# zser092/Focused-Attention-ViT

Hardware: AMD Instinct MI355X
Metric: images/sec (train fwd+bwd) ViT-MHLA 224/p16 (higher is better)
Workload: dtype bf16; 1 GPU; ViT-MHLA-Small (D384/12L/6H, window 7) 224x224 patch16, 197 tokens, 256 images/GPU; step = fwd + cross-entropy + bwd + grad all-reduce + AdamW; global_batch=256, parallelism=dp1, weights=random-init (seed 1234), hip_graph=False

## Files before the change

### focused-attention-vit_amd/_abi.py

```python
from __future__ import annotations

import ctypes as C
import os
import re

_HERE = os.path.dirname(os.path.abspath(__file__))
LIB_PATH = os.path.join(_HERE, "lib", "libfavit.so")
HEADER_PATH = os.path.join(os.path.dirname(_HERE), "include", "favit.h")

F32, BF16, FP8 = 0, 1, 2
F32X3 = 3
E4M3, E5M2 = 0, 1
ACT_NONE, ACT_GELU, ACT_DGELU, ACT_GELU_SAVEGRAD, ACT_MULAUX = 0, 1, 2, 3, 4
ERR_INVALID, ERR_UNSUPPORTED, ERR_ALIGN, ERR_LAUNCH = -1, -2, -3, -4
POOL = {"mean": 0, "max": 1, "attention": 2}

vp, i32, i64, u64, f32 = C.c_void_p, C.c_int32, C.c_int64, C.c_uint64, C.c_float


class GemmDesc(C.Structure):
    _fields_ = [
        ("A", vp), ("B", vp), ("C", vp), ("bias", vp), ("aux_in", vp), ("aux_out", vp), ("residual", vp),
        ("a_rowsum", vp),
        ("M", i64), ("N", i64), ("K", i64),
        ("lda", i64), ("ldb", i64), ("ldc", i64), ("ld_aux_in", i64), ("ld_aux_out", i64), ("ld_res", i64),
        ("sAo", i64), ("sAi", i64), ("sBo", i64), ("sBi", i64), ("sCo", i64), ("sCi", i64),
        ("batch", i32), ("batch_inner", i32), ("a_kmajor", i32), ("b_kmajor", i32),
        ("in_dtype", i32), ("out_dtype", i32), ("act", i32), ("accumulate", i32), ("split_k", i32),
        ("alpha", f32), ("dropout_p", f32), ("fp8_fmt", i32), ("dropout_seed", u64),
        ("scale_a", vp), ("scale_b", vp),
    ]


class SdpaDesc(C.Structure):
    _fields_ = [
        ("q", vp), ("k", vp), ("v", vp), ("o", vp), ("lse", vp), ("dout", vp), ("dq", vp), ("dk", vp), ("dv", vp),
        ("delta", vp), ("mask", vp), ("m_sb", i64), ("m_sq", i64),
        ("q_str", i64 * 3), ("k_str", i64 * 3), ("v_str", i64 * 3), ("o_str", i64 * 3), ("do_str", i64 * 3),
        ("dq_str", i64 * 3), ("dk_str", i64 * 3), ("dv_str", i64 * 3),
        ("B", i32), ("H", i32), ("Lq", i32), ("Lk", i32), ("hd", i32), ("dtype", i32),
        ("scale", f32), ("dropout_p", f32), ("seed", u64),
    ]


class BlockDesc(C.Structure):
    _fields_ = [
        ("x", vp), ("tape", vp), ("g1", vp), ("b1", vp), ("g2", vp), ("b2", vp), ("weff", vp), ("beff", vp),
        ("wproj", vp), ("bproj", vp), ("wfc1", vp), ("bfc1", vp), ("wfc2", vp), ("bfc2", vp),
        ("tape_bytes", i64),
        ("B", i32), ("n", i32), ("D", i32), ("H", i32), ("W", i32), ("hidden", i32), ("training", i32), ("eps", f32),
    ]


BLOCK_TAPE_SLOTS = ("xn1", "mu1", "rs1", "qkv", "o", "lse", "x1", "xn2", "mu2", "rs2", "h", "pre", "x2")
BLOCK_BWD_SLOTS = ("dpre", "dxn2", "g1_f32", "g1_lp", "do", "dqkv", "dxn1", "g_out_f32", "g_out_lp", "part1", "part2")

_SIGS = {
    "favit_abi_version": ([], C.c_int),
    "favit_strerror": ([C.c_int], C.c_char_p),
    "favit_set_dropout_epoch": ([vp], C.c_int),
    "favit_set_health_word": ([vp], C.c_int),
    "favit_gemm": ([C.POINTER(GemmDesc), vp], C.c_int),
    "favit_gemm_last_kernel": ([], C.c_char_p),
    "favit_ln_gemm": ([C.POINTER(GemmDesc), vp, i64, vp, vp, f32, vp, vp, vp, vp], C.c_int),
    "favit_gemm_grouped_tn": ([C.POINTER(GemmDesc), i32, vp], C.c_int),
    "favit_gemm_grouped_tn_workspace": ([C.POINTER(GemmDesc), i32], C.c_int64),
    "favit_gemm_grouped_tn_ws": ([C.POINTER(GemmDesc), i32, vp, i64, vp], C.c_int),
    "favit_gemm_grouped_tn_ragged": ([C.POINTER(GemmDesc), i32, vp], C.c_int),
    "favit_gemm_grouped_tn_ragged_workspace": ([C.POINTER(GemmDesc), i32], C.c_int64),
    "favit_gemm_grouped_tn_ragged_ws": ([C.POINTER(GemmDesc), i32, vp, i64, vp], C.c_int),
    "favit_gemm_grouped_last_splits": ([], C.c_int),
    "favit_gemm_grouped_plan": ([C.POINTER(GemmDesc), i32, i32, vp, i32], C.c_int),
    "favit_cast": ([vp, C.c_int, vp, C.c_int, i64, vp], C.c_int),
    "favit_fp8_amax": ([vp, C.c_int, i64, i64, i64, vp, vp], C.c_int),
    "favit_fp8_quantize": ([vp, C.c_int, i64, i64, i64, vp, i64, vp, i64, C.c_int, vp, vp, vp, vp, vp, vp], C.c_int),
    "favit_layernorm_fwd": ([vp, i64, vp, vp, vp, C.c_int, vp, vp, i64, i32, f32, vp], C.c_int),
    "favit_layernorm_bwd": ([vp, C.c_int, vp, i64, vp, vp, vp, vp, vp, i64, vp, C.c_int, vp, vp, i32, vp, vp, i32,
                             i64, i32, f32, u64, vp], C.c_int),
    "favit_layernorm_fwd_q8": ([vp, i64, vp, vp, vp, vp, vp, i64, i32, f32, vp, C.c_int, vp, vp, vp, vp, vp], C.c_int),
    "favit_layernorm_bwd_q8": ([vp, vp, i64, vp, vp, vp, vp, vp, i64, vp, vp, vp, i32, vp, vp, i32, i64, i32, f32, u64,
                                vp, C.c_int, vp, vp, vp, vp, vp], C.c_int),
    "favit_small_linear_fwd": ([vp, i64, vp, vp, vp, i32, i32, i32, vp], C.c_int),
    "favit_small_linear_bwd": ([vp, vp, i64, vp, vp, vp, vp, i32, i32, i32, i32, vp], C.c_int),
    "favit_reduce_rows": ([vp, i64, vp, i64, i32, i32, vp], C.c_int),
    "favit_reduce_rows_multi": ([i32, vp, vp, vp, i64, i32, vp], C.c_int),
    "favit_reduce_rows_multi_ragged": ([i32, vp, vp, vp, vp, i32, vp], C.c_int),
    "favit_mhla_fold_fwd": ([vp, vp, vp, vp, vp, C.c_int, vp, vp, i32, i32, vp], C.c_int),
    "favit_mhla_fold_fwd_multi": ([i32, vp, vp, vp, vp, vp, C.c_int, vp, i32, i32, vp], C.c_int),
    "favit_mhla_fold_bwd": ([vp, vp, vp, vp, vp, vp, vp, vp, vp, i32, i32, i32, vp], C.c_int),
    "favit_mhla_fold_bwd_multi": ([i32, vp, vp, vp, vp, vp, vp, vp, vp, vp, i32, i32, vp], C.c_int),
    "favit_mhla_attn_fwd": ([vp, vp, vp, i32, i32, i32, i32, i32, C.c_int, f32, u64, vp], C.c_int),
    "favit_mhla_attn_bwd": ([vp, vp, vp, vp, i32, i32, i32, i32, i32, C.c_int, f32, u64, vp], C.c_int),
    "favit_mhla_attn_lse_supported": ([i32, i32, i32, C.c_int], C.c_int),
    "favit_mhla_attn_fwd_lse": ([vp, vp, vp, vp, i32, i32, i32, i32, i32, C.c_int, f32, u64, vp], C.c_int),
    "favit_mhla_attn_bwd_lse": ([vp, vp, vp, vp, vp, vp, i32, i32, i32, i32, i32, C.c_int, f32, u64, vp], C.c_int),
    "favit_sdpa_fwd": ([C.POINTER(SdpaDesc), vp], C.c_int),
    "favit_sdpa_bwd": ([C.POINTER(SdpaDesc), vp], C.c_int),
    "favit_softmax_fwd": ([vp, vp, vp, C.c_int, vp, i64, i64, i32, i64, i32, i32, f32, u64, vp], C.c_int),
    "favit_softmax_bwd": ([vp, C.c_int, vp, vp, C.c_int, i64, i32, i32, f32, u64, vp], C.c_int),
    "favit_patchify_fwd": ([vp, vp, C.c_int, i32, i32, i32, i32, vp], C.c_int),
    "favit_patchify_bwd": ([vp, vp, i32, i32, i32, i32, vp], C.c_int),
    "favit_embed_prologue_fwd": ([vp, vp, vp, vp, i32, i32, i32, vp], C.c_int),
    "favit_embed_prologue_bwd": ([vp, vp, C.c_int, vp, vp, i32, i32, i32, vp], C.c_int),
    "favit_rows_cut_fwd": ([vp, vp, i32, i32, i32, i32, i32, vp], C.c_int),
    "favit_rows_cut_bwd": ([vp, vp, vp, C.c_int, i32, i32, i32, i32, i32, vp], C.c_int),
    "favit_mhla_block_tape_layout": ([C.POINTER(BlockDesc), C.POINTER(i64)], C.c_int64),
    "favit_mhla_block_bwd_layout": ([C.POINTER(BlockDesc), i32, C.POINTER(i64)], C.c_int64),
    "favit_mhla_block_fwd": ([C.POINTER(BlockDesc), vp], C.c_int),
    "favit_mhla_block_bwd": ([C.POINTER(BlockDesc), vp, vp, vp, i64, i32, vp], C.c_int),
    "favit_dropout": ([vp, vp, C.c_int, i64, f32, u64, vp], C.c_int),
    "favit_sppp_map_patches": ([vp, vp, vp, vp, vp, vp, i32, i32, i32, vp], C.c_int),
    "favit_sppp_pool_fwd": ([vp, vp, vp, vp, vp, i32, i32, i32, i32, i32, vp], C.c_int),
    "favit_sppp_pool_bwd": ([vp, vp, vp, vp, vp, vp, vp, i32, i32, i32, i32, i32, vp], C.c_int),
    "favit_sppp_centroids": ([vp, vp, i32, i32, i32, vp], C.c_int),
    "favit_sppp_posenc_fwd": ([vp, vp, vp, i32, i32, i32, i32, vp], C.c_int),
    "favit_image_transform": ([vp, vp, vp, vp, vp, i32, i32, i32, i32, i32, i32, C.POINTER(f32), C.POINTER(f32), vp], C.c_int),
    "favit_image_transform_ragged": ([vp, vp, vp, vp, vp, vp, i32, i32, i32, i32, C.POINTER(f32), C.POINTER(f32), vp], C.c_int),
    "favit_slic_features_workspace": ([i32, i32, i32], C.c_int64),
    "favit_slic_features": ([vp, vp, i32, i32, i32, f32, i32, vp, vp], C.c_int),
    "favit_slic_cluster_workspace": ([i32, i32], C.c_int64),
    "favit_slic_cluster": ([vp, vp, vp, i32, i32, i32, i32, i32, i64, i32, vp, vp], C.c_int),
    "favit_slic_connect": ([vp, vp, vp, vp, vp, i32, i32, i32, i32, vp], C.c_int),
    "favit_cross_entropy": ([vp, vp, vp, vp, i32, i32, f32, vp], C.c_int),
    "favit_adamw": ([vp, vp, vp, vp, vp, i64, f32, f32, f32, f32, f32, f32, f32, f32, vp], C.c_int),
    "favit_cross_entropy_ls": ([vp, vp, vp, vp, i32, i32, f32, f32, vp], C.c_int),
    "favit_grad_norm_workspace": ([], C.c_int64),
    "favit_grad_norm": ([i32, vp, vp, f32, f32, vp, vp, vp, i64, vp], C.c_int),
    "favit_adamw_clip": ([vp, vp, vp, vp, vp, i64, f32, f32, f32, f32, f32, f32, f32, f32, vp, i32, vp], C.c_int),
    "favit_adamw_ema": ([vp, vp, vp, vp, vp, vp, i64, f32, f32, f32, f32, f32, f32, f32, f32, f32, vp], C.c_int),
    "favit_adamw_clip_ema": ([vp, vp, vp, vp, vp, vp, i64, f32, f32, f32, f32, f32, f32, f32, f32, vp, i32, f32, vp],
                             C.c_int),
    "favit_swap_params": ([vp, vp, vp, i64, vp], C.c_int),
    "favit_batch_mix": ([vp, vp, vp, i32, i32, i32, i32, vp], C.c_int),
    "favit_cross_entropy_mix": ([vp, vp, vp, vp, vp, i32, i32, f32, f32, vp], C.c_int),
    "favit_randaugment_max_ops": ([], C.c_int),
    "favit_randaugment": ([vp, vp, vp, vp, vp, i32, vp, C.POINTER(f32), i32, u64, i32, i32, i32, C.POINTER(f32),
                           C.POINTER(f32), vp], C.c_int),
    "favit_random_erase": ([vp, vp, C.POINTER(f32), i32, u64, i32, i32, i32, i32, vp], C.c_int),
}

_lib = None


class FavitLibraryError(RuntimeError):
    pass


def declared_symbols():
    with open(HEADER_PATH) as f:
        txt = f.read()
    return sorted(set(re.findall(r"\b(favit_[a-z0-9_]+)\s*\(", txt)))


def lib():
    global _lib
    if _lib is None:
        if not os.path.exists(LIB_PATH):
            raise FavitLibraryError(
                f"{LIB_PATH} not found: build it with `python -c 'import __graft_entry__ as g; g.build()'` "
                "or `make -C focused-attention-vit_amd/csrc`.  There is no CPU / PyTorch fallback.")
        try:
            l = C.CDLL(LIB_PATH)
        except OSError as e:
            raise FavitLibraryError(f"cannot load {LIB_PATH}: {e}") from e
        for name, (args, res) in _SIGS.items():
            fn = getattr(l, name)
            fn.argtypes = args
            fn.restype = res
        _lib = l
    return _lib


def check(code: int, what: str):
    if code != 0:
        msg = lib().favit_strerror(code).decode()
        raise RuntimeError(f"{what} failed: {msg} (code {code})")
```

### focused-attention-vit_amd/csrc/block.hip

```cpp
#include <string.h>

#include "favit.h"

namespace {
constexpr int64_t ALIGN = 256;
constexpr int TAPE_N = FAVIT_BLOCK_TAPE_SLOTS, BWD_N = FAVIT_BLOCK_BWD_SLOTS;
enum { T_XN1, T_MU1, T_RS1, T_QKV, T_O, T_LSE, T_X1, T_XN2, T_MU2, T_RS2, T_H, T_PRE, T_X2 };
enum { G_DPRE, G_DXN2, G_G1_F32, G_G1_LP, G_DO, G_DQKV, G_DXN1, G_OUT_F32, G_OUT_LP, G_PART1, G_PART2 };

inline int64_t up(int64_t v) { return (v + ALIGN - 1) / ALIGN * ALIGN; }

int check_geometry(const favit_mhla_block_t* d) {
  if (!d) return FAVIT_ERR_INVALID;
  if (d->B <= 0 || d->n <= 0 || d->D <= 0 || d->H <= 0 || d->W <= 0 || d->hidden <= 0 || !(d->eps > 0.f))
    return FAVIT_ERR_INVALID;
  if (d->D % 64 != 0 || d->D % d->H != 0 || d->D / d->H != 64) return FAVIT_ERR_UNSUPPORTED;
  if (d->hidden % 8 != 0) return FAVIT_ERR_UNSUPPORTED;
  if (!favit_mhla_attn_lse_supported(d->n, 64, d->W, FAVIT_BF16)) return FAVIT_ERR_UNSUPPORTED;
  if ((int64_t)d->B * d->n >= (int64_t)1 << 31) return FAVIT_ERR_UNSUPPORTED;
  return FAVIT_OK;
}

int64_t layout(const int64_t* sizes, int n, int64_t* offsets) {
  int64_t off = 0;
  for (int i = 0; i < n; ++i) {
    if (offsets) offsets[i] = off;
    off += up(sizes[i]);
  }
  return off;
}

void tape_sizes(const favit_mhla_block_t* d, int64_t* s) {
  const int64_t M = (int64_t)d->B * d->n, D = d->D, Hd = d->hidden;
  s[T_XN1] = M * D * 2; s[T_MU1] = M * 4; s[T_RS1] = M * 4;
  s[T_QKV] = M * 3 * D * 2; s[T_O] = M * D * 2;
  s[T_LSE] = d->training ? (int64_t)d->B * d->H * d->n * 4 : 0;
  s[T_X1] = M * D * 4;
  s[T_XN2] = M * D * 2; s[T_MU2] = M * 4; s[T_RS2] = M * 4;
  s[T_H] = M * Hd * 2; s[T_PRE] = M * Hd * 2;
  s[T_X2] = M * D * 4;
}

int32_t ln_parts(int64_t rows) { return (int32_t)((rows + 3) / 4 < 2048 ? (rows + 3) / 4 : 2048); }

void bwd_sizes(const favit_mhla_block_t* d, int want_lp_out, int64_t* s) {
  const int64_t M = (int64_t)d->B * d->n, D = d->D, Hd = d->hidden;
  const int64_t part = 2 * (int64_t)ln_parts(M) * D * 4;
  s[G_DPRE] = M * Hd * 2; s[G_DXN2] = M * D * 2;
  s[G_G1_F32] = M * D * 4; s[G_G1_LP] = M * D * 2;
  s[G_DO] = M * D * 2; s[G_DQKV] = M * 3 * D * 2; s[G_DXN1] = M * D * 2;
  s[G_OUT_F32] = M * D * 4; s[G_OUT_LP] = want_lp_out ? M * D * 2 : 0;
  s[G_PART1] = part; s[G_PART2] = part;
}

favit_gemm_t gemm_base(const void* A, const void* B, void* C, int64_t M, int64_t N, int64_t K, int64_t ldb, int b_kmajor,
                       int out_dtype) {
  favit_gemm_t g;
  memset(&g, 0, sizeof(g));
  g.A = A; g.B = B; g.C = C;
  g.M = M; g.N = N; g.K = K;
  g.lda = K; g.ldb = ldb; g.ldc = N;
  g.batch = 1; g.batch_inner = 1;
  g.a_kmajor = 1; g.b_kmajor = b_kmajor;
  g.in_dtype = FAVIT_BF16; g.out_dtype = out_dtype;
  g.act = FAVIT_ACT_NONE;
  g.alpha = 1.0f;
  return g;
}

int check_params(const favit_mhla_block_t* d) {
  if (!d->x || !d->tape || !d->g1 || !d->b1 || !d->g2 || !d->b2 || !d->weff || !d->beff || !d->wproj || !d->bproj ||
      !d->wfc1 || !d->bfc1 || !d->wfc2 || !d->bfc2)
    return FAVIT_ERR_INVALID;
  if (((uintptr_t)d->tape % ALIGN) != 0 || ((uintptr_t)d->x % 16) != 0) return FAVIT_ERR_ALIGN;
  return FAVIT_OK;
}
}

extern "C" int64_t favit_mhla_block_tape_layout(const favit_mhla_block_t* desc, int64_t* offsets_out) {
  const int rc = check_geometry(desc);
  if (rc != FAVIT_OK) return rc;
  int64_t s[TAPE_N];
  tape_sizes(desc, s);
  return layout(s, TAPE_N, offsets_out);
}

extern "C" int64_t favit_mhla_block_bwd_layout(const favit_mhla_block_t* desc, int32_t want_lp_out, int64_t* offsets_out) {
  const int rc = check_geometry(desc);
  if (rc != FAVIT_OK) return rc;
  int64_t s[BWD_N];
  bwd_sizes(desc, want_lp_out, s);
  return layout(s, BWD_N, offsets_out);
}

extern "C" int favit_mhla_block_fwd(const favit_mhla_block_t* d, void* stream) {
  int rc = check_geometry(d);
  if (rc != FAVIT_OK) return rc;
  if ((rc = check_params(d)) != FAVIT_OK) return rc;
  int64_t s[TAPE_N], o[TAPE_N];
  tape_sizes(d, s);
  if (d->tape_bytes < layout(s, TAPE_N, o)) return FAVIT_ERR_INVALID;
  char* t = reinterpret_cast<char*>(d->tape);
  const int64_t M = (int64_t)d->B * d->n;
  const int32_t D = d->D, Hd = d->hidden;
  float* x1 = reinterpret_cast<float*>(t + o[T_X1]);
  if ((rc = favit_layernorm_fwd(d->x, D, d->g1, d->b1, t + o[T_XN1], FAVIT_BF16, reinterpret_cast<float*>(t + o[T_MU1]),
                                reinterpret_cast<float*>(t + o[T_RS1]), M, D, d->eps, stream)) != FAVIT_OK)
    return rc;
  favit_gemm_t g = gemm_base(t + o[T_XN1], d->weff, t + o[T_QKV], M, 3 * D, D, D, 1, FAVIT_BF16);
  g.bias = d->beff;
  g.ld_aux_out = 3 * D; g.ld_res = 3 * D;
  if ((rc = favit_gemm(&g, stream)) != FAVIT_OK) return rc;
  rc = d->training ? favit_mhla_attn_fwd_lse(t + o[T_QKV], t + o[T_O], reinterpret_cast<float*>(t + o[T_LSE]), nullptr,
                                             d->B, d->n, d->H, 64, d->W, FAVIT_BF16, 0.f, 0, stream)
                   : favit_mhla_attn_fwd(t + o[T_QKV], t + o[T_O], nullptr, d->B, d->n, d->H, 64, d->W, FAVIT_BF16, 0.f, 0,
                                         stream);
  if (rc != FAVIT_OK) return rc;
  g = gemm_base(t + o[T_O], d->wproj, x1, M, D, D, D, 1, FAVIT_F32);
  g.bias = d->bproj; g.residual = d->x;
  g.ld_aux_out = D; g.ld_res = D;
  if ((rc = favit_gemm(&g, stream)) != FAVIT_OK) return rc;
  if ((rc = favit_layernorm_fwd(x1, D, d->g2, d->b2, t + o[T_XN2], FAVIT_BF16, reinterpret_cast<float*>(t + o[T_MU2]),
                                reinterpret_cast<float*>(t + o[T_RS2]), M, D, d->eps, stream)) != FAVIT_OK)
    return rc;
  g = gemm_base(t + o[T_XN2], d->wfc1, t + o[T_H], M, Hd, D, D, 1, FAVIT_BF16);
  g.bias = d->bfc1; g.act = FAVIT_ACT_GELU_SAVEGRAD; g.aux_out = t + o[T_PRE];
  g.ld_aux_out = Hd; g.ld_res = Hd;
  if ((rc = favit_gemm(&g, stream)) != FAVIT_OK) return rc;
  g = gemm_base(t + o[T_H], d->wfc2, t + o[T_X2], M, D, Hd, Hd, 1, FAVIT_F32);
  g.bias = d->bfc2; g.residual = x1;
  g.ld_aux_out = D; g.ld_res = D;
  return favit_gemm(&g, stream);
}

extern "C" int favit_mhla_block_bwd(const favit_mhla_block_t* d, const float* g_f32, const void* g_lp, void* bwd_buffers,
                                    int64_t bwd_bytes, int32_t want_lp_out, void* stream) {
  int rc = check_geometry(d);
  if (rc != FAVIT_OK) return rc;
  if ((rc = check_params(d)) != FAVIT_OK) return rc;
  if (!d->training || !g_f32 || !g_lp || !bwd_buffers) return FAVIT_ERR_INVALID;
  if (((uintptr_t)bwd_buffers % ALIGN) != 0 || ((uintptr_t)g_f32 % 16) != 0 || ((uintptr_t)g_lp % 16) != 0)
    return FAVIT_ERR_ALIGN;
  int64_t s[TAPE_N], o[TAPE_N], bs[BWD_N], b[BWD_N];
  tape_sizes(d, s);
  if (d->tape_bytes < layout(s, TAPE_N, o)) return FAVIT_ERR_INVALID;
  bwd_sizes(d, want_lp_out, bs);
  if (bwd_bytes < layout(bs, BWD_N, b)) return FAVIT_ERR_INVALID;
  char* t = reinterpret_cast<char*>(d->tape);
  char* w = reinterpret_cast<char*>(bwd_buffers);
  const int64_t M = (int64_t)d->B * d->n;
  const int32_t D = d->D, Hd = d->hidden, np = ln_parts(M);
  float* g1 = reinterpret_cast<float*>(w + b[G_G1_F32]);
  float* part1 = reinterpret_cast<float*>(w + b[G_PART1]);
  float* part2 = reinterpret_cast<float*>(w + b[G_PART2]);
  favit_gemm_t g = gemm_base(g_lp, d->wfc2, w + b[G_DPRE], M, Hd, D, Hd, 0, FAVIT_BF16);
  g.act = FAVIT_ACT_MULAUX; g.aux_in = t + o[T_PRE]; g.ld_aux_in = Hd;
  if ((rc = favit_gemm(&g, stream)) != FAVIT_OK) return rc;
  g = gemm_base(w + b[G_DPRE], d->wfc1, w + b[G_DXN2], M, D, Hd, D, 0, FAVIT_BF16);
  g.ld_aux_in = D;
  if ((rc = favit_gemm(&g, stream)) != FAVIT_OK) return rc;
  if ((rc = favit_layernorm_bwd(w + b[G_DXN2], FAVIT_BF16, reinterpret_cast<const float*>(t + o[T_X1]), D, d->g2,
                                reinterpret_cast<const float*>(t + o[T_MU2]), reinterpret_cast<const float*>(t + o[T_RS2]),
                                g_f32, g1, D, w + b[G_G1_LP], FAVIT_BF16, part2, part2 + (int64_t)np * D, np, nullptr,
                                nullptr, 1, M, D, 0.f, 0, stream)) != FAVIT_OK)
    return rc;
  g = gemm_base(w + b[G_G1_LP], d->wproj, w + b[G_DO], M, D, D, D, 0, FAVIT_BF16);
  g.ld_aux_in = D;
  if ((rc = favit_gemm(&g, stream)) != FAVIT_OK) return rc;
  if ((rc = favit_mhla_attn_bwd_lse(t + o[T_QKV], w + b[G_DO], t + o[T_O], reinterpret_cast<const float*>(t + o[T_LSE]),
                                    w + b[G_DQKV], nullptr, d->B, d->n, d->H, 64, d->W, FAVIT_BF16, 0.f, 0, stream)) !=
      FAVIT_OK)
    return rc;
  g = gemm_base(w + b[G_DQKV], d->weff, w + b[G_DXN1], M, D, 3 * D, D, 0, FAVIT_BF16);
  g.ld_aux_in = D;
  if ((rc = favit_gemm(&g, stream)) != FAVIT_OK) return rc;
  return favit_layernorm_bwd(w + b[G_DXN1], FAVIT_BF16, d->x, D, d->g1, reinterpret_cast<const float*>(t + o[T_MU1]),
                             reinterpret_cast<const float*>(t + o[T_RS1]), g1, reinterpret_cast<float*>(w + b[G_OUT_F32]), D,
                             want_lp_out ? w + b[G_OUT_LP] : nullptr, FAVIT_BF16, part1, part1 + (int64_t)np * D, np, nullptr,
                             nullptr, 1, M, D, 0.f, 0, stream);
}
```

### focused-attention-vit_amd/functional.py

```python
from __future__ import annotations

import os
import weakref
from typing import List, Optional, Sequence, Tuple

import torch

from . import kernels as K
from ._abi import ACT_DGELU, ACT_GELU, ACT_GELU_SAVEGRAD, ACT_MULAUX, ACT_NONE

_STATE = {"cdt": torch.float32, "epoch": 0, "direct_grads": True, "grad_ready": None}


def set_direct_grads(on: bool) -> None:
    _STATE["direct_grads"] = bool(on)


def set_grad_ready_hook(fn) -> None:
    _STATE["grad_ready"] = fn


def _gt(p):
    if p is None or not _STATE["direct_grads"] or not getattr(p, "requires_grad", False):
        return None
    g = p.grad
    if g is None or g.dtype != torch.float32 or not g.is_contiguous() or g.shape != p.shape or not g.is_cuda:
        return None
    return g


def _ready(*params):
    fn = _STATE["grad_ready"]
    if fn is not None:
        for p in params:
            if p is not None:
                if _SIDE["active"]:
                    _SIDE["pending"].append(p)
                else:
                    fn(p)


_SIDE = {"enabled": False, "stream": None, "active": False, "pending": [], "used": False}


def set_side_stream(on: bool) -> None:
    _SIDE["enabled"] = bool(on)


class _side_stream:

    def __init__(self, *tensors):
        self.tensors = [t for t in tensors if t is not None]

    def __enter__(self):
        if not _SIDE["enabled"]:
            self.ctx = None
            return self
        if _SIDE["stream"] is None:
            _SIDE["stream"] = torch.cuda.Stream()
        s = _SIDE["stream"]
        s.wait_stream(torch.cuda.current_stream())
        for t in self.tensors:
            t.record_stream(s)
        self.ctx = torch.cuda.stream(s)
        self.ctx.__enter__()
        _SIDE["active"] = True
        _SIDE["used"] = True
        return self

    def __exit__(self, *exc):
        if self.ctx is not None:
            _SIDE["active"] = False
            self.ctx.__exit__(*exc)
        return False


def join_side_stream() -> None:
    if _SIDE["used"]:
        torch.cuda.current_stream().wait_stream(_SIDE["stream"])
        _SIDE["used"] = False
    if _SIDE["pending"]:
        fn = _STATE["grad_ready"]
        pend, _SIDE["pending"] = _SIDE["pending"], []
        if fn is not None:
            for p in pend:
                fn(p)


def set_compute_dtype(d) -> None:
    fp8 = x3 = False
    if isinstance(d, str):
        fp8 = d == "fp8"
        x3 = d == "fp32x3"
        d = {"fp32": torch.float32, "float32": torch.float32, "fp32x3": torch.float32, "bf16": torch.bfloat16,
             "bfloat16": torch.bfloat16, "fp8": torch.bfloat16}[d]
    if d not in (torch.float32, torch.bfloat16):
        raise ValueError("compute dtype must be fp32, fp32x3, bf16 or fp8")
    if d == torch.float32 and os.environ.get("FAVIT_FP32_GEMM") == "x3":
        x3 = True
    _STATE["cdt"] = d
    _STATE["fp8"] = fp8
    _STATE["x3"] = x3
    K.set_f32_gemm_split(x3)


def get_compute_mode() -> str:
    if _STATE.get("fp8"):
        return "fp8"
    if _STATE["cdt"] == torch.bfloat16:
        return "bf16"
    return "fp32x3" if _STATE.get("x3") else "fp32"


def get_compute_dtype() -> torch.dtype:
    return _STATE["cdt"]


def bump_weight_epoch(synced_mirrors=()) -> None:
    _STATE["epoch"] += 1
    for m in synced_mirrors:
        m.epoch = _STATE["epoch"]


class _LPMirror:
    __slots__ = ("flat_ref", "lp", "epoch", "versions", "params")

    def __init__(self, flat_p, lp, params=()):
        self.flat_ref, self.lp, self.params = weakref.ref(flat_p), lp, [weakref.ref(p) for p in params]
        self.mark_synced()

    def mark_synced(self):
        self.epoch = _STATE["epoch"]
        self.versions = {id(p): p._version for p in (r() for r in self.params) if p is not None}

    def refresh_if_stale(self) -> bool:
        fp = self.flat_ref()
        if fp is None:
            return False
        stale = self.epoch != _STATE["epoch"]
        if not stale:
            for r in self.params:
                p = r()
                if p is not None and self.versions.get(id(p), p._version) != p._version:
                    stale = True
                    break
        if stale:
            K.cast(fp, torch.bfloat16, out=self.lp)
            self.mark_synced()
        return stale

    def lookup(self, src, w):
        fp = self.flat_ref()
        if fp is None:
            return None
        base, ptr = fp.data_ptr(), w.data_ptr()
        if not (base <= ptr < base + 4 * fp.numel()):
            return False
        if self.epoch != _STATE["epoch"]:
            K.cast(fp, torch.bfloat16, out=self.lp)
            self.epoch = _STATE["epoch"]
        off = (ptr - base) // 4
        view = self.lp[off:off + w.numel()].view(w.shape)
        key = id(src)
        ver = src._version
        if self.versions.get(key, ver) != ver:
            K.cast(w, torch.bfloat16, out=view)
        self.versions[key] = ver
        return view


_LP_MIRRORS: List[_LPMirror] = []


def register_lp_mirror(flat_p: torch.Tensor, flat_lp: torch.Tensor, params=()) -> _LPMirror:
    m = _LPMirror(flat_p, flat_lp, params)
    _LP_MIRRORS.append(m)
    return m


def clear_lp_mirrors() -> None:
    _LP_MIRRORS.clear()


def invalidate_weight_cache() -> None:
    _STATE["epoch"] += 1


def wcast(w: torch.Tensor) -> torch.Tensor:
    cdt = _STATE["cdt"]
    src = w
    w = w.detach()
    if w.dtype == cdt and w.is_contiguous():
        return w
    if cdt == torch.bfloat16 and w.dtype == torch.float32 and w.is_contiguous():
        for m in list(_LP_MIRRORS):
            hit = m.lookup(src, w)
            if hit is None:
                _LP_MIRRORS.remove(m)
            elif hit is not False:
                return hit
    tag = (w.data_ptr(), tuple(w.shape), w._version, _STATE["epoch"], cdt)
    hit = getattr(src, "_favit_cast", None)
    if hit is not None and hit[0] == tag:
        return hit[1]
    c = K.cast(w, cdt)
    try:
        src._favit_cast = (tag, c)
    except AttributeError:
        pass
    return c


def set_dropout_epoch(word: Optional[torch.Tensor]) -> None:
    if word is not None:
        K.require_gpu(word)
        if word.dtype != torch.int64 or word.numel() != 1:
            raise TypeError("the dropout epoch is a one-element int64 device tensor")
    _STATE["drop_epoch"] = word
    from . import _abi
    _abi.check(_abi.lib().favit_set_dropout_epoch(None if word is None else word.data_ptr()), "favit_set_dropout_epoch")


def get_dropout_epoch() -> Optional[torch.Tensor]:
    return _STATE.get("drop_epoch")


def _seed() -> int:
    if torch.cuda.is_available() and torch.cuda.is_current_stream_capturing() and _STATE.get("drop_epoch") is None:
        raise RuntimeError("dropout inside a captured HIP graph: the seed is a kernel argument and would be frozen "
                           "into the graph; register a dropout epoch word first (functional.set_dropout_epoch; "
                           "train.GraphedStep does it for models with dropout)")
    return int(torch.empty((), dtype=torch.int64).random_().item())


_SEG = {"n": 1, "boundaries": []}


class encoder_segments:

    def __init__(self, n: int):
        self.n = max(1, int(n))

    def __enter__(self):
        self.prev = (_SEG["n"], _SEG["boundaries"])
        _SEG["n"], _SEG["boundaries"] = self.n, []
        self.boundaries = _SEG["boundaries"]
        return self

    def __exit__(self, *exc):
        _SEG["n"], _SEG["boundaries"] = self.prev
        return False


def get_encoder_segments() -> int:
    return _SEG["n"]


def note_segment_boundary(x: torch.Tensor) -> torch.Tensor:
    leaf = x.detach().requires_grad_(True)
    _SEG["boundaries"].append((x, leaf))
    return leaf


def _as_cdt(x: torch.Tensor) -> torch.Tensor:
    cdt = _STATE["cdt"]
    x = x.contiguous()
    return x if x.dtype == cdt else K.cast(x, cdt)


def _as_f32(x: torch.Tensor) -> torch.Tensor:
    x = x.contiguous()
    return x if x.dtype == torch.float32 else K.cast(x, torch.float32)


def _mask_u8(mask: Optional[torch.Tensor]) -> Optional[torch.Tensor]:
    if mask is None:
        return None
    return (mask != 0).to(torch.uint8).contiguous()


E4M3, E5M2 = torch.float8_e4m3fn, torch.float8_e5m2


_FP8_HIST = {}


def _fp8_hist(site, role: str):
    if site is None or torch.cuda.is_current_stream_capturing():
        return None
    key = (id(site), role)
    ent = _FP8_HIST.get(key)
    if ent is None or ent[0]() is not site:
        ent = (weakref.ref(site), K.Fp8History(site.device))
        _FP8_HIST[key] = ent
        if len(_FP8_HIST) > 4096:
            for k in [k for k, v in _FP8_HIST.items() if v[0]() is None]:
                del _FP8_HIST[k]
    return ent[1]


def _q8(t: torch.Tensor, fmt: torch.dtype, want_t: bool = False, hist=None):
    hit = getattr(t, "_favit_q8", None)
    if hit is not None and hit[0] == (fmt, t._version) and (hit[1][1] is not None or not want_t):
        return hit[1]
    q, qt, sinv = K.fp8_quantize(t, fmt, want=True, want_t=want_t, hist=hist)
    out = (q, qt, sinv)
    try:
        t._favit_q8 = ((fmt, t._version), out)
    except AttributeError:
        pass
    return out


def _q8_request(chain, prm, which: str, D: int):
    if not _STATE.get("fp8") or get_compute_dtype() != torch.bfloat16 or D % 64 != 0 or os.environ.get("FAVIT_FP8_NO_LNQ8"):
        return None
    idx = getattr(chain, "q8_" + which, None)
    if idx is None or prm is None or idx >= len(prm) or prm[idx] is None:
        return None
    hist = _fp8_hist(prm[idx], "a" if which == "fwd" else "dy")
    return None if hist is None else ((E4M3 if which == "fwd" else E5M2), hist)


def _use_fp8(allow, *mats, k_dims=()):
    if not (allow and _STATE.get("fp8")):
        return False
    return all(m.dtype == torch.bfloat16 and m.dim() == 2 and m.is_contiguous() for m in mats) and \
        all(k % 64 == 0 for k in k_dims)


def lin_fwd(a, w_c, bias, M, N, Kd, out_dtype, *, act=ACT_NONE, residual=None, want_pre=False, drop=(0.0, 0),
            allow_fp8=True, site=None):
    out = torch.empty((M, N), dtype=out_dtype, device=a.device)
    pre = torch.empty((M, N), dtype=out_dtype, device=a.device) if want_pre else None
    if _use_fp8(allow_fp8, a, w_c, k_dims=(Kd,)):
        aq, _, sa = _q8(a, E4M3, hist=_fp8_hist(site, "a"))
        wq, _, sw = _q8(w_c, E4M3, want_t=True, hist=_fp8_hist(site, "w"))
        K.gemm(aq, wq, out, M, N, Kd, Kd, Kd, N, bias=bias, act=act, aux_out=pre, ld_aux_out=N, residual=residual,
               ld_res=N, dropout_p=drop[0], dropout_seed=drop[1], scale_a=sa, scale_b=sw)
        return (out, pre) if want_pre else out
    K.gemm(a, w_c, out, M, N, Kd, Kd, Kd, N, bias=bias, act=act, aux_out=pre, ld_aux_out=N, residual=residual,
           ld_res=N, dropout_p=drop[0], dropout_seed=drop[1])
    return (out, pre) if want_pre else out


_LN_FUSE = bool(os.environ.get("FAVIT_LN_FUSE"))


def lin_fwd_ln(ln, w_c, bias, M, N, Kd, out_dtype, *, act=ACT_NONE, want_pre=False, drop=(0.0, 0)):
    x, gamma, beta = ln
    if _LN_FUSE and w_c.dtype == torch.bfloat16 and get_compute_mode() != "fp8":
        out = torch.empty((M, N), dtype=out_dtype, device=x.device)
        pre = torch.empty((M, N), dtype=out_dtype, device=x.device) if want_pre else None
        r = K.ln_gemm(x, Kd, gamma, beta, w_c, out, M, N, Kd, bias=bias, act=act, aux_out=pre, dropout_p=drop[0],
                      dropout_seed=drop[1])
        if r is not None:
            return (out, pre) + r
    xn, mu, rs = K.layernorm_fwd(x, Kd, gamma, beta, M, Kd, get_compute_dtype())
    o = lin_fwd(xn, w_c, bias, M, N, Kd, out_dtype, act=act, want_pre=want_pre, drop=drop)
    return (o + (xn, mu, rs)) if want_pre else (o, None, xn, mu, rs)


def lin_bwd_x(dy, w_c, M, N, Kd, out_dtype, *, dgelu_pre=None, pre_is_grad=False, drop=(0.0, 0), allow_fp8=True,
              site=None):
    dx = torch.empty((M, Kd), dtype=out_dtype, device=dy.device)
    act = (ACT_MULAUX if pre_is_grad else ACT_DGELU) if dgelu_pre is not None else ACT_NONE
    if _use_fp8(allow_fp8, dy, w_c, k_dims=(N,)) and (dgelu_pre is None or dgelu_pre.dtype == torch.bfloat16):
        dyq, _, sdy = _q8(dy, E5M2, hist=_fp8_hist(site, "dy"))
        _, wqt, sw = _q8(w_c, E4M3, want_t=True, hist=_fp8_hist(site, "w"))
        K.gemm(dyq, wqt, dx, M, Kd, N, N, wqt.stride(0), Kd, act=act, aux_in=dgelu_pre, ld_aux_in=Kd,
               dropout_p=drop[0], dropout_seed=drop[1], scale_a=sdy, scale_b=sw)
        return dx
    K.gemm(dy, w_c, dx, M, Kd, N, N, Kd, Kd, b_kmajor=False, act=act,
           aux_in=dgelu_pre, ld_aux_in=Kd, dropout_p=drop[0], dropout_seed=drop[1])
    return dx


_WG = {"list": None, "blocks": 0, "every": 1, "bytes": 0, "ragged": False, "ends": [], "blk_bytes": 0}
_WG_HOLD_BYTES = int(float(os.environ.get("FAVIT_WGRAD_HOLD_MB", "384")) * (1 << 20))
_WG_HOLD_RAGGED_BYTES = int(float(os.environ.get("FAVIT_WGRAD_HOLD_MB", "2048")) * (1 << 20))


def begin_wgrads(per_block: bool = False) -> None:
    every = 4 if _STATE["grad_ready"] is not None else K.GROUP_MAX // 4
    ragged = per_block
    if _SIDE["enabled"] or os.environ.get("FAVIT_WGRAD_PER_BLOCK"):
        every = 1
        ragged = False
    _WG.update(list=[], blocks=0, every=every, bytes=0, ragged=ragged, ends=[], blk_bytes=0)


def _launch_wgrads(probs) -> None:
    if not K.gemm_grouped_tn(probs):
        for dy, a, dw, db, acc in probs:
            K.gemm(dy, a, dw, dy.shape[1], a.shape[1], dy.shape[0], dy.stride(0), a.stride(0), dw.stride(0),
                   a_kmajor=False, b_kmajor=False, a_rowsum=db, accumulate=acc)


def flush_wgrads(force: bool = True, next_rows=None) -> bool:
    lst = _WG["list"]
    if lst is None:
        return True
    if not force:
        _WG["blocks"] += 1
        nb = _WG["blocks"]
        if _WG["ragged"]:
            ends = _WG["ends"]
            n_blk = len(lst) - (ends[-1] if ends else 0)
            b_blk = _WG["bytes"] - _WG["blk_bytes"]
            ends.append(len(lst))
            _WG["blk_bytes"] = _WG["bytes"]
            scale = next_rows[1] / max(next_rows[0], 1) if next_rows else 1.0
            if nb < _WG["every"] and _WG["bytes"] + b_blk * scale <= _WG_HOLD_RAGGED_BYTES and len(lst) + n_blk <= K.GROUP_MAX:
                return not lst
        elif nb < _WG["every"] and _WG["bytes"] * (nb + 1) <= _WG_HOLD_BYTES * nb and len(lst) * (nb + 1) <= K.GROUP_MAX * nb:
            return not lst
    ends = _WG["ends"]
    _WG.update(blocks=0, bytes=0, ends=[], blk_bytes=0)
    if lst:
        _WG["list"] = []
        probs = [(dy, a, dw, db, acc) for dy, a, dw, db, acc, _ in lst]
        with _side_stream(*[t for pr in probs for t in pr[:4]]):
            if not _WG["ragged"]:
                _launch_wgrads(probs)
            elif not K.gemm_grouped_tn_ragged(probs):
                bounds = [0] + [e for e in ends if 0 < e < len(probs)] + [len(probs)]
                for lo, hi in zip(bounds[:-1], bounds[1:]):
                    if hi > lo:
                        _launch_wgrads(probs[lo:hi])
            for *_, ready in lst:
                _ready(*ready)
    return True


def end_wgrads() -> None:
    flush_wgrads()
    _WG["list"] = None


_DEFER = {"on": False, "fold": [], "ln": []}


def begin_deferred() -> None:
    _DEFER.update(on=not _SIDE["enabled"], fold=[], ln=[])


def flush_deferred() -> None:
    if not _DEFER["on"]:
        return
    assert not _WG["list"], "the latent_proj fold reads weight gradients that have not been launched"
    fold, ln = _DEFER["fold"], _DEFER["ln"]
    _DEFER["fold"], _DEFER["ln"] = [], []
    if ln:
        by_cols = {}
        for e in ln:
            by_cols.setdefault(e[0].shape[-1], []).append(e)
        for es in by_cols.values():
            K.reduce_rows_multi([e[:3] for e in es])
        for e in ln:
            _ready(*e[3])
    by_h = {}
    for e in fold:
        by_h.setdefault((e[6], tuple(e[2].shape), e[5][0] is None), []).append(e)
    for (H, _, _), es in by_h.items():
        K.mhla_fold_bwd_multi([e[:6] for e in es], H)
        for e in es:
            _ready(*e[7])


def end_deferred() -> None:
    flush_deferred()
    _DEFER["on"] = False


_ZPOOL = {"buf": None, "off": 0}


def begin_zero_pool(n_floats: int, device) -> None:
    _ZPOOL["buf"] = torch.zeros(n_floats, dtype=torch.float32, device=device) if n_floats > 0 else None
    _ZPOOL["off"] = 0


def end_zero_pool() -> None:
    _ZPOOL["buf"] = None


def _zero_vec(n: int, device) -> torch.Tensor:
    buf = _ZPOOL["buf"]
    n4 = (n + 3) // 4 * 4
    if buf is not None and buf.device == device and _ZPOOL["off"] + n4 <= buf.numel():
        o = _ZPOOL["off"]
        _ZPOOL["off"] = o + n4
        return buf[o:o + n]
    return torch.zeros(n, dtype=torch.float32, device=device)


def lin_bwd_w(dy, a, M, N, Kd, want_bias=True, wp=None, bp=None, allow_fp8=True):
    frozen_w = wp is not None and not wp.requires_grad
    frozen_b = (not want_bias) or (bp is not None and not bp.requires_grad)
    if frozen_w and frozen_b:
        return None, None
    tw = _gt(wp)
    tb = _gt(bp) if want_bias else None
    dw = tw if tw is not None else torch.empty((N, Kd), dtype=torch.float32, device=dy.device)
    db = None
    if want_bias:
        db = tb if tb is not None else _zero_vec(N, dy.device)
    if _WG["list"] is not None and dy.dtype == torch.bfloat16:
        _WG["list"].append((dy, a, dw, db, tw is not None,
                            [p for p, t in ((wp, tw), (bp, tb)) if t is not None]))
        _WG["bytes"] += dy.numel() * dy.element_size() + a.numel() * a.element_size()
        return (None if tw is not None else dw), (None if tb is not None else db)
    with _side_stream(dy, a, dw, db):
        if not (dy.dtype == torch.bfloat16 and M >= 8192 and (db is not None or not want_bias) and
                K.gemm_grouped_tn([(dy, a, dw, db, tw is not None)])):
            K.gemm(dy, a, dw, N, Kd, M, N, Kd, Kd, a_kmajor=False, b_kmajor=False, a_rowsum=db,
                   accumulate=tw is not None)
    if tw is not None:
        _ready(wp)
    if tb is not None:
        _ready(bp)
    return (None if tw is not None else dw), (None if tb is not None else db)


class _View:
    __slots__ = ("t", "off", "ld", "sb", "sh")

    def __init__(self, t, off, ld, sb, sh):
        self.t, self.off, self.ld, self.sb, self.sh = t, off, ld, sb, sh


def sdpa_fwd(q: _View, k: _View, v: _View, o: _View, B, H, Lq, Lk, hd, scale, mask, m_sb, m_sq, p, seed):
    if hd % 16 == 0:
        return (K.sdpa_fwd(q, k, v, o, B, H, Lq, Lk, hd, scale, mask, m_sb, m_sq, p, seed),)
    cdt = q.t.dtype
    Z = B * H
    S = torch.empty((Z, Lq, Lk), dtype=torch.float32, device=q.t.device)
    K.gemm(q.t, k.t, S, Lq, Lk, hd, q.ld, k.ld, Lk, alpha=scale, batch=Z, batch_inner=H, sA=(q.sb, q.sh),
           sB=(k.sb, k.sh), sC=(H * Lq * Lk, Lq * Lk), a_off=q.off, b_off=k.off)
    P, Pd = K.softmax_fwd(S, cdt, H, Z, Lq, Lk, mask, m_sb, m_sq, p, seed)
    K.gemm(Pd, v.t, o.t, Lq, hd, Lk, Lk, v.ld, o.ld, b_kmajor=False, batch=Z, batch_inner=H,
           sA=(H * Lq * Lk, Lq * Lk), sB=(v.sb, v.sh), sC=(o.sb, o.sh), b_off=v.off, c_off=o.off)
    return P, Pd


def sdpa_bwd(q: _View, k: _View, v: _View, o: _View, do: _View, dq: _View, dk: _View, dv: _View, saved, B, H, Lq, Lk,
             hd, scale, mask, m_sb, m_sq, p, seed):
    if len(saved) == 1:
        K.sdpa_bwd(q, k, v, o, do, dq, dk, dv, saved[0], B, H, Lq, Lk, hd, scale, mask, m_sb, m_sq, p, seed)
        return
    P, Pd = saved
    Z = B * H
    sP = (H * Lq * Lk, Lq * Lk)
    dPd = torch.empty((Z, Lq, Lk), dtype=torch.float32, device=q.t.device)
    K.gemm(do.t, v.t, dPd, Lq, Lk, hd, do.ld, v.ld, Lk, batch=Z, batch_inner=H, sA=(do.sb, do.sh), sB=(v.sb, v.sh),
           sC=sP, a_off=do.off, b_off=v.off)
    dS = K.softmax_bwd(P, dPd, Z, Lq, Lk, p, seed)
    K.gemm(dS, k.t, dq.t, Lq, hd, Lk, Lk, k.ld, dq.ld, b_kmajor=False, alpha=scale, batch=Z, batch_inner=H, sA=sP,
           sB=(k.sb, k.sh), sC=(dq.sb, dq.sh), b_off=k.off, c_off=dq.off)
    K.gemm(dS, q.t, dk.t, Lk, hd, Lq, Lk, q.ld, dk.ld, a_kmajor=False, b_kmajor=False, alpha=scale, batch=Z,
           batch_inner=H, sA=sP, sB=(q.sb, q.sh), sC=(dk.sb, dk.sh), b_off=q.off, c_off=dk.off)
    K.gemm(Pd, do.t, dv.t, Lk, hd, Lq, Lk, do.ld, dv.ld, a_kmajor=False, b_kmajor=False, batch=Z, batch_inner=H,
           sA=sP, sB=(do.sb, do.sh), sC=(dv.sb, dv.sh), b_off=do.off, c_off=dv.off)


class MHLAChain:
    q8_fwd, q8_bwd = 0, 4
    """MultiHeadLatentAttention.forward (models/mhla.py:85-161)."""
    names = ("qkv.weight", "qkv.bias", "latent_proj.weight", "latent_proj.bias", "proj.weight", "proj.bias")

    def __init__(self, H, W, p_attn=0.0, p_proj=0.0):
        if W % 2 == 0:
            raise ValueError("window_size must be odd: the reference crashes on even sizes (models/mhla.py:83)")
        self.H, self.W, self.p_attn, self.p_proj = H, W, p_attn, p_proj

    def fwd(self, xn, prm, B, L, residual, mask, training, pre=None, ln=None):
        wqkv, bqkv, wl, bl, wp, bp = prm
        M, D = xn.shape if ln is None else ln[0].shape
        cdt = xn.dtype if ln is None else get_compute_dtype()
        H, hd = self.H, D // self.H
        pa = self.p_attn if training else 0.0
        pp = self.p_proj if training else 0.0
        sa = _seed() if pa > 0 else 0
        sp = _seed() if pp > 0 else 0
        weff, beff = pre if pre is not None else K.mhla_fold_fwd(wqkv, bqkv, wl, bl, H, cdt)
        if ln is not None:
            qkv, _, xn, mu, rs = lin_fwd_ln(ln[:3], weff, beff, M, 3 * D, D, cdt)
            ln[3][:] = [xn, mu, rs]
        else:
            qkv = lin_fwd(xn, weff, beff, M, 3 * D, D, xn.dtype, site=wqkv)
        o, lse = K.mhla_attn_fwd(qkv, B, L, H, hd, self.W, mask, pa, sa, want_lse=True) if training else \
            (K.mhla_attn_fwd(qkv, B, L, H, hd, self.W, mask, pa, sa), None)
        wp_c = wcast(wp)
        y = lin_fwd(o, wp_c, bp.detach(), M, D, D, torch.float32, residual=residual, drop=(pp, sp), site=wp)
        return y, (xn, weff, qkv, o, wp_c, mask, B, L, pa, sa, pp, sp, prm, lse)

    @staticmethod
    def out_dropout(saved):
        return saved[10], saved[11]

    def bwd(self, saved, dy_lp, premasked=False):
        xn, weff, qkv, o, wp_c, mask, B, L, pa, sa, pp, sp, prm, lse = saved
        wqkv, bqkv, wl, bl, wp, bp = prm
        M, D = xn.shape
        H, hd = self.H, D // self.H
        dym = K.dropout(dy_lp, pp, sp) if (pp > 0 and not premasked) else dy_lp
        do = lin_bwd_x(dym, wp_c, M, D, D, xn.dtype, site=wp)
        dwp, dbp = self.proj_grads(dym, o, prm)
        dqkv = K.mhla_attn_bwd(qkv, do, B, L, H, hd, self.W, mask, pa, sa, o=o if lse is not None else None, lse=lse)
        dxn = lin_bwd_x(dqkv, weff, M, 3 * D, D, xn.dtype, site=wqkv)
        return dxn, self.qkv_grads(dqkv, xn, prm) + [dwp, dbp]

    @staticmethod
    def proj_grads(dym, o, prm):
        M, D = o.shape
        return lin_bwd_w(dym, o, M, D, D, wp=prm[4], bp=prm[5])

    def qkv_grads(self, dqkv, xn, prm):
        wqkv, bqkv, wl, bl = prm[:4]
        M, D = xn.shape
        H = self.H
        dweff, dbeff = lin_bwd_w(dqkv, xn, M, 3 * D, D)
        tg = [_gt(p) for p in (wqkv, bqkv, wl, bl)]
        if all(t is not None for t in tg) and _DEFER["on"]:
            _DEFER["fold"].append((dweff, dbeff, wqkv.detach(), bqkv.detach(), wl.detach(), tg, H, (wqkv, bqkv, wl, bl)))
            return [None, None, None, None]
        if (_DEFER["on"] and not wqkv.requires_grad and not bqkv.requires_grad and tg[2] is not None and tg[3] is not None):
            _DEFER["fold"].append((dweff, dbeff, wqkv.detach(), bqkv.detach(), wl.detach(), [None, None, tg[2], tg[3]], H,
                                   (wl, bl)))
            return [None, None, None, None]
        flush_wgrads()
        if all(t is not None for t in tg):
            with _side_stream(dweff, dbeff):
                K.mhla_fold_bwd(dweff, dbeff, wqkv, bqkv, wl, H, out=tg)
                _ready(wqkv, bqkv, wl, bl)
            return [None, None, None, None]
        join_side_stream()
        return list(K.mhla_fold_bwd(dweff, dbeff, wqkv, bqkv, wl, H))


class DenseChain:
    q8_fwd, q8_bwd = 0, 2
    """vit.MultiHeadAttention.forward (models/vit.py:77-104) and, with the
    nn.MultiheadAttention parameter names, the use_mhla=False branch
    (models/vit_mhla.py:57-62,96-101).  mask: key-keep [B,L] (torch MHA) or None."""

    def __init__(self, H, p_attn=0.0, p_proj=0.0, torch_mha=False):
        self.H, self.p_attn, self.p_proj, self.torch_mha = H, p_attn, p_proj, torch_mha
        self.names = (("in_proj_weight", "in_proj_bias", "out_proj.weight", "out_proj.bias") if torch_mha
                      else ("qkv.weight", "qkv.bias", "proj.weight", "proj.bias"))

    def _views(self, t, B, L, D, hd):
        ld = 3 * D
        return (_View(t, 0, ld, L * ld, hd), _View(t, D, ld, L * ld, hd), _View(t, 2 * D, ld, L * ld, hd))

    def fwd(self, xn, prm, B, L, residual, mask, training, ln=None):
        wqkv, bqkv, wp, bp = prm
        M, D = xn.shape if ln is None else ln[0].shape
        H, hd = self.H, D // self.H
        pa = self.p_attn if training else 0.0
        pp = self.p_proj if (training and not self.torch_mha) else 0.0
        sa = _seed() if pa > 0 else 0
        sp = _seed() if pp > 0 else 0
        wqkv_c, wp_c = wcast(wqkv), wcast(wp)
        if ln is not None:
            qkv, _, xn, mu, rs = lin_fwd_ln(ln[:3], wqkv_c, bqkv.detach(), M, 3 * D, D, get_compute_dtype())
            ln[3][:] = [xn, mu, rs]
        else:
            qkv = lin_fwd(xn, wqkv_c, bqkv.detach(), M, 3 * D, D, xn.dtype, site=wqkv)
        o = torch.empty((M, D), dtype=xn.dtype, device=xn.device)
        q, k, v = self._views(qkv, B, L, D, hd)
        ov = _View(o, 0, D, L * D, hd)
        att = sdpa_fwd(q, k, v, ov, B, H, L, L, hd, hd ** -0.5, mask, L if mask is not None else 0, 0, pa, sa)
        y = lin_fwd(o, wp_c, bp.detach(), M, D, D, torch.float32, residual=residual, drop=(pp, sp), site=wp)
        return y, (xn, wqkv_c, qkv, o, wp_c, att, mask, B, L, pa, sa, pp, sp, prm)

    @staticmethod
    def out_dropout(saved):
        return saved[11], saved[12]

    def bwd(self, saved, dy_lp, premasked=False):
        xn, wqkv_c, qkv, o, wp_c, att, mask, B, L, pa, sa, pp, sp, prm = saved
        wqkv, bqkv, wp, bp = prm
        M, D = xn.shape
        H, hd = self.H, D // self.H
        dym = K.dropout(dy_lp, pp, sp) if (pp > 0 and not premasked) else dy_lp
        do = lin_bwd_x(dym, wp_c, M, D, D, xn.dtype, site=wp)
        dwp, dbp = lin_bwd_w(dym, o, M, D, D, wp=wp, bp=bp)
        dqkv = torch.empty_like(qkv)
        q, k, v = self._views(qkv, B, L, D, hd)
        dq, dk, dv = self._views(dqkv, B, L, D, hd)
        sdpa_bwd(q, k, v, _View(o, 0, D, L * D, hd), _View(do, 0, D, L * D, hd), dq, dk, dv, att, B, H, L, L, hd,
                 hd ** -0.5, mask, L if mask is not None else 0, 0, pa, sa)
        dxn = lin_bwd_x(dqkv, wqkv_c, M, 3 * D, D, xn.dtype, site=wqkv)
        dwqkv, dbqkv = lin_bwd_w(dqkv, xn, M, 3 * D, D, wp=wqkv, bp=bqkv)
        return dxn, [dwqkv, dbqkv, dwp, dbp]


class CrossChain:
    names = ("q_proj.weight", "q_proj.bias", "k_proj.weight", "k_proj.bias", "v_proj.weight", "v_proj.bias",
             "out_proj.weight", "out_proj.bias")

    def __init__(self, H, p_attn=0.0):
        self.H, self.p_attn = H, p_attn

    def fwd(self, qn, kn, prm, B, Lq, Lk, residual, mask, training):
        wq, bq, wk, bk, wv, bv, wo, bo = prm
        D = qn.shape[1]
        H, hd = self.H, D // self.H
        pa = self.p_attn if training else 0.0
        sa = _seed() if pa > 0 else 0
        cdt = qn.dtype
        wq_c, wk_c, wv_c, wo_c = wcast(wq), wcast(wk), wcast(wv), wcast(wo)
        q = lin_fwd(qn, wq_c, bq.detach(), B * Lq, D, D, cdt)
        k = lin_fwd(kn, wk_c, bk.detach(), B * Lk, D, D, cdt)
        v = lin_fwd(kn, wv_c, bv.detach(), B * Lk, D, D, cdt)
        o = torch.empty((B * Lq, D), dtype=cdt, device=qn.device)
        scale = 1.0 / (hd ** 0.5)
        att = sdpa_fwd(_View(q, 0, D, Lq * D, hd), _View(k, 0, D, Lk * D, hd), _View(v, 0, D, Lk * D, hd),
                       _View(o, 0, D, Lq * D, hd), B, H, Lq, Lk, hd, scale, mask,
                       Lq * Lk if mask is not None else 0, Lk if mask is not None else 0, pa, sa)
        y = lin_fwd(o, wo_c, bo.detach(), B * Lq, D, D, torch.float32, residual=residual)
        return y, (qn, kn, q, k, v, o, (wq_c, wk_c, wv_c, wo_c), att, mask, B, Lq, Lk, pa, sa, scale, prm)

    def bwd(self, saved, dy_lp):
        qn, kn, q, k, v, o, (wq_c, wk_c, wv_c, wo_c), att, mask, B, Lq, Lk, pa, sa, scale, prm = saved
        wq, bq, wk, bk, wv, bv, wo, bo = prm
        D = qn.shape[1]
        H, hd = self.H, D // self.H
        cdt = qn.dtype
        Mq, Mk = B * Lq, B * Lk
        do = lin_bwd_x(dy_lp, wo_c, Mq, D, D, cdt)
        dwo, dbo = lin_bwd_w(dy_lp, o, Mq, D, D, wp=wo, bp=bo)
        dq, dk, dv = torch.empty_like(q), torch.empty_like(k), torch.empty_like(v)
        sdpa_bwd(_View(q, 0, D, Lq * D, hd), _View(k, 0, D, Lk * D, hd), _View(v, 0, D, Lk * D, hd),
                 _View(o, 0, D, Lq * D, hd), _View(do, 0, D, Lq * D, hd), _View(dq, 0, D, Lq * D, hd),
                 _View(dk, 0, D, Lk * D, hd), _View(dv, 0, D, Lk * D, hd), att, B, H, Lq, Lk, hd, scale, mask,
                 Lq * Lk if mask is not None else 0, Lk if mask is not None else 0, pa, sa)
        dqn = lin_bwd_x(dq, wq_c, Mq, D, D, cdt)
        dwq, dbq = lin_bwd_w(dq, qn, Mq, D, D, wp=wq, bp=bq)
        dkn = torch.empty((Mk, D), dtype=torch.float32, device=qn.device)
        K.gemm(dk, wk_c, dkn, Mk, D, D, D, D, D, b_kmajor=False)
        K.gemm(dv, wv_c, dkn, Mk, D, D, D, D, D, b_kmajor=False, accumulate=True)
        dwk, dbk = lin_bwd_w(dk, kn, Mk, D, D, wp=wk, bp=bk)
        dwv, dbv = lin_bwd_w(dv, kn, Mk, D, D, wp=wv, bp=bv)
        return dqn, dkn, [dwq, dbq, dwk, dbk, dwv, dbv, dwo, dbo]


class MLPChain:
    q8_fwd, q8_bwd = 0, 2
    """MLP.forward fc1 -> GELU -> drop -> fc2 -> drop (models/vit.py:124-139)."""

    def __init__(self, p=0.0, fc1="fc1", fc2="fc2"):
        self.p = p
        self.names = (f"{fc1}.weight", f"{fc1}.bias", f"{fc2}.weight", f"{fc2}.bias")

    def fwd(self, xn, prm, residual, training, ln=None):
        w1, b1, w2, b2 = prm
        M, D = xn.shape if ln is None else ln[0].shape
        Hd = w1.shape[0]
        Do = w2.shape[0]
        p = self.p if training else 0.0
        s1 = _seed() if p > 0 else 0
        s2 = _seed() if p > 0 else 0
        w1_c, w2_c = wcast(w1), wcast(w2)
        if ln is not None:
            sg = True
            h, pre, xn, mu, rs = lin_fwd_ln(ln[:3], w1_c, b1.detach(), M, Hd, D, get_compute_dtype(), act=ACT_GELU_SAVEGRAD,
                                            want_pre=True, drop=(p, s1))
            ln[3][:] = [xn, mu, rs]
        else:
            sg = self.saves_gelu_grad(xn.dtype)
            h, pre = lin_fwd(xn, w1_c, b1.detach(), M, Hd, D, xn.dtype, act=ACT_GELU_SAVEGRAD if sg else ACT_GELU,
                             want_pre=True, drop=(p, s1), site=w1)
        y = lin_fwd(h, w2_c, b2.detach(), M, Do, Hd, torch.float32, residual=residual, drop=(p, s2), site=w2)
        return y, (xn, (pre, sg), h, w1_c, w2_c, p, s1, s2, prm)

    @staticmethod
    def saves_gelu_grad(cdt) -> bool:
        return cdt != torch.float32

    @staticmethod
    def out_dropout(saved):
        return saved[5], saved[7]

    def bwd(self, saved, dy_lp, premasked=False):
        xn, (pre, sg), h, w1_c, w2_c, p, s1, s2, prm = saved
        w1, b1, w2, b2 = prm
        M, D = xn.shape
        Hd, Do = w1_c.shape[0], w2_c.shape[0]
        dym = K.dropout(dy_lp, p, s2) if (p > 0 and not premasked) else dy_lp
        dpre = lin_bwd_x(dym, w2_c, M, Do, Hd, xn.dtype, dgelu_pre=pre, pre_is_grad=sg, drop=(p, s1), site=w2)
        dw2, db2 = self.fc2_grads(dym, h, prm)
        dxn = lin_bwd_x(dpre, w1_c, M, Hd, D, xn.dtype, site=w1)
        dw1, db1 = self.fc1_grads(dpre, xn, prm)
        return dxn, [dw1, db1, dw2, db2]

    @staticmethod
    def fc2_grads(dym, h, prm):
        return lin_bwd_w(dym, h, dym.shape[0], dym.shape[1], h.shape[1], wp=prm[2], bp=prm[3])

    @staticmethod
    def fc1_grads(dpre, xn, prm):
        return lin_bwd_w(dpre, xn, dpre.shape[0], dpre.shape[1], xn.shape[1], wp=prm[0], bp=prm[1])


class OpFn(torch.autograd.Function):

    @staticmethod
    def forward(ctx, op, n_in, *tensors):
        K.require_gpu(*[t for t in tensors if t is not None])
        ins, prm = tensors[:n_in], tensors[n_in:]
        out, saved = op.fwd(ins, prm)
        ctx.op, ctx.saved, ctx.n_in, ctx.n_prm = op, saved, n_in, len(prm)
        return out

    @staticmethod
    def backward(ctx, dout):
        din, dprm = ctx.op.bwd(ctx.saved, _as_f32(dout), ctx.needs_input_grad[2:2 + ctx.n_in])
        join_side_stream()
        ctx.saved = None
        return (None, None, *din, *dprm)


def run(op, inputs: Sequence[torch.Tensor], params: Sequence[torch.Tensor]) -> torch.Tensor:
    return OpFn.apply(op, len(inputs), *inputs, *params)


class LinearOp:

    def __init__(self, act=ACT_NONE):
        self.act = act

    def fwd(self, ins, prm):
        (x,), (w, b) = ins, prm
        shp = x.shape
        N = w.shape[0]
        if (self.act == ACT_NONE and N <= K.SMALL_LINEAR_MAX_N and x.dtype == torch.float32 and w.dtype == torch.float32
                and (b is None or b.dtype == torch.float32)):
            x2 = x.reshape(-1, shp[-1])
            if x2.stride(-1) != 1:
                x2 = x2.contiguous()
            y = K.small_linear_fwd(x2, w.detach(), None if b is None else b.detach())
            return y.reshape(*shp[:-1], N), ("small", x2, shp, b is not None, (w, b))
        a = _as_cdt(x.reshape(-1, shp[-1]))
        w_c = wcast(w)
        M, Kd, N = a.shape[0], a.shape[1], w.shape[0]
        y = lin_fwd(a, w_c, None if b is None else b.detach(), M, N, Kd, torch.float32, allow_fp8=False)
        return y.reshape(*shp[:-1], N), (a, w_c, shp, b is not None, (w, b))

    def bwd(self, saved, dy, needs):
        if isinstance(saved[0], str):
            _, x2, shp, has_b, (w, b) = saved
            M, N = x2.shape[0], w.shape[0]
            dy2 = _as_f32(dy.reshape(M, N))
            if not dy2.is_contiguous():
                dy2 = dy2.contiguous()
            tw, tb = _gt(w), (_gt(b) if has_b else None)
            direct = tw is not None and (tb is not None or not has_b)
            dx, dw, db = K.small_linear_bwd(dy2, x2, w.detach(), want_dx=bool(needs[0]), want_db=has_b,
                                            dw_out=tw if direct else None, db_out=tb if direct else None)
            if direct:
                _ready(w, *( [b] if has_b else [] ))
            dx = dx.reshape(shp) if dx is not None else None
            return [dx], [dw, db] if has_b else [dw]
        a, w_c, shp, has_b, (w, b) = saved
        M, Kd, N = a.shape[0], a.shape[1], w_c.shape[0]
        dy_c = _as_cdt(dy.reshape(M, N))
        dx = lin_bwd_x(dy_c, w_c, M, N, Kd, torch.float32, allow_fp8=False).reshape(shp) if needs[0] else None
        dw, db = lin_bwd_w(dy_c, a, M, N, Kd, want_bias=has_b, wp=w, bp=b, allow_fp8=False)
        return [dx], [dw, db] if has_b else [dw]


class PatchEmbedOp:

    def __init__(self, P):
        self.P = P

    def fwd(self, ins, prm):
        (img,), (w, b) = ins, prm
        B, Cc, HW, _ = img.shape
        patches = K.patchify_fwd(_as_f32(img), self.P, get_compute_dtype())
        M, Kd = patches.shape
        D = w.shape[0]
        w_c = wcast(w)
        tok = lin_fwd(patches, w_c, b.detach(), M, D, Kd, torch.float32, allow_fp8=False)
        return tok.reshape(B, M // B, D), (patches, w_c, (B, Cc, HW), (w, b))

    def bwd(self, saved, dy, needs):
        patches, w_c, (B, Cc, HW), (w, b) = saved
        M, Kd = patches.shape
        D = w_c.shape[0]
        dy_c = _as_cdt(dy.reshape(M, D))
        dw, db = lin_bwd_w(dy_c, patches, M, D, Kd, wp=w if w.is_leaf else None, bp=b, allow_fp8=False)
        dimg = None
        if needs[0]:
            dpatch = lin_bwd_x(dy_c, w_c, M, D, Kd, torch.float32, allow_fp8=False)
            dimg = K.patchify_bwd(dpatch, B, Cc, HW, self.P)
        return [dimg], [dw, db]


class PrologueOp:

    def __init__(self, has_pos):
        self.has_pos = has_pos

    def fwd(self, ins, prm):
        (tok,) = ins
        cls = prm[0]
        pos = prm[1] if self.has_pos else None
        B, N, D = tok.shape
        x = K.embed_prologue_fwd(_as_f32(tok), cls.detach().contiguous(), None if pos is None else pos.detach().contiguous(),
                                 B, N, D)
        return x, (B, N, D)

    def bwd(self, saved, dy, needs):
        B, N, D = saved
        dtok, dcls, dpos = K.embed_prologue_bwd(dy, B, N, D, torch.float32, want_pos=self.has_pos)
        out = [dcls.reshape(1, 1, D)]
        if self.has_pos:
            out.append(dpos.reshape(1, N + 1, D))
        return [dtok.reshape(B, N, D)], out


class BlockSpec:

    def __init__(self, attn, mlp):
        self.attn, self.mlp = attn, mlp
        self.names = (("norm1.weight", "norm1.bias") + tuple("attn." + n for n in attn.names) +
                      ("norm2.weight", "norm2.bias") + tuple("mlp." + n for n in mlp.names))
        self.n = len(self.names)


def cls_plan(L: int, W: int, depth: int) -> List[Optional[Tuple[int, int]]]:
    h = W // 2
    plan: List[Optional[Tuple[int, int]]] = []
    for k in range(1, depth + 1):
        j = depth - k
        a, b = 1 + h * (j + 1), 1 + h * j
        plan.append(None if a + b >= L else (a, b))
    return plan


def cls_only_cuts(specs: Sequence["BlockSpec"], L: int, mask, training: bool):
    if os.environ.get("FAVIT_NO_PRUNE") or mask is not None or not specs or _STATE.get("fp8"):
        return None
    if not all(isinstance(s.attn, MHLAChain) and isinstance(s.mlp, MLPChain) for s in specs):
        return None
    if len({s.attn.W for s in specs}) != 1:
        return None
    if training and any(s.attn.p_attn > 0 or s.attn.p_proj > 0 or s.mlp.p > 0 for s in specs):
        return None
    plan = cls_plan(L, specs[0].attn.W, len(specs))
    return plan if any(c is not None for c in plan) else None


_NATIVE = {"on": True}


def set_native_blocks(on: bool) -> None:
    _NATIVE["on"] = bool(on)


def _native_blocks_on() -> bool:
    return (_NATIVE["on"] and K.GEMM_TRACE is None and not _SIDE["enabled"] and not _LN_FUSE
            and get_compute_mode() == "bf16" and not os.environ.get("FAVIT_NO_NATIVE_BLOCKS"))


def _carve(flat, off, shape):
    st, n = [], 1
    for d in reversed(shape):
        st.append(n)
        n *= d
    return torch.as_strided(flat, shape, tuple(reversed(st)), off)


class _NativeTape:
    __slots__ = ("plan", "buf", "x", "ln", "pa", "pm", "weff", "wc", "cut", "_bf", "_f32")

    def __init__(self, plan, buf, x, ln, pa, pm, weff, wc, cut):
        self.plan, self.buf, self.x, self.ln, self.pa, self.pm, self.weff, self.wc, self.cut = \
            plan, buf, x, ln, pa, pm, weff, wc, cut
        self._bf = self._f32 = None

    def bf(self, name, *shape):
        if self._bf is None:
            self._bf = self.buf.view(torch.bfloat16)
        return _carve(self._bf, self.plan.off[name][0] // 2, shape)

    def f32(self, name, *shape):
        if self._f32 is None:
            self._f32 = self.buf.view(torch.float32)
        return _carve(self._f32, self.plan.off[name][0] // 4, shape)

    def unpack(self):
        pl = self.plan
        M, D, Hd = pl.M, pl.D, pl.hidden
        (g1, b1, g2, b2), (wp_c, w1_c, w2_c) = self.ln, self.wc
        lse = self.f32("lse", pl.B, pl.H, pl.n) if pl.off["lse"][1] else None
        sa = (self.bf("xn1", M, D), self.weff, self.bf("qkv", M, 3 * D), self.bf("o", M, D), wp_c, None, pl.B, pl.n,
              0.0, 0, 0.0, 0, self.pa, lse)
        sm = (self.bf("xn2", M, D), (self.bf("pre", M, Hd), MLPChain.saves_gelu_grad(torch.bfloat16)), self.bf("h", M, Hd),
              w1_c, w2_c, 0.0, 0, 0, self.pm)
        return (self.x, self.f32("mu1", M), self.f32("rs1", M), (g1, b1), sa, self.f32("x1", M, D), self.f32("mu2", M),
                self.f32("rs2", M), (g2, b2), sm, (self.pa, self.pm), self.cut)


def _tape_cut(tp):
    return tp.cut if isinstance(tp, _NativeTape) else tp[11]


def _tape_rows(tp):
    return tp.plan.M if isinstance(tp, _NativeTape) else tp[0].shape[0]


class EncoderOp:

    def __init__(self, blocks: List[BlockSpec], mask=None, training=False, cuts=None):
        self.blocks, self.mask, self.training = blocks, mask, training
        self.cuts = list(cuts) if cuts is not None else None
        if self.cuts is not None and (len(self.cuts) != len(blocks) or mask is not None):
            raise ValueError("cuts: one entry per block, and no attention mask")

    def fwd(self, ins, prm):
        (x,) = ins
        B, L, D = x.shape
        M = B * L
        L_in = L
        cdt = get_compute_dtype()
        x = _as_f32(x).reshape(M, D)
        tapes = []
        fuse_ok = _LN_FUSE and cdt == torch.bfloat16 and get_compute_mode() == "bf16" and D % 64 == 0 and D <= 512
        pre = [None] * len(self.blocks)
        idx, fp, off = [], [], 0
        for bi, bs in enumerate(self.blocks):
            if isinstance(bs.attn, MHLAChain):
                idx.append(bi)
                fp.append(tuple(prm[off + 2:off + 6]))
            off += bs.n
        if 2 <= len(idx) <= 32 and len({(self.blocks[i].attn.H, tuple(q[0].shape)) for i, q in zip(idx, fp)}) == 1:
            for bi, we in zip(idx, K.mhla_fold_fwd_multi(fp, self.blocks[idx[0]].attn.H, cdt)):
                pre[bi] = we
        native = self.mask is None and x.is_cuda and _native_blocks_on()
        off = 0
        for bi, bs in enumerate(self.blocks):
            p = list(prm[off:off + bs.n])
            off += bs.n
            na = len(bs.attn.names)
            g1, b1 = p[0], p[1]
            pa = p[2:2 + na]
            g2, b2 = p[2 + na], p[3 + na]
            pm = p[4 + na:]
            cut = None
            if self.cuts is not None and self.cuts[bi] is not None and sum(self.cuts[bi]) < L:
                ca, cb = self.cuts[bi]
                x = K.rows_cut_fwd(x, B, L, ca, cb, D).reshape(B * (ca + cb), D)
                cut = (L, ca, cb)
                L = ca + cb
                M = B * L
            if native and pre[bi] is not None:
                nt = self._fwd_native(bs, p, x, B, L, D, pre[bi], cut)
                if nt is not None:
                    tapes.append(nt)
                    x = nt.f32("x2", M, D)
                    continue
            fuse = fuse_ok and M <= 16384
            if fuse and isinstance(bs.attn, (MHLAChain, DenseChain)):
                o1 = [None, None, None]
                kw = {"pre": pre[bi]} if pre[bi] is not None else {}
                x1, sa = bs.attn.fwd(None, pa, B, L, x, self.mask, self.training, ln=(x, g1.detach(), b1.detach(), o1), **kw)
                xn1, mu1, rs1 = o1
            else:
                xn1, mu1, rs1 = K.layernorm_fwd(x, D, g1, b1, M, D, cdt, q8=_q8_request(bs.attn, pa, "fwd", D))
                if pre[bi] is not None:
                    x1, sa = bs.attn.fwd(xn1, pa, B, L, x, self.mask, self.training, pre=pre[bi])
                else:
                    x1, sa = bs.attn.fwd(xn1, pa, B, L, x, self.mask, self.training)
            if fuse and isinstance(bs.mlp, MLPChain):
                o2 = [None, None, None]
                x2, sm = bs.mlp.fwd(None, pm, x1, self.training, ln=(x1, g2.detach(), b2.detach(), o2))
                xn2, mu2, rs2 = o2
            else:
                xn2, mu2, rs2 = K.layernorm_fwd(x1, D, g2, b2, M, D, cdt, q8=_q8_request(bs.mlp, pm, "fwd", D))
                x2, sm = bs.mlp.fwd(xn2, pm, x1, self.training)
            tapes.append((x, mu1, rs1, (g1, b1), sa, x1, mu2, rs2, (g2, b2), sm, (pa, pm), cut))
            x = x2
        return x.reshape(B, L, D), (tapes, B, L_in, D)

    def _fwd_native(self, bs, p, x, B, L, D, pre, cut):
        at, ml = bs.attn, bs.mlp
        if not (isinstance(at, MHLAChain) and isinstance(ml, MLPChain)) or len(p) != 14:
            return None
        if self.training and (at.p_attn > 0 or at.p_proj > 0 or ml.p > 0):
            return None
        g1, b1, wqkv, bqkv, wl, bl, wp, bp, g2, b2, w1, c1, w2, c2 = p
        Hd = w1.shape[0]
        if tuple(w2.shape) != (D, Hd) or tuple(w1.shape) != (Hd, D) or tuple(wp.shape) != (D, D):
            return None
        if any(t.dtype != torch.float32 or not t.is_contiguous() for t in (g1, b1, g2, b2, bp, c1, c2)):
            return None
        weff, beff = pre
        wc = (wcast(wp), wcast(w1), wcast(w2))
        if weff.dtype != torch.bfloat16 or any(w.dtype != torch.bfloat16 or not w.is_contiguous() for w in wc):
            return None
        plans = getattr(g1, "_favit_blocks", None)
        if plans is None:
            plans = g1._favit_blocks = {}
        key = (B, L, D, at.H, at.W, Hd, bool(self.training))
        if key not in plans:
            plans[key] = K.mhla_block_plan(*key)
        plan = plans[key]
        if plan is None:
            return None
        buf = torch.empty(plan.tape_bytes, dtype=torch.uint8, device=x.device)
        if K.mhla_block_fwd(plan, x, buf, g1, b1, g2, b2, weff, beff, wc[0], bp, wc[1], c1, wc[2], c2) != 0:
            return None
        return _NativeTape(plan, buf, x, (g1, b1, g2, b2), p[2:8], p[10:], weff, wc, cut)

    def _bwd_native(self, bs, tp, g, g_lp):
        plan = tp.plan
        g1, b1, g2, b2 = tp.ln
        tg = [_gt(q) for q in tp.ln]
        if any(t is None for t in tg):
            return None
        M, D, Hd = plan.M, plan.D, plan.hidden
        if (g.dtype != torch.float32 or g_lp.dtype != torch.bfloat16 or tuple(g.shape) != (M, D) or not g.is_contiguous()
                or tuple(g_lp.shape) != (M, D) or not g_lp.is_contiguous()):
            return None
        want_lp = tp.cut is None
        arena = torch.empty(plan.bwd_bytes[want_lp], dtype=torch.uint8, device=g.device)
        wp_c, w1_c, w2_c = tp.wc
        if K.mhla_block_bwd(plan, tp.x, tp.buf, g1, g2, tp.weff, wp_c, w1_c, w2_c, g, g_lp, arena, want_lp) != 0:
            return None
        bo = plan.boff[want_lp]
        abf, af = arena.view(torch.bfloat16), arena.view(torch.float32)
        part = lambda k: _carve(af, bo[k][0] // 4, (2, plan.nparts, D))
        g1_lp = _carve(abf, bo["g1_lp"][0] // 2, (M, D))
        dqkv = _carve(abf, bo["dqkv"][0] // 2, (M, 3 * D))
        dw2, db2 = bs.mlp.fc2_grads(g_lp, tp.bf("h", M, Hd), tp.pm)
        dw1, db1 = bs.mlp.fc1_grads(_carve(abf, bo["dpre"][0] // 2, (M, Hd)), tp.bf("xn2", M, D), tp.pm)
        _DEFER["ln"].append((part("part2"), tg[2], tg[3], (g2, b2)))
        dwp, dbp = bs.attn.proj_grads(g1_lp, tp.bf("o", M, D), tp.pa)
        ga = bs.attn.qkv_grads(dqkv, tp.bf("xn1", M, D), tp.pa) + [dwp, dbp]
        _DEFER["ln"].append((part("part1"), tg[0], tg[1], (g1, b1)))
        g_out = _carve(af, bo["g_out_f32"][0] // 4, (M, D))
        return g_out, (_carve(abf, bo["g_out_lp"][0] // 2, (M, D)) if want_lp else None), ga, [dw1, db1, dw2, db2]

    def bwd(self, saved, dy, needs):
        tapes, B, L, D = saved
        g = dy.reshape(-1, D)
        g_lp = _as_cdt(g)
        grads = []
        begin_wgrads(per_block=any(_tape_cut(tp) is not None for tp in tapes))
        begin_deferred()
        begin_zero_pool(sum(3 * D + 4 for bs in self.blocks if isinstance(bs.attn, MHLAChain)), dy.device)

        def ln_bwd(dxn, xin, gam, bet, mu, rs, dres, pd, q8=None, want_lp=True):
            M = xin.shape[0]
            if not gam.requires_grad and not bet.requires_grad:
                return K.layernorm_bwd(dxn, xin, D, gam, mu, rs, M, D, dres=dres, want_lp=want_lp, lp_drop=pd, frozen=True, q8=q8)
            tg_, tb_ = _gt(gam), _gt(bet)
            lst = _DEFER["ln"] if (_DEFER["on"] and tg_ is not None and tb_ is not None) else None
            n0 = len(lst) if lst is not None else 0
            out = K.layernorm_bwd(dxn, xin, D, gam, mu, rs, M, D, dres=dres, want_lp=want_lp, dg_out=tg_, db_out=tb_,
                                  lp_drop=pd, defer=lst, q8=q8)
            if lst is not None:
                lst[n0] = lst[n0] + ((gam, bet),)
            elif out[2] is None:
                _ready(gam, bet)
            return out
        try:
            order = list(zip(reversed(self.blocks), reversed(tapes)))
            premasked = False
            for bi, (bs, tp) in enumerate(order):
                pd_n, q8n = (0.0, 0), None
                if bi + 1 < len(order) and not isinstance(order[bi + 1][1], _NativeTape):
                    nbs, ntp = order[bi + 1]
                    pd_n = nbs.mlp.out_dropout(ntp[9])
                    q8n = _q8_request(nbs.mlp, ntp[10][1], "bwd", D)
                done = None
                if isinstance(tp, _NativeTape):
                    if not premasked and pd_n[0] == 0 and q8n is None and _DEFER["on"] and _native_blocks_on():
                        done = self._bwd_native(bs, tp, g, g_lp)
                    if done is None:
                        tp = tp.unpack()
                if done is not None:
                    g, g_lp, ga, gm = done
                    dg1 = db1 = dg2 = db2 = None
                    cut, lp_dt = tp.cut, torch.bfloat16
                else:
                    x, mu1, rs1, (g1, b1), sa, x1, mu2, rs2, (g2, b2), sm, (pa_, _), cut = tp
                    dxn2, gm = bs.mlp.bwd(sm, g_lp, premasked=premasked)
                    pd = bs.attn.out_dropout(sa) if hasattr(bs.attn, "out_dropout") else (0.0, 0)
                    g, g_lp, dg2, db2 = ln_bwd(dxn2, x1, g2, b2, mu2, rs2, g, pd,
                                               q8=_q8_request(bs.attn, pa_, "bwd", D) if hasattr(bs.attn, "out_dropout") else None)
                    dxn1, ga = (bs.attn.bwd(sa, g_lp, premasked=pd[0] > 0) if hasattr(bs.attn, "out_dropout")
                                else bs.attn.bwd(sa, g_lp))
                    g, g_lp, dg1, db1 = ln_bwd(dxn1, x, g1, b1, mu1, rs1, g, pd_n, q8=q8n, want_lp=cut is None)
                    lp_dt = dxn1.dtype
                premasked = pd_n[0] > 0
                if cut is not None:
                    n_in, ca, cb = cut
                    more = bi + 1 < len(order) and g.dtype != lp_dt
                    g, g_lp = K.rows_cut_bwd(g, B, n_in, ca, cb, D, lp_dtype=lp_dt if more else None)
                    g = g.reshape(B * n_in, D)
                    g_lp = g_lp.reshape(B * n_in, D) if g_lp is not None else g
                nxt = (_tape_rows(tp), _tape_rows(order[bi + 1][1])) if bi + 1 < len(order) else None
                if flush_wgrads(force=False, next_rows=nxt) and _STATE["grad_ready"] is not None:
                    flush_deferred()
                if not _SIDE["enabled"]:
                    join_side_stream()
                grads = [dg1, db1] + ga + [dg2, db2] + gm + grads
        except BaseException:
            _WG["list"] = None
            _SIDE["pending"].clear()
            _DEFER.update(on=False, fold=[], ln=[])
            end_zero_pool()
            raise
        end_wgrads()
        end_deferred()
        end_zero_pool()
        join_side_stream()
        return [g.reshape(B, L, D)], grads


class FinalNormOp:

    def fwd(self, ins, prm):
        (x,), (g, b) = ins, prm
        B, L, D = x.shape
        x = _as_f32(x)
        y, mu, rs = K.layernorm_fwd(x, L * D, g, b, B, D, torch.float32)
        return y, (x, mu, rs, (g, b), (B, L, D))

    def bwd(self, saved, dy, needs):
        x, mu, rs, (g, b), (B, L, D) = saved
        dx = torch.zeros((B, L, D), dtype=torch.float32, device=x.device)
        _, _, dg, db = K.layernorm_bwd(dy, x, L * D, g, mu, rs, B, D, dx=dx, lddx=L * D, dg_out=_gt(g), db_out=_gt(b))
        if dg is None:
            _ready(g, b)
        return [dx], [dg, db]


class AttnOp:

    def __init__(self, chain, mask=None, training=False):
        self.chain, self.mask, self.training = chain, mask, training

    def fwd(self, ins, prm):
        (x,) = ins
        B, L, D = x.shape
        xn = _as_cdt(x.reshape(B * L, D))
        y, saved = self.chain.fwd(xn, list(prm), B, L, None, self.mask, self.training)
        return y.reshape(B, L, D), (saved, (B, L, D))

    def bwd(self, saved, dy, needs):
        s, (B, L, D) = saved
        dxn, grads = self.chain.bwd(s, _as_cdt(dy.reshape(B * L, D)))
        return [_as_f32(dxn).reshape(B, L, D)], grads


class MLPOp:
    def __init__(self, chain, training=False):
        self.chain, self.training = chain, training

    def fwd(self, ins, prm):
        (x,) = ins
        shp = x.shape
        xn = _as_cdt(x.reshape(-1, shp[-1]))
        y, saved = self.chain.fwd(xn, list(prm), None, self.training)
        return y.reshape(*shp[:-1], y.shape[-1]), (saved, shp)

    def bwd(self, saved, dy, needs):
        s, shp = saved
        dxn, grads = self.chain.bwd(s, _as_cdt(dy.reshape(-1, dy.shape[-1])))
        return [_as_f32(dxn).reshape(shp)], grads


class CrossAttnOp:

    def __init__(self, chain, mask=None, training=False):
        self.chain, self.mask, self.training = chain, mask, training

    def fwd(self, ins, prm):
        q, kv = ins
        B, Lq, D = q.shape
        Lk = kv.shape[1]
        qn, kn = _as_cdt(q.reshape(B * Lq, D)), _as_cdt(kv.reshape(B * Lk, D))
        y, saved = self.chain.fwd(qn, kn, list(prm), B, Lq, Lk, None, self.mask, self.training)
        return y.reshape(B, Lq, D), (saved, (B, Lq, Lk, D))

    def bwd(self, saved, dy, needs):
        s, (B, Lq, Lk, D) = saved
        dqn, dkn, grads = self.chain.bwd(s, _as_cdt(dy.reshape(B * Lq, D)))
        return [_as_f32(dqn).reshape(B, Lq, D), dkn.reshape(B, Lk, D)], grads


class CrossBlockOp:

    def __init__(self, chain, mlp, mask=None, training=False):
        self.chain, self.mlp, self.mask, self.training = chain, mlp, mask, training
        self.names = (("norm1_query.weight", "norm1_query.bias", "norm1_kv.weight", "norm1_kv.bias") +
                      tuple("attn." + n for n in chain.names) + ("norm2.weight", "norm2.bias") +
                      tuple("mlp." + n for n in mlp.names))

    def fwd(self, ins, prm):
        q, kv = ins
        B, Lq, D = q.shape
        Lk = kv.shape[1]
        Mq, Mk = B * Lq, B * Lk
        cdt = get_compute_dtype()
        p = list(prm)
        q2, kv2 = _as_f32(q).reshape(Mq, D), _as_f32(kv).reshape(Mk, D)
        qn, muq, rsq = K.layernorm_fwd(q2, D, p[0], p[1], Mq, D, cdt)
        kn, muk, rsk = K.layernorm_fwd(kv2, D, p[2], p[3], Mk, D, cdt)
        x1, sa = self.chain.fwd(qn, kn, p[4:12], B, Lq, Lk, q2, self.mask, self.training)
        xn2, mu2, rs2 = K.layernorm_fwd(x1, D, p[12], p[13], Mq, D, cdt)
        x2, sm = self.mlp.fwd(xn2, p[14:], x1, self.training)
        return x2.reshape(B, Lq, D), (q2, kv2, muq, rsq, muk, rsk, sa, x1, mu2, rs2, sm, p, (B, Lq, Lk, D))

    def bwd(self, saved, dy, needs):
        q2, kv2, muq, rsq, muk, rsk, sa, x1, mu2, rs2, sm, p, (B, Lq, Lk, D) = saved
        Mq, Mk = B * Lq, B * Lk
        g = dy.reshape(Mq, D)
        dxn2, gm = self.mlp.bwd(sm, _as_cdt(g))
        g, g_lp, dg2, db2 = K.layernorm_bwd(dxn2, x1, D, p[12], mu2, rs2, Mq, D, dres=g, want_lp=True)
        dqn, dkn, ga = self.chain.bwd(sa, g_lp)
        dq, _, dgq, dbq = K.layernorm_bwd(dqn, q2, D, p[0], muq, rsq, Mq, D, dres=g)
        dkv, _, dgk, dbk = K.layernorm_bwd(dkn, kv2, D, p[2], muk, rsk, Mk, D)
        return [dq.reshape(B, Lq, D), dkv.reshape(B, Lk, D)], [dgq, dbq, dgk, dbk] + ga + [dg2, db2] + gm


class PoolOp:

    def __init__(self, kind, perm, offs, R):
        self.kind, self.perm, self.offs, self.R = kind, perm, offs, R

    def fwd(self, ins, prm):
        (emb,) = ins
        emb = _as_f32(emb)
        out, argmax = K.sppp_pool_fwd(emb, self.perm, self.offs, self.kind, self.R)
        return out, (emb, argmax)

    def bwd(self, saved, dy, needs):
        emb, argmax = saved
        return [K.sppp_pool_bwd(dy, emb, self.perm, self.offs, argmax, self.kind, self.R)], []


class PosEncOp:

    def __init__(self, cent):
        self.cent = cent

    def fwd(self, ins, prm):
        (x,) = ins
        return K.sppp_posenc_fwd(_as_f32(x), self.cent), None

    def bwd(self, saved, dy, needs):
        return [dy], []


class DropoutOp:

    def __init__(self, p):
        self.p = p

    def fwd(self, ins, prm):
        s = _seed()
        return K.dropout(_as_f32(ins[0]), self.p, s), s

    def bwd(self, saved, dy, needs):
        return [K.dropout(dy, self.p, saved)], []
```

### focused-attention-vit_amd/kernels.py

```python
from __future__ import annotations

import ctypes as C
import math
from typing import Optional

import numpy as np
import torch

from . import _abi
from ._abi import ACT_DGELU, ACT_GELU, ACT_NONE, BF16, F32, GemmDesc, SdpaDesc

_DT = {torch.float32: F32, torch.bfloat16: BF16}

_F32_GEMM = {"in_dtype": F32}


def set_f32_gemm_split(on: bool) -> None:
    _F32_GEMM["in_dtype"] = _abi.F32X3 if on else F32

GEMM_TRACE = None


def dt(t_or_dtype) -> int:
    d = t_or_dtype.dtype if torch.is_tensor(t_or_dtype) else t_or_dtype
    try:
        return _DT[d]
    except KeyError:
        raise TypeError(f"favit kernels support float32 / bfloat16 only, got {d}") from None


def require_gpu(*ts):
    cur = None
    for t in ts:
        if t is None:
            continue
        if not t.is_cuda:
            raise RuntimeError(
                "focused-attention-vit_amd runs its hot path in HIP kernels on an MI355X; got a CPU tensor. "
                "There is no CPU fallback (move the module and its inputs to the GPU).")
        if cur is None:
            cur = torch.cuda.current_device()
        if t.device.index != cur:
            raise RuntimeError(
                f"tensor on cuda:{t.device.index} but the current device is cuda:{cur}: one process drives one GPU "
                "(torch.cuda.set_device(local_rank) before building the model), or wrap the call in "
                "`with torch.cuda.device(t.device):`")


def _p(t: Optional[torch.Tensor]):
    return None if t is None else C.c_void_p(t.data_ptr())


def _st():
    return C.c_void_p(torch.cuda.current_stream().cuda_stream)


def gemm(A, B, Cc, M, N, K, lda, ldb, ldc, *, a_kmajor=True, b_kmajor=True, bias=None, act=ACT_NONE,
         aux_in=None, ld_aux_in=0, aux_out=None, ld_aux_out=0, residual=None, ld_res=0, a_rowsum=None,
         accumulate=False, alpha=1.0, batch=1, batch_inner=1, sA=(0, 0), sB=(0, 0), sC=(0, 0), split_k=0,
         a_off=0, b_off=0, c_off=0, dropout_p=0.0, dropout_seed=0, scale_a=None, scale_b=None, in_dtype=None):
    require_gpu(A, B, Cc)
    fp8 = A.dtype in _FP8_DT
    if fp8:
        if B.dtype != torch.float8_e4m3fn:
            raise TypeError("fp8 gemm: B must be float8_e4m3fn")
    elif A.dtype != B.dtype:
        raise TypeError("gemm operands must share a dtype")
    d = GemmDesc()
    ea, ec = A.element_size(), Cc.element_size()
    d.A = A.data_ptr() + a_off * ea
    d.B = B.data_ptr() + b_off * ea
    d.C = Cc.data_ptr() + c_off * ec
    d.bias = bias.data_ptr() if bias is not None else None
    d.aux_in = aux_in.data_ptr() if aux_in is not None else None
    d.aux_out = aux_out.data_ptr() if aux_out is not None else None
    d.residual = residual.data_ptr() if residual is not None else None
    d.a_rowsum = a_rowsum.data_ptr() if a_rowsum is not None else None
    d.M, d.N, d.K = M, N, K
    d.lda, d.ldb, d.ldc = lda, ldb, ldc
    d.ld_aux_in, d.ld_aux_out, d.ld_res = ld_aux_in, ld_aux_out, ld_res
    d.sAo, d.sAi = sA
    d.sBo, d.sBi = sB
    d.sCo, d.sCi = sC
    d.batch, d.batch_inner = batch, batch_inner
    d.a_kmajor, d.b_kmajor = int(a_kmajor), int(b_kmajor)
    d.in_dtype, d.out_dtype = (_abi.FP8 if fp8 else dt(A)), dt(Cc)
    if d.in_dtype == F32:
        d.in_dtype = _F32_GEMM["in_dtype"] if in_dtype is None else in_dtype
    elif in_dtype is not None:
        raise TypeError("in_dtype selects the product of fp32 operands only")
    if fp8:
        d.fp8_fmt = 1 if A.dtype == torch.float8_e5m2 else 0
        d.scale_a = scale_a.data_ptr() if scale_a is not None else None
        d.scale_b = scale_b.data_ptr() if scale_b is not None else None
    d.act = act
    d.accumulate = int(accumulate)
    d.split_k = split_k
    d.alpha = alpha
    d.dropout_p = dropout_p
    d.dropout_seed = dropout_seed
    if bias is not None and bias.dtype != torch.float32:
        raise TypeError("bias must be fp32")
    if residual is not None and residual.dtype != torch.float32:
        raise TypeError("residual must be fp32")
    if GEMM_TRACE is None:
        _abi.check(_abi.lib().favit_gemm(C.byref(d), _st()), "favit_gemm")
        return
    e0, e1 = torch.cuda.Event(enable_timing=True), torch.cuda.Event(enable_timing=True)
    e0.record()
    _abi.check(_abi.lib().favit_gemm(C.byref(d), _st()), "favit_gemm")
    e1.record()
    key = ("fp8" if fp8 else "bf16" if A.dtype == torch.bfloat16 else "f32x3" if d.in_dtype == _abi.F32X3 else "f32") + ("_K" if a_kmajor else "_M") + ("K" if b_kmajor else "M") + \
          ("_obf16" if Cc.dtype == torch.bfloat16 else "_of32")
    GEMM_TRACE.append((e0, e1, 2.0 * M * N * K * batch, key, (M, N, K, batch), _abi.lib().favit_gemm_last_kernel().decode()))


def ln_gemm(x, ldx, gamma, beta, w, out, M, N, D, *, bias=None, act=ACT_NONE, aux_in=None, ld_aux_in=0, aux_out=None,
            residual=None, dropout_p=0.0, dropout_seed=0, eps=1e-5):
    require_gpu(x, gamma, beta, w, out)
    if w.dtype != torch.bfloat16 or x.dtype != torch.float32:
        return None
    d = GemmDesc()
    d.A = None
    d.B, d.C = w.data_ptr(), out.data_ptr()
    d.bias = bias.data_ptr() if bias is not None else None
    d.aux_in = aux_in.data_ptr() if aux_in is not None else None
    d.aux_out = aux_out.data_ptr() if aux_out is not None else None
    d.residual = residual.data_ptr() if residual is not None else None
    d.M, d.N, d.K = M, N, D
    d.lda, d.ldb, d.ldc = D, w.stride(0), out.stride(0)
    d.ld_aux_in, d.ld_aux_out, d.ld_res = ld_aux_in, N, N
    d.batch, d.batch_inner = 1, 1
    d.a_kmajor, d.b_kmajor = 1, 1
    d.in_dtype, d.out_dtype = BF16, dt(out)
    d.act, d.alpha = act, 1.0
    d.dropout_p, d.dropout_seed = dropout_p, dropout_seed
    xn = torch.empty((M, D), dtype=torch.bfloat16, device=x.device)
    mean = torch.empty(M, dtype=torch.float32, device=x.device)
    rstd = torch.empty(M, dtype=torch.float32, device=x.device)
    if GEMM_TRACE is not None:
        e0, e1 = torch.cuda.Event(enable_timing=True), torch.cuda.Event(enable_timing=True)
        e0.record()
    rc = _abi.lib().favit_ln_gemm(C.byref(d), _p(x), ldx, _p(gamma), _p(beta), eps, _p(xn), _p(mean), _p(rstd), _st())
    if rc == -2:
        return None
    _abi.check(rc, "favit_ln_gemm")
    if GEMM_TRACE is not None:
        e1.record()
        GEMM_TRACE.append((e0, e1, 2.0 * M * N * D, "bf16_KK_" + ("obf16" if out.dtype == torch.bfloat16 else "of32"),
                           (M, N, D, 1), "s64ln"))
    return xn, mean, rstd


_GROUPED_WS = {}
_GROUPED_WS_RETIRED = []


GROUP_MAX = 48


def gemm_grouped_tn(problems, use_workspace: bool = True) -> bool:
    if len(problems) > GROUP_MAX:
        T = problems[0][0].shape[0]
        if any(p[0].shape[0] != T or p[0].dtype != torch.bfloat16 or p[1].dtype != torch.bfloat16 for p in problems) or T % 32:
            return False
        for i in range(0, len(problems), GROUP_MAX):
            if not gemm_grouped_tn(problems[i:i + GROUP_MAX], use_workspace):
                raise RuntimeError("grouped weight-gradient launch declined a chunk after launching another")
        return True
    return _grouped_launch(problems, use_workspace, False)


def gemm_grouped_tn_ragged(problems, use_workspace: bool = True) -> bool:
    if len(problems) > GROUP_MAX:
        return False
    return _grouped_launch(problems, use_workspace, True)


def _grouped_launch(problems, use_workspace, ragged):
    n = len(problems)
    if n == 0:
        return True
    L = _abi.lib()
    f_query, f_ws, f_plain = ((L.favit_gemm_grouped_tn_ragged_workspace, L.favit_gemm_grouped_tn_ragged_ws,
                               L.favit_gemm_grouped_tn_ragged) if ragged else
                              (L.favit_gemm_grouped_tn_workspace, L.favit_gemm_grouped_tn_ws, L.favit_gemm_grouped_tn))
    arr = (GemmDesc * n)()
    T = problems[0][0].shape[0]
    for d, (dy, a, dw, db, acc) in zip(arr, problems):
        require_gpu(dy, a, dw)
        if dy.dtype != torch.bfloat16 or a.dtype != torch.bfloat16 or dw.dtype != torch.float32:
            return False
        if a.shape[0] != dy.shape[0] or (dy.shape[0] != T and not ragged):
            return False
        T_i = dy.shape[0]
        N, Kd = dy.shape[1], a.shape[1]
        d.A, d.B, d.C = dy.data_ptr(), a.data_ptr(), dw.data_ptr()
        d.a_rowsum = db.data_ptr() if db is not None else None
        d.M, d.N, d.K = N, Kd, T_i
        d.lda, d.ldb, d.ldc = dy.stride(0), a.stride(0), dw.stride(0)
        d.batch, d.batch_inner = 1, 1
        d.a_kmajor, d.b_kmajor = 0, 0
        d.in_dtype, d.out_dtype = BF16, F32
        d.act, d.accumulate, d.split_k = ACT_NONE, int(acc), 0
        d.alpha, d.dropout_p, d.dropout_seed = 1.0, 0.0, 0
    if GEMM_TRACE is not None:
        e0, e1 = torch.cuda.Event(enable_timing=True), torch.cuda.Event(enable_timing=True)
        e0.record()
    need = int(f_query(arr, n)) if use_workspace else 0
    if need > 0:
        dev = problems[0][0].device
        ws = _GROUPED_WS.get(dev.index)
        if ws is None or ws.numel() < need:
            if ws is not None:
                _GROUPED_WS_RETIRED.append(ws)
            ws = torch.empty(need, dtype=torch.uint8, device=dev)
            _GROUPED_WS[dev.index] = ws
        rc = f_ws(arr, n, _p(ws), ws.numel(), _st())
    else:
        rc = f_plain(arr, n, _st())
    if rc == -2:
        return False
    _abi.check(rc, "favit_gemm_grouped_tn")
    if GEMM_TRACE is not None:
        e1.record()
        fl = sum(2.0 * p[0].shape[0] * p[0].shape[1] * p[1].shape[1] for p in problems)
        GEMM_TRACE.append((e0, e1, fl, "bf16_MM_of32_grouped", (len(problems), int(_abi.lib().favit_gemm_grouped_last_splits())),
                           "grouped_tn"))
    return True


_FP8_DT = (torch.float8_e4m3fn, torch.float8_e5m2)


class Fp8History:
    __slots__ = ("slots", "scale_inv", "calls")

    NSLOT = 256

    def __init__(self, device):
        self.slots = torch.zeros(3 * self.NSLOT, dtype=torch.float32, device=device)
        self.scale_inv = torch.ones(1, dtype=torch.float32, device=device)
        self.calls = 0


def fp8_quantize(src: torch.Tensor, fmt: torch.dtype, *, want=True, want_t=False, colsum: Optional[torch.Tensor] = None,
                 hist: Optional[Fp8History] = None):
    require_gpu(src)
    if src.dim() != 2 or src.stride(1) != 1:
        raise ValueError("fp8_quantize expects a row-major 2-D matrix")
    rows, cols = src.shape
    dev = src.device
    L = _abi.lib()
    q = torch.empty((rows, cols), dtype=fmt, device=dev) if want else None
    ld_t = (rows + 63) // 64 * 64
    q_t = torch.empty((cols, ld_t), dtype=fmt, device=dev) if want_t else None
    f8 = _abi.E5M2 if fmt == torch.float8_e5m2 else _abi.E4M3
    if hist is None:
        st = torch.zeros(2, dtype=torch.float32, device=dev)
        _abi.check(L.favit_fp8_amax(_p(src), dt(src), rows, cols, src.stride(0), _p(st), _st()), "favit_fp8_amax")
        _abi.check(L.favit_fp8_quantize(_p(src), dt(src), rows, cols, src.stride(0), _p(q), cols, _p(q_t), ld_t, f8,
                                        _p(st), C.c_void_p(st.data_ptr() + 4), _p(colsum), None, None, _st()),
                   "favit_fp8_quantize")
        return q, q_t, st[1:2]
    base = hist.slots.data_ptr()
    stride = 4 * hist.NSLOT
    cur, nxt, clr = hist.calls % 3, (hist.calls + 1) % 3, (hist.calls + 2) % 3
    if hist.calls == 0:
        _abi.check(L.favit_fp8_amax(_p(src), dt(src), rows, cols, src.stride(0), C.c_void_p(base + stride * cur), _st()),
                   "favit_fp8_amax")
    hist.calls += 1
    sinv = torch.empty(1, dtype=torch.float32, device=dev)
    _abi.check(L.favit_fp8_quantize(_p(src), dt(src), rows, cols, src.stride(0), _p(q), cols, _p(q_t), ld_t, f8,
                                    C.c_void_p(base + stride * cur), _p(sinv), _p(colsum), C.c_void_p(base + stride * nxt),
                                    C.c_void_p(base + stride * clr), _st()), "favit_fp8_quantize")
    return q, q_t, sinv


def cast(src: torch.Tensor, dtype: torch.dtype, out: Optional[torch.Tensor] = None) -> torch.Tensor:
    require_gpu(src)
    src = src.contiguous()
    if out is None:
        out = torch.empty(src.shape, dtype=dtype, device=src.device)
    _abi.check(_abi.lib().favit_cast(_p(src), dt(src), _p(out), dt(out), src.numel(), _st()), "favit_cast")
    return out


def _q8_slots(hist: "Fp8History"):
    base, stride = hist.slots.data_ptr(), 4 * hist.NSLOT
    cur, nxt, clr = hist.calls % 3, (hist.calls + 1) % 3, (hist.calls + 2) % 3
    hist.calls += 1
    return C.c_void_p(base + stride * cur), C.c_void_p(base + stride * nxt), C.c_void_p(base + stride * clr)


def _q8_fused_ok(q8, out_dtype, D) -> bool:
    return q8 is not None and q8[1] is not None and q8[1].calls > 0 and out_dtype == torch.bfloat16 and D % 4 == 0


def layernorm_fwd(x, ldx, gamma, beta, rows, D, out_dtype, eps=1e-5, q8=None):
    require_gpu(x, gamma, beta)
    y = torch.empty((rows, D), dtype=out_dtype, device=x.device)
    mean = torch.empty(rows, dtype=torch.float32, device=x.device)
    rstd = torch.empty(rows, dtype=torch.float32, device=x.device)
    if _q8_fused_ok(q8, out_dtype, D):
        fmt, hist = q8
        q = torch.empty((rows, D), dtype=fmt, device=x.device)
        sinv = torch.empty(1, dtype=torch.float32, device=x.device)
        cur, nxt, clr = _q8_slots(hist)
        _abi.check(_abi.lib().favit_layernorm_fwd_q8(_p(x), ldx, _p(gamma), _p(beta), _p(y), _p(mean), _p(rstd), rows, D, eps,
                                                     _p(q), _abi.E5M2 if fmt == torch.float8_e5m2 else _abi.E4M3, cur,
                                                     _p(sinv), nxt, clr, _st()), "favit_layernorm_fwd_q8")
        y._favit_q8 = ((fmt, y._version), (q, None, sinv))
        return y, mean, rstd
    _abi.check(_abi.lib().favit_layernorm_fwd(_p(x), ldx, _p(gamma), _p(beta), _p(y), dt(y), _p(mean), _p(rstd),
                                              rows, D, eps, _st()), "favit_layernorm_fwd")
    return y, mean, rstd


SMALL_LINEAR_MAX_N = 64


def small_linear_fwd(x, w, bias):
    require_gpu(x, w)
    M, Kd = x.shape
    N = w.shape[0]
    y = torch.empty((M, N), dtype=torch.float32, device=x.device)
    _abi.check(_abi.lib().favit_small_linear_fwd(_p(x), x.stride(0), _p(w), _p(bias), _p(y), M, N, Kd, _st()),
               "favit_small_linear_fwd")
    return y


def small_linear_bwd(dy, x, w, *, want_dx=True, dw_out=None, db_out=None, want_db=True):
    require_gpu(dy, x, w)
    M, Kd = x.shape
    N = w.shape[0]
    dev = x.device
    dx = torch.empty((M, Kd), dtype=torch.float32, device=dev) if want_dx else None
    acc = dw_out is not None and (db_out is not None or not want_db)
    dw = dw_out if acc else torch.empty((N, Kd), dtype=torch.float32, device=dev)
    db = (db_out if acc else torch.empty(N, dtype=torch.float32, device=dev)) if want_db else None
    _abi.check(_abi.lib().favit_small_linear_bwd(_p(dy), _p(x), x.stride(0), _p(w), _p(dx), _p(dw), _p(db), int(acc), M, N, Kd,
                                                 _st()), "favit_small_linear_bwd")
    return dx, (None if acc else dw), (None if (acc or not want_db) else db)


def layernorm_bwd(dy, x, ldx, gamma, mean, rstd, rows, D, *, dres=None, dx=None, lddx=None, want_lp=False,
                  dg_out=None, db_out=None, lp_drop=(0.0, 0), defer=None, frozen=False, q8=None):
    require_gpu(dy, x)
    dev = x.device
    if dx is None:
        dx = torch.empty((rows, D), dtype=torch.float32, device=dev)
        lddx = D
    dx_lp = torch.empty((rows, D), dtype=dy.dtype, device=dev) if want_lp else None
    nparts = int(min(2048, (rows + 3) // 4))
    part = torch.empty((2, nparts, D), dtype=torch.float32, device=dev)
    acc = dg_out is not None and db_out is not None
    if frozen:
        acc, dg, db = True, None, None
    elif acc and defer is not None:
        defer.append((part, dg_out, db_out))
        dg = db = None
    elif acc:
        dg, db = dg_out, db_out
    else:
        dgb = torch.empty((2, D), dtype=torch.float32, device=dev)
        dg, db = dgb[0], dgb[1]
    if want_lp and _q8_fused_ok(q8, dy.dtype, D):
        fmt, hist = q8
        q = torch.empty((rows, D), dtype=fmt, device=dev)
        sinv = torch.empty(1, dtype=torch.float32, device=dev)
        cur, nxt, clr = _q8_slots(hist)
        _abi.check(_abi.lib().favit_layernorm_bwd_q8(_p(dy), _p(x), ldx, _p(gamma), _p(mean), _p(rstd), _p(dres), _p(dx), lddx,
                                                     _p(dx_lp), _p(part[0]), _p(part[1]), nparts, _p(dg), _p(db), int(acc), rows, D,
                                                     float(lp_drop[0]), int(lp_drop[1]) & ((1 << 64) - 1), _p(q),
                                                     _abi.E5M2 if fmt == torch.float8_e5m2 else _abi.E4M3, cur, _p(sinv), nxt, clr,
                                                     _st()), "favit_layernorm_bwd_q8")
        dx_lp._favit_q8 = ((fmt, dx_lp._version), (q, None, sinv))
        return (dx, dx_lp, None, None) if acc else (dx, dx_lp, dg, db)
    _abi.check(_abi.lib().favit_layernorm_bwd(_p(dy), dt(dy), _p(x), ldx, _p(gamma), _p(mean), _p(rstd), _p(dres),
                                              _p(dx), lddx, _p(dx_lp), dt(dy), _p(part[0]), _p(part[1]), nparts,
                                              _p(dg), _p(db), int(acc), rows, D, float(lp_drop[0]), int(lp_drop[1]) & ((1 << 64) - 1),
                                              _st()), "favit_layernorm_bwd")
    return (dx, dx_lp, None, None) if acc else (dx, dx_lp, dg, db)


def reduce_rows_multi(entries):
    if entries and any(tuple(e[0].shape) != tuple(entries[0][0].shape) for e in entries):
        return reduce_rows_multi_ragged(entries)
    for i in range(0, len(entries), 32):
        chunk = entries[i:i + 32]
        n = len(chunk)
        rows, cols = chunk[0][0].shape[1], chunk[0][0].shape[2]
        arr = C.c_void_p * n
        for part, o0, o1 in chunk:
            require_gpu(part, o0, o1)
            if tuple(part.shape) != (2, rows, cols) or not part.is_contiguous() or part.dtype != torch.float32:
                raise ValueError("reduce_rows_multi: every entry must be a contiguous fp32 [2, rows, cols] stack of one shape")
        _abi.check(_abi.lib().favit_reduce_rows_multi(n, arr(*[e[0].data_ptr() for e in chunk]),
                                                      arr(*[e[1].data_ptr() for e in chunk]),
                                                      arr(*[e[2].data_ptr() for e in chunk]), rows, cols, _st()),
                   "favit_reduce_rows_multi")


def reduce_rows_multi_ragged(entries):
    if not entries:
        return
    cols = entries[0][0].shape[-1]
    for part, o0, o1 in entries:
        require_gpu(part, o0, o1)
        if part.dim() != 3 or part.shape[0] != 2 or part.shape[2] != cols or not part.is_contiguous() or part.dtype != torch.float32:
            raise ValueError("reduce_rows_multi: every entry must be a contiguous fp32 [2, rows, cols] stack of one cols")
    for i in range(0, len(entries), 32):
        chunk = entries[i:i + 32]
        n = len(chunk)
        arr = C.c_void_p * n
        rows = (C.c_int64 * n)(*[e[0].shape[1] for e in chunk])
        _abi.check(_abi.lib().favit_reduce_rows_multi_ragged(n, arr(*[e[0].data_ptr() for e in chunk]),
                                                             arr(*[e[1].data_ptr() for e in chunk]),
                                                             arr(*[e[2].data_ptr() for e in chunk]), rows, cols, _st()),
                   "favit_reduce_rows_multi_ragged")


def reduce_rows(t2d: torch.Tensor) -> torch.Tensor:
    require_gpu(t2d)
    rows, cols = t2d.shape
    out = torch.empty(cols, dtype=torch.float32, device=t2d.device)
    _abi.check(_abi.lib().favit_reduce_rows(_p(t2d), t2d.stride(0), _p(out), rows, cols, 0, _st()), "favit_reduce_rows")
    return out


def mhla_fold_fwd(wqkv, bqkv, wl, bl, H, dtype):
    require_gpu(wqkv, bqkv, wl, bl)
    D = wqkv.shape[1]
    weff = torch.empty((3 * D, D), dtype=dtype, device=wqkv.device)
    beff = torch.empty(3 * D, dtype=torch.float32, device=wqkv.device)
    _abi.check(_abi.lib().favit_mhla_fold_fwd(_p(wqkv), _p(bqkv), _p(wl), _p(bl), _p(weff), dt(weff), None, _p(beff),
                                              D, H, _st()), "favit_mhla_fold_fwd")
    return weff, beff


def mhla_fold_fwd_multi(params, H, dtype):
    n = len(params)
    D = params[0][0].shape[1]
    dev = params[0][0].device
    for q in params:
        require_gpu(*q)
    weff = torch.empty((n, 3 * D, D), dtype=dtype, device=dev)
    beff = torch.empty((n, 3 * D), dtype=torch.float32, device=dev)
    arr = C.c_void_p * n
    cols = [arr(*[q[j].data_ptr() for q in params]) for j in range(4)]
    wp = arr(*[weff[i].data_ptr() for i in range(n)])
    bp = arr(*[beff[i].data_ptr() for i in range(n)])
    _abi.check(_abi.lib().favit_mhla_fold_fwd_multi(n, cols[0], cols[1], cols[2], cols[3], wp, dt(weff), bp, D, H, _st()),
               "favit_mhla_fold_fwd_multi")
    return [(weff[i], beff[i]) for i in range(n)]


def mhla_fold_bwd(dweff, dbeff, wqkv, bqkv, wl, H, out=None):
    D = wqkv.shape[1]
    hd = D // H
    dev = wqkv.device
    acc = out is not None
    if acc:
        dwqkv, dbqkv, dwl, dbl = out
    else:
        dwqkv = torch.empty((3 * D, D), dtype=torch.float32, device=dev)
        dbqkv = torch.empty(3 * D, dtype=torch.float32, device=dev)
        dwl = torch.empty((hd, hd), dtype=torch.float32, device=dev)
        dbl = torch.empty(hd, dtype=torch.float32, device=dev)
    _abi.check(_abi.lib().favit_mhla_fold_bwd(_p(dweff), _p(dbeff), _p(wqkv), _p(bqkv), _p(wl), _p(dwqkv), _p(dbqkv),
                                              _p(dwl), _p(dbl), D, H, int(acc), _st()), "favit_mhla_fold_bwd")
    return dwqkv, dbqkv, dwl, dbl


def mhla_fold_bwd_multi(entries, H):
    for i in range(0, len(entries), 16):
        chunk = entries[i:i + 16]
        n = len(chunk)
        D = chunk[0][2].shape[1]
        arr = C.c_void_p * n
        cols = []
        for j in range(5):
            cols.append(arr(*[e[j].data_ptr() for e in chunk]))
        for j in range(4):
            cols.append(arr(*[(e[5][j].data_ptr() if e[5][j] is not None else None) for e in chunk]))
        for e in chunk:
            require_gpu(*e[:5], *e[5])
        _abi.check(_abi.lib().favit_mhla_fold_bwd_multi(n, *cols, D, H, _st()), "favit_mhla_fold_bwd_multi")


def mhla_attn_lse_supported(L, hd, W, dtype) -> bool:
    code = {torch.float32: _abi.F32, torch.bfloat16: _abi.BF16}.get(dtype)
    return code is not None and bool(_abi.lib().favit_mhla_attn_lse_supported(L, hd, W, code))


def mhla_attn_fwd(qkv, B, L, H, hd, W, mask=None, p=0.0, seed=0, want_lse=False):
    require_gpu(qkv, mask)
    out = torch.empty((B * L, H * hd), dtype=qkv.dtype, device=qkv.device)
    if want_lse and mhla_attn_lse_supported(L, hd, W, qkv.dtype):
        lse = torch.empty((B, H, L), dtype=torch.float32, device=qkv.device)
        _abi.check(_abi.lib().favit_mhla_attn_fwd_lse(_p(qkv), _p(out), _p(lse), _p(mask), B, L, H, hd, W, dt(qkv), p,
                                                      seed, _st()), "favit_mhla_attn_fwd_lse")
        return out, lse
    _abi.check(_abi.lib().favit_mhla_attn_fwd(_p(qkv), _p(out), _p(mask), B, L, H, hd, W, dt(qkv), p, seed, _st()),
               "favit_mhla_attn_fwd")
    return (out, None) if want_lse else out


def mhla_attn_bwd(qkv, dout, B, L, H, hd, W, mask=None, p=0.0, seed=0, o=None, lse=None):
    require_gpu(qkv, dout, mask, o, lse)
    dqkv = torch.empty_like(qkv)
    if o is not None and lse is not None:
        _abi.check(_abi.lib().favit_mhla_attn_bwd_lse(_p(qkv), _p(dout), _p(o), _p(lse), _p(dqkv), _p(mask), B, L, H, hd,
                                                      W, dt(qkv), p, seed, _st()), "favit_mhla_attn_bwd_lse")
        return dqkv
    _abi.check(_abi.lib().favit_mhla_attn_bwd(_p(qkv), _p(dout), _p(dqkv), _p(mask), B, L, H, hd, W, dt(qkv), p, seed,
                                              _st()), "favit_mhla_attn_bwd")
    return dqkv


class BlockPlan:
    __slots__ = ("desc", "ref", "M", "D", "hidden", "B", "n", "H", "nparts", "tape_bytes", "off", "bwd_bytes", "boff")


def mhla_block_plan(B, n, D, H, W, hidden, training, eps=1e-5) -> Optional[BlockPlan]:
    d = _abi.BlockDesc()
    d.B, d.n, d.D, d.H, d.W, d.hidden, d.training, d.eps = B, n, D, H, W, hidden, int(bool(training)), eps
    lib = _abi.lib()
    to = (C.c_int64 * len(_abi.BLOCK_TAPE_SLOTS))()
    tape_bytes = lib.favit_mhla_block_tape_layout(C.byref(d), to)
    if tape_bytes < 0:
        return None
    p = BlockPlan()
    p.desc, p.ref, p.M, p.D, p.hidden, p.B, p.n, p.H = d, C.byref(d), B * n, D, hidden, B, n, H
    p.nparts = int(min(2048, (B * n + 3) // 4))
    p.tape_bytes = d.tape_bytes = tape_bytes
    ends = list(to[1:]) + [tape_bytes]
    p.off = {k: (to[i], ends[i] - to[i]) for i, k in enumerate(_abi.BLOCK_TAPE_SLOTS)}
    p.bwd_bytes, p.boff = [], []
    for want_lp in (0, 1):
        bo = (C.c_int64 * len(_abi.BLOCK_BWD_SLOTS))()
        nb = lib.favit_mhla_block_bwd_layout(C.byref(d), want_lp, bo)
        ends = list(bo[1:]) + [nb]
        p.bwd_bytes.append(nb)
        p.boff.append({k: (bo[i], ends[i] - bo[i]) for i, k in enumerate(_abi.BLOCK_BWD_SLOTS)})
    return p


def _block_code(code: int, what: str) -> int:
    if code == _abi.ERR_LAUNCH:
        _abi.check(code, what)
    return code


def mhla_block_fwd(plan: BlockPlan, x, tape, g1, b1, g2, b2, weff, beff, wproj, bproj, wfc1, bfc1, wfc2, bfc2) -> int:
    d = plan.desc
    d.x, d.tape, d.tape_bytes = x.data_ptr(), tape.data_ptr(), tape.numel()
    d.g1, d.b1, d.g2, d.b2 = g1.data_ptr(), b1.data_ptr(), g2.data_ptr(), b2.data_ptr()
    d.weff, d.beff, d.wproj, d.bproj = weff.data_ptr(), beff.data_ptr(), wproj.data_ptr(), bproj.data_ptr()
    d.wfc1, d.bfc1, d.wfc2, d.bfc2 = wfc1.data_ptr(), bfc1.data_ptr(), wfc2.data_ptr(), bfc2.data_ptr()
    return _block_code(_abi.lib().favit_mhla_block_fwd(plan.ref, _st()), "favit_mhla_block_fwd")


def mhla_block_bwd(plan: BlockPlan, x, tape, g1, g2, weff, wproj, wfc1, wfc2, g, g_lp, arena, want_lp_out: bool) -> int:
    d = plan.desc
    d.x, d.tape, d.tape_bytes = x.data_ptr(), tape.data_ptr(), tape.numel()
    d.g1, d.g2 = g1.data_ptr(), g2.data_ptr()
    d.weff, d.wproj, d.wfc1, d.wfc2 = weff.data_ptr(), wproj.data_ptr(), wfc1.data_ptr(), wfc2.data_ptr()
    return _block_code(_abi.lib().favit_mhla_block_bwd(plan.ref, g.data_ptr(), g_lp.data_ptr(), arena.data_ptr(),
                                                       arena.numel(), int(bool(want_lp_out)), _st()),
                       "favit_mhla_block_bwd")


def _sdpa_desc(q, k, v, o, lse, B, H, Lq, Lk, hd, scale, mask, m_sb, m_sq, p, seed):
    d = SdpaDesc()
    es = q.t.element_size()
    for name, vw in (("q", q), ("k", k), ("v", v), ("o", o)):
        setattr(d, name, vw.t.data_ptr() + vw.off * es)
        getattr(d, name + "_str")[:] = [vw.ld, vw.sb, vw.sh]
    d.lse = lse.data_ptr()
    d.mask = mask.data_ptr() if mask is not None else None
    d.m_sb, d.m_sq = m_sb, m_sq
    d.B, d.H, d.Lq, d.Lk, d.hd, d.dtype = B, H, Lq, Lk, hd, dt(q.t)
    d.scale, d.dropout_p, d.seed = scale, p, seed
    return d


def sdpa_fwd(q, k, v, o, B, H, Lq, Lk, hd, scale, mask=None, m_sb=0, m_sq=0, p=0.0, seed=0):
    require_gpu(q.t, k.t, v.t, o.t, mask)
    lse = torch.empty((B * H, Lq), dtype=torch.float32, device=q.t.device)
    d = _sdpa_desc(q, k, v, o, lse, B, H, Lq, Lk, hd, scale, mask, m_sb, m_sq, p, seed)
    _abi.check(_abi.lib().favit_sdpa_fwd(C.byref(d), _st()), "favit_sdpa_fwd")
    return lse


def sdpa_bwd(q, k, v, o, do, dq, dk, dv, lse, B, H, Lq, Lk, hd, scale, mask=None, m_sb=0, m_sq=0, p=0.0, seed=0):
    require_gpu(q.t, k.t, v.t, o.t, do.t, dq.t, dk.t, dv.t, lse, mask)
    delta = torch.empty((B * H, Lq), dtype=torch.float32, device=q.t.device)
    d = _sdpa_desc(q, k, v, o, lse, B, H, Lq, Lk, hd, scale, mask, m_sb, m_sq, p, seed)
    es = q.t.element_size()
    for name, vw in (("dout", do), ("dq", dq), ("dk", dk), ("dv", dv)):
        setattr(d, name, vw.t.data_ptr() + vw.off * es)
        getattr(d, ("do" if name == "dout" else name) + "_str")[:] = [vw.ld, vw.sb, vw.sh]
    d.delta = delta.data_ptr()
    _abi.check(_abi.lib().favit_sdpa_bwd(C.byref(d), _st()), "favit_sdpa_bwd")


def softmax_fwd(S, p_dtype, H, Z, Lq, Lk, mask=None, m_sb=0, m_sq=0, p=0.0, seed=0):
    require_gpu(S, mask)
    P = torch.empty((Z, Lq, Lk), dtype=p_dtype, device=S.device)
    Pd = torch.empty_like(P) if p > 0 else None
    _abi.check(_abi.lib().favit_softmax_fwd(_p(S), _p(P), _p(Pd), dt(P), _p(mask), m_sb, m_sq, H, Z, Lq, Lk, p, seed,
                                            _st()), "favit_softmax_fwd")
    return P, (Pd if Pd is not None else P)


def softmax_bwd(P, dPd, Z, Lq, Lk, p=0.0, seed=0):
    dS = torch.empty_like(P)
    _abi.check(_abi.lib().favit_softmax_bwd(_p(P), dt(P), _p(dPd), _p(dS), dt(dS), Z, Lq, Lk, p, seed, _st()),
               "favit_softmax_bwd")
    return dS


def patchify_fwd(img, P, dtype):
    require_gpu(img)
    B, Cc, HW, HW2 = img.shape
    if HW != HW2 or HW % P:
        raise ValueError("patchify needs square images with size divisible by patch_size")
    img = img.contiguous()
    g = HW // P
    out = torch.empty((B * g * g, P * P * Cc), dtype=dtype, device=img.device)
    _abi.check(_abi.lib().favit_patchify_fwd(_p(img), _p(out), dt(out), B, Cc, HW, P, _st()), "favit_patchify_fwd")
    return out


def patchify_bwd(dpatch, B, Cc, HW, P):
    dimg = torch.empty((B, Cc, HW, HW), dtype=torch.float32, device=dpatch.device)
    _abi.check(_abi.lib().favit_patchify_bwd(_p(dpatch), _p(dimg), B, Cc, HW, P, _st()), "favit_patchify_bwd")
    return dimg


def embed_prologue_fwd(tok, cls, pos, B, N, D):
    x = torch.empty((B, N + 1, D), dtype=torch.float32, device=tok.device)
    _abi.check(_abi.lib().favit_embed_prologue_fwd(_p(tok), _p(cls), _p(pos), _p(x), B, N, D, _st()),
               "favit_embed_prologue_fwd")
    return x


def embed_prologue_bwd(dx, B, N, D, tok_dtype, want_pos=True):
    dev = dx.device
    dtok = torch.empty((B * N, D), dtype=tok_dtype, device=dev)
    dcls = torch.empty(D, dtype=torch.float32, device=dev)
    dpos = torch.empty((N + 1, D), dtype=torch.float32, device=dev) if want_pos else None
    _abi.check(_abi.lib().favit_embed_prologue_bwd(_p(dx), _p(dtok), dt(dtok), _p(dcls), _p(dpos), B, N, D, _st()),
               "favit_embed_prologue_bwd")
    return dtok, dcls, dpos


def rows_cut_fwd(x, B, n_in, a, b, D):
    require_gpu(x)
    if x.dtype != torch.float32 or not x.is_contiguous() or x.numel() != B * n_in * D:
        raise ValueError("rows_cut_fwd expects a contiguous fp32 [B, n_in, D] tensor")
    y = torch.empty((B, a + b, D), dtype=torch.float32, device=x.device)
    _abi.check(_abi.lib().favit_rows_cut_fwd(_p(x), _p(y), B, n_in, a, b, D, _st()), "favit_rows_cut_fwd")
    return y


def rows_cut_bwd(dy, B, n_in, a, b, D, lp_dtype=None):
    require_gpu(dy)
    if dy.dtype != torch.float32 or not dy.is_contiguous() or dy.numel() != B * (a + b) * D:
        raise ValueError("rows_cut_bwd expects a contiguous fp32 [B, a + b, D] tensor")
    dx = torch.empty((B, n_in, D), dtype=torch.float32, device=dy.device)
    lp = torch.empty((B, n_in, D), dtype=lp_dtype, device=dy.device) if lp_dtype is not None else None
    _abi.check(_abi.lib().favit_rows_cut_bwd(_p(dy), _p(dx), _p(lp), dt(lp) if lp is not None else F32, B, n_in, a, b, D,
                                             _st()), "favit_rows_cut_bwd")
    return dx, lp


def dropout(x, p, seed):
    y = torch.empty_like(x)
    _abi.check(_abi.lib().favit_dropout(_p(x), _p(y), dt(x), x.numel(), p, seed, _st()), "favit_dropout")
    return y


def sppp_map_patches(seg, P):
    require_gpu(seg)
    if seg.dtype != torch.int64:
        seg = seg.to(torch.int64)
    seg = seg.contiguous()
    B, HW, _ = seg.shape
    N = (HW // P) ** 2
    dev = seg.device
    rank = torch.empty((B, N), dtype=torch.int32, device=dev)
    ntok = torch.empty(B, dtype=torch.int32, device=dev)
    perm = torch.empty((B, N), dtype=torch.int32, device=dev)
    offs = torch.empty((B, N + 1), dtype=torch.int32, device=dev)
    dom = torch.empty((B, N), dtype=torch.int64, device=dev)
    _abi.check(_abi.lib().favit_sppp_map_patches(_p(seg), _p(rank), _p(ntok), _p(perm), _p(offs), _p(dom), B, HW, P,
                                                 _st()), "favit_sppp_map_patches")
    return rank, ntok, perm, offs, dom


def sppp_pool_fwd(emb, perm, offs, kind, R):
    B, N, D = emb.shape
    out = torch.empty((B, R, D), dtype=torch.float32, device=emb.device)
    argmax = torch.empty((B, R, D), dtype=torch.int32, device=emb.device) if kind == 1 else None
    _abi.check(_abi.lib().favit_sppp_pool_fwd(_p(emb), _p(perm), _p(offs), _p(out), _p(argmax), kind, B, N, R, D,
                                              _st()), "favit_sppp_pool_fwd")
    return out, argmax


def sppp_pool_bwd(dout, emb, perm, offs, argmax, kind, R):
    B, N, D = emb.shape
    demb = torch.zeros_like(emb)
    _abi.check(_abi.lib().favit_sppp_pool_bwd(_p(dout), _p(emb), None, _p(perm), _p(offs), _p(argmax), _p(demb), kind,
                                              B, N, R, D, _st()), "favit_sppp_pool_bwd")
    return demb


def sppp_centroids(seg, S):
    require_gpu(seg)
    seg = seg.to(torch.int64).contiguous()
    B, HW, _ = seg.shape
    cent = torch.empty((B, S, 2), dtype=torch.float32, device=seg.device)
    _abi.check(_abi.lib().favit_sppp_centroids(_p(seg), _p(cent), B, HW, S, _st()), "favit_sppp_centroids")
    return cent


def sppp_posenc_fwd(x, cent):
    B, L, D = x.shape
    y = torch.empty_like(x)
    _abi.check(_abi.lib().favit_sppp_posenc_fwd(_p(x), _p(cent), _p(y), B, L, D, 0 if cent is None else cent.shape[1], _st()),
               "favit_sppp_posenc_fwd")
    return y


def slic_grid(H, W, n_segments):
    import math
    if H * W <= n_segments:
        return list(range(H)), list(range(W)), 1
    s = math.sqrt(H * W / float(n_segments))
    sy = sx = s
    if min(H, W) < s:
        if H <= W:
            sy, sx = float(H), (W / float(n_segments))
        else:
            sx, sy = float(W), (H / float(n_segments))
    ys = list(range(int(sy // 2), H, max(1, int(round(sy)))))
    xs = list(range(int(sx // 2), W, max(1, int(round(sx)))))
    return ys, xs, max(max(1, int(round(sy))), max(1, int(round(sx))))


def slic(images, n_segments=16, compactness=0.1, sigma=1.0, max_num_iter=10, min_size_factor=0.5, stages=False,
         rescale=True):
    require_gpu(images)
    if images.dim() != 4 or images.shape[1] != 3 or images.dtype != torch.float32:
        raise TypeError("slic expects fp32 images [B, 3, H, W]")
    images = images.contiguous()
    B, _, H, W = images.shape
    ys, xs, step = slic_grid(H, W, n_segments)
    if len(ys) * len(xs) > 64:
        raise ValueError("slic: at most 64 seed centres are supported")
    dev = images.device
    init = torch.tensor([[y, x] for y in ys for x in xs], dtype=torch.int32, device=dev)
    Kc = init.shape[0]
    coef = int(round((step / float(compactness)) ** 2))
    min_size = int(min_size_factor * (H * W / float(Kc)))
    feat = torch.empty((B, H * W, 4), dtype=torch.int16, device=dev)
    lab = torch.empty((B, H * W), dtype=torch.uint8, device=dev)
    ws = torch.empty((2, B, H * W), dtype=torch.int32, device=dev)
    out = torch.empty((B, H, W), dtype=torch.int64, device=dev)
    nreg = torch.empty(B, dtype=torch.int32, device=dev)
    L = _abi.lib()
    fws = torch.empty(int(L.favit_slic_features_workspace(B, H, W)) // 4, dtype=torch.float32, device=dev)
    _abi.check(L.favit_slic_features(_p(images), _p(feat), B, H, W, float(sigma), int(bool(rescale)), _p(fws), _st()),
               "favit_slic_features")
    cws = torch.empty(int(L.favit_slic_cluster_workspace(Kc, B)) // 8 + 1, dtype=torch.int64, device=dev)
    _abi.check(L.favit_slic_cluster(_p(feat), _p(lab), _p(init), Kc, B, H, W, step, coef, max_num_iter, _p(cws), _st()),
               "favit_slic_cluster")
    _abi.check(L.favit_slic_connect(_p(lab), _p(ws[0]), _p(ws[1]), _p(out), _p(nreg), B, H, W, min_size, _st()),
               "favit_slic_connect")
    return (out, feat, lab.view(B, H, W), nreg) if stages else out


def slic_stage_times(images, n_segments=16, compactness=0.1, sigma=1.0, max_num_iter=10, min_size_factor=0.5, reps=5):
    out = []
    import functools
    B, _, H, W = images.shape
    ys, xs, step = slic_grid(H, W, n_segments)
    dev = images.device
    init = torch.tensor([[y, x] for y in ys for x in xs], dtype=torch.int32, device=dev)
    Kc = init.shape[0]
    coef = int(round((step / float(compactness)) ** 2))
    min_size = int(min_size_factor * (H * W / float(Kc)))
    feat = torch.empty((B, H * W, 4), dtype=torch.int16, device=dev)
    lab = torch.empty((B, H * W), dtype=torch.uint8, device=dev)
    ws = torch.empty((2, B, H * W), dtype=torch.int32, device=dev)
    o = torch.empty((B, H, W), dtype=torch.int64, device=dev)
    nreg = torch.empty(B, dtype=torch.int32, device=dev)
    L = _abi.lib()
    cws = torch.empty(int(L.favit_slic_cluster_workspace(Kc, B)) // 8 + 1, dtype=torch.int64, device=dev)
    fws = torch.empty(int(L.favit_slic_features_workspace(B, H, W)) // 4, dtype=torch.float32, device=dev)
    stages = [
        ("features", lambda: L.favit_slic_features(_p(images), _p(feat), B, H, W, float(sigma), 1, _p(fws), _st())),
        ("cluster", lambda: L.favit_slic_cluster(_p(feat), _p(lab), _p(init), Kc, B, H, W, step, coef, max_num_iter, _p(cws), _st())),
        ("connect", lambda: L.favit_slic_connect(_p(lab), _p(ws[0]), _p(ws[1]), _p(o), _p(nreg), B, H, W, min_size, _st())),
    ]
    for name, fn in stages:
        fn()
        torch.cuda.synchronize()
        e0, e1 = torch.cuda.Event(enable_timing=True), torch.cuda.Event(enable_timing=True)
        e0.record()
        for _ in range(reps):
            fn()
        e1.record()
        torch.cuda.synchronize()
        out.append((name, e0.elapsed_time(e1) / reps))
    return out


def batch_mix(x, lam, box):
    require_gpu(x, lam, box)
    if x.dim() != 4 or x.dtype != torch.float32 or not x.is_contiguous():
        raise TypeError("batch_mix: x must be a contiguous fp32 [B, C, H, W] tensor")
    B, Cn, H, W = x.shape
    if lam.dtype != torch.float32 or tuple(lam.shape) != (B,) or not lam.is_contiguous():
        raise TypeError("batch_mix: lam must be a contiguous fp32 [B] tensor")
    if box.dtype != torch.int32 or tuple(box.shape) != (B, 4) or not box.is_contiguous():
        raise TypeError("batch_mix: box must be a contiguous int32 [B, 4] tensor of (y0, y1, x0, x1)")
    _abi.check(_abi.lib().favit_batch_mix(_p(x), _p(lam), _p(box), B, Cn, H, W, _st()), "favit_batch_mix")
    return x


def _erase_fill(value, channels):
    n = max(int(channels), 3)
    if isinstance(value, str):
        if value != "normal":
            raise ValueError(f"erase value {value!r}: a number, a per-channel sequence or 'normal'")
        return (C.c_float * n)(), 1
    v = [float(value)] * n if np.ndim(value) == 0 else [float(t) for t in value]
    if len(v) < channels or not all(math.isfinite(t) for t in v):
        raise ValueError(f"erase value {value!r}: one finite number, or one per channel ({channels})")
    v = (v + [v[-1]] * n)[:n]
    return (C.c_float * n)(*v), 0


def randaugment(src_u8, ops, mean, std, erase_box=None, erase_value=0.0, erase_seed=0, want_bytes=False):
    require_gpu(src_u8, ops)
    if src_u8.dtype != torch.uint8 or src_u8.dim() != 4 or src_u8.shape[1] != src_u8.shape[2] or not src_u8.is_contiguous():
        raise TypeError("randaugment: src_u8 must be a contiguous uint8 [B, S, S, C] tensor")
    B, S, _, Cn = src_u8.shape
    if ops.dtype != torch.int32 or ops.dim() != 3 or ops.shape[0] != B or ops.shape[2] != 8 or not ops.is_contiguous():
        raise TypeError(f"randaugment: ops must be a contiguous int32 [{B}, n_ops, 8] tensor")
    fill, normal = (None, 0)
    if erase_box is not None:
        require_gpu(erase_box)
        if erase_box.dtype != torch.int32 or tuple(erase_box.shape) != (B, 4) or not erase_box.is_contiguous():
            raise TypeError(f"randaugment: erase_box must be a contiguous int32 [{B}, 4] tensor of (y0, y1, x0, x1)")
        fill, normal = _erase_fill(erase_value, Cn)
    dev = src_u8.device
    scratch = torch.empty((2, B, S, S, Cn), dtype=torch.uint8, device=dev)
    out = torch.empty((B, Cn, S, S), dtype=torch.float32, device=dev)
    u8 = torch.empty((B, S, S, Cn), dtype=torch.uint8, device=dev) if want_bytes else None
    _abi.check(_abi.lib().favit_randaugment(_p(src_u8), _p(scratch), _p(out), _p(u8), _p(ops), int(ops.shape[1]),
                                            _p(erase_box), fill, normal, int(erase_seed) & 0xFFFFFFFFFFFFFFFF, B, S, Cn,
                                            mean, std, _st()), "favit_randaugment")
    return (out, u8) if want_bytes else out


def random_erase(x, box, value=0.0, seed=0):
    require_gpu(x, box)
    if x.dim() != 4 or x.dtype != torch.float32 or not x.is_contiguous():
        raise TypeError("random_erase: x must be a contiguous fp32 [B, C, H, W] tensor")
    B, Cn, H, W = x.shape
    if box.dtype != torch.int32 or tuple(box.shape) != (B, 4) or not box.is_contiguous():
        raise TypeError(f"random_erase: box must be a contiguous int32 [{B}, 4] tensor of (y0, y1, x0, x1)")
    fill, normal = _erase_fill(value, Cn)
    _abi.check(_abi.lib().favit_random_erase(_p(x), _p(box), fill, normal, int(seed) & 0xFFFFFFFFFFFFFFFF, B, Cn, H, W,
                                             _st()), "favit_random_erase")
    return x


def cross_entropy(logits, labels, grad_scale=None, label_smoothing=0.0, mix_lam=None):
    if not 0.0 <= label_smoothing < 1.0:
        raise ValueError(f"cross_entropy: label_smoothing must be in [0, 1), got {label_smoothing}")
    require_gpu(logits, labels)
    if logits.dim() != 2 or logits.dtype != torch.float32 or not logits.is_contiguous():
        raise TypeError("cross_entropy: logits must be a contiguous fp32 [B, C] tensor")
    B, Cn = logits.shape
    if labels.dtype != torch.int64 or tuple(labels.shape) != (B,) or not labels.is_contiguous():
        raise TypeError("cross_entropy: labels must be a contiguous int64 [B] tensor of class indices "
                        "(out-of-range labels, e.g. ignore_index = -100, give a NaN loss row)")
    loss_rows = torch.empty(B, dtype=torch.float32, device=logits.device)
    dlog = torch.empty_like(logits) if grad_scale is not None else None
    gs = 0.0 if grad_scale is None else grad_scale
    if mix_lam is not None:
        require_gpu(mix_lam)
        if mix_lam.dtype != torch.float32 or tuple(mix_lam.shape) != (B,) or not mix_lam.is_contiguous():
            raise TypeError("cross_entropy: mix_lam must be a contiguous fp32 [B] tensor")
        _abi.check(_abi.lib().favit_cross_entropy_mix(_p(logits), _p(labels), _p(mix_lam), _p(loss_rows), _p(dlog), B,
                                                      Cn, gs, float(label_smoothing), _st()),
                   "favit_cross_entropy_mix")
    elif label_smoothing:
        _abi.check(_abi.lib().favit_cross_entropy_ls(_p(logits), _p(labels), _p(loss_rows), _p(dlog), B, Cn, gs,
                                                     float(label_smoothing), _st()), "favit_cross_entropy_ls")
    else:
        _abi.check(_abi.lib().favit_cross_entropy(_p(logits), _p(labels), _p(loss_rows), _p(dlog), B, Cn, gs, _st()),
                   "favit_cross_entropy")
    return loss_rows, dlog


GRAD_NORM_MAX_BUFS = 16


def grad_norm_workspace(device) -> torch.Tensor:
    return torch.empty(int(_abi.lib().favit_grad_norm_workspace()) // 8, dtype=torch.float64, device=device)


def grad_norm(bufs, scale=1.0, max_norm=0.0, out=None, skipped=None, ws=None):
    bufs = list(bufs)
    n = len(bufs)
    if n > GRAD_NORM_MAX_BUFS:
        raise ValueError(f"grad_norm: at most {GRAD_NORM_MAX_BUFS} buffers per call, got {n}")
    if not n and out is None:
        raise ValueError("grad_norm: no buffer and no `out` to take the device from")
    require_gpu(*bufs, out, skipped, ws)
    for t in bufs:
        if t.dtype != torch.float32 or (t.numel() and not t.is_contiguous()):
            raise TypeError("grad_norm: every buffer must be a contiguous fp32 tensor")
    dev = bufs[0].device if n else out.device
    if out is None:
        out = torch.empty(2, dtype=torch.float32, device=dev)
    elif out.dtype != torch.float32 or out.numel() != 2 or not out.is_contiguous():
        raise TypeError("grad_norm: out must be two contiguous fp32")
    if skipped is not None and (skipped.dtype != torch.int32 or skipped.numel() != 1):
        raise TypeError("grad_norm: skipped must be one int32")
    if ws is None:
        ws = grad_norm_workspace(dev)
    ptrs = (C.c_void_p * max(1, n))(*[t.data_ptr() if t.numel() else None for t in bufs])
    lens = (C.c_int64 * max(1, n))(*[t.numel() for t in bufs])
    _abi.check(_abi.lib().favit_grad_norm(n, ptrs, lens, float(scale), float(max_norm), _p(out), _p(skipped), _p(ws),
                                          ws.numel() * ws.element_size(), _st()), "favit_grad_norm")
    return out


def adamw(p, g, m, v, lr, beta1, beta2, eps, wd, step, grad_scale=1.0, p_lp=None, coef=None, skip_nonfinite=False,
          ema=None, ema_decay=0.0):
    bc1 = 1.0 - beta1 ** step
    bc2 = 1.0 - beta2 ** step
    if ema is not None:
        require_gpu(ema)
        if ema.dtype != torch.float32 or ema.numel() != p.numel() or (ema.numel() and not ema.is_contiguous()):
            raise TypeError("adamw: ema must be a contiguous fp32 tensor of p's length")
        if not 0.0 <= float(ema_decay) <= 1.0:
            raise ValueError(f"adamw: ema_decay must be in [0, 1], got {ema_decay}")
    if coef is None:
        if skip_nonfinite:
            raise ValueError("adamw: skip_nonfinite needs the device coefficient of grad_norm (coef)")
        if ema is not None:
            _abi.check(_abi.lib().favit_adamw_ema(_p(p), _p(g), _p(m), _p(v), _p(p_lp), _p(ema), p.numel(), lr, beta1,
                                                  beta2, eps, wd, bc1, bc2, grad_scale, float(ema_decay), _st()),
                       "favit_adamw_ema")
            return
        _abi.check(_abi.lib().favit_adamw(_p(p), _p(g), _p(m), _p(v), _p(p_lp), p.numel(), lr, beta1, beta2, eps, wd,
                                          bc1, bc2, grad_scale, _st()), "favit_adamw")
        return
    require_gpu(coef)
    if coef.dtype != torch.float32 or coef.numel() != 1:
        raise TypeError("adamw: coef must be one fp32 on the device")
    if ema is not None:
        _abi.check(_abi.lib().favit_adamw_clip_ema(_p(p), _p(g), _p(m), _p(v), _p(p_lp), _p(ema), p.numel(), lr, beta1,
                                                   beta2, eps, wd, bc1, bc2, grad_scale, _p(coef),
                                                   int(bool(skip_nonfinite)), float(ema_decay), _st()),
                   "favit_adamw_clip_ema")
        return
    _abi.check(_abi.lib().favit_adamw_clip(_p(p), _p(g), _p(m), _p(v), _p(p_lp), p.numel(), lr, beta1, beta2, eps, wd,
                                           bc1, bc2, grad_scale, _p(coef), int(bool(skip_nonfinite)), _st()),
               "favit_adamw_clip")


def swap_params(a, b, a_lp=None):
    require_gpu(a, b, a_lp)
    for t in (a, b):
        if t.dtype != torch.float32 or (t.numel() and not t.is_contiguous()):
            raise TypeError("swap_params: a and b must be contiguous fp32 tensors")
    if a.numel() != b.numel() or (a_lp is not None and (a_lp.dtype != torch.bfloat16 or a_lp.numel() != a.numel()
                                                         or (a_lp.numel() and not a_lp.is_contiguous()))):
        raise TypeError("swap_params: b (fp32) and a_lp (bf16, optional) must have a's length")
    _abi.check(_abi.lib().favit_swap_params(_p(a), _p(b), _p(a_lp), a.numel(), _st()), "favit_swap_params")
```

### focused-attention-vit_amd/models/vit.py

```python
import torch
import torch.nn as nn

from ._backend import F, params


class PatchRearrange(nn.Module):

    def __init__(self, patch_size):
        super().__init__()
        self.patch_size = patch_size

    def extra_repr(self):
        return f"'b c (h p1) (w p2) -> b (h w) (p1 p2 c)', p1=p2={self.patch_size}"

    def forward(self, x):
        raise RuntimeError("PatchRearrange is fused into PatchEmbedding.forward")


class PatchEmbedding(nn.Module):

    def __init__(self, img_size=224, patch_size=16, in_channels=3, embed_dim=768):
        super().__init__()
        self.img_size = img_size
        self.patch_size = patch_size
        self.num_patches = (img_size // patch_size) ** 2
        self.projection = nn.Sequential(
            PatchRearrange(patch_size),
            nn.Linear(patch_size * patch_size * in_channels, embed_dim),
        )

    def forward(self, x):
        lin = self.projection[1]
        return F.run(F.PatchEmbedOp(self.patch_size), [x], [lin.weight, lin.bias])


class MultiHeadAttention(nn.Module):

    def __init__(self, embed_dim, num_heads, dropout=0.0):
        super().__init__()
        self.embed_dim = embed_dim
        self.num_heads = num_heads
        self.head_dim = embed_dim // num_heads
        assert self.head_dim * num_heads == embed_dim, "embed_dim must be divisible by num_heads"
        self.qkv = nn.Linear(embed_dim, embed_dim * 3)
        self.attn_dropout = nn.Dropout(dropout)
        self.proj = nn.Linear(embed_dim, embed_dim)
        self.proj_dropout = nn.Dropout(dropout)

    def _chain(self):
        return F.DenseChain(self.num_heads, self.attn_dropout.p, self.proj_dropout.p)

    def forward(self, x):
        ch = self._chain()
        return F.run(F.AttnOp(ch, None, self.training), [x], params(self, ch.names))


class MLP(nn.Module):

    def __init__(self, in_features, hidden_features, out_features, dropout=0.0):
        super().__init__()
        self.fc1 = nn.Linear(in_features, hidden_features)
        self.act = nn.GELU()
        self.fc2 = nn.Linear(hidden_features, out_features)
        self.dropout = nn.Dropout(dropout)

    def _chain(self):
        return F.MLPChain(self.dropout.p)

    def forward(self, x):
        ch = self._chain()
        return F.run(F.MLPOp(ch, self.training), [x], params(self, ch.names))


class TransformerBlock(nn.Module):

    def __init__(self, embed_dim, num_heads, mlp_ratio=4.0, dropout=0.0, attn_dropout=0.0):
        super().__init__()
        self.norm1 = nn.LayerNorm(embed_dim)
        self.attn = MultiHeadAttention(embed_dim, num_heads, attn_dropout)
        self.norm2 = nn.LayerNorm(embed_dim)
        self.mlp = MLP(in_features=embed_dim, hidden_features=int(embed_dim * mlp_ratio), out_features=embed_dim,
                       dropout=dropout)

    def _spec(self):
        return F.BlockSpec(self.attn._chain(), self.mlp._chain())

    def forward(self, x):
        spec = self._spec()
        return F.run(F.EncoderOp([spec], None, self.training), [x], params(self, spec.names))


def run_encoder(blocks, x, mask, training, cls_only=False):
    blocks = list(blocks)
    nseg = max(1, min(F.get_encoder_segments(), len(blocks)))
    m = F._mask_u8(mask)
    per = (len(blocks) + nseg - 1) // nseg
    all_specs = [b._spec() for b in blocks]
    cuts = F.cls_only_cuts(all_specs, x.shape[1], m, training) if cls_only else None
    for i in range(0, len(blocks), per):
        grp = blocks[i:i + per]
        specs = all_specs[i:i + per]
        prm = []
        for b, s in zip(grp, specs):
            prm += params(b, s.names)
        if i:
            x = F.note_segment_boundary(x)
        x = F.run(F.EncoderOp(specs, m, training, cuts=None if cuts is None else cuts[i:i + per]), [x], prm)
    return x


def embed_dropout(x, p, training):
    if not training or p <= 0.0:
        return x
    return F.run(F.DropoutOp(p), [x], [])


class VisionTransformer(nn.Module):

    def __init__(self, img_size=224, patch_size=4, in_channels=3, num_classes=1000, embed_dim=768, depth=12,
                 num_heads=12, mlp_ratio=4.0, dropout=0.0, attn_dropout=0.0, embed_dropout=0.0):
        super().__init__()
        self.img_size = img_size
        self.patch_size = patch_size
        self.in_channels = in_channels
        self.num_classes = num_classes
        self.embed_dim = embed_dim
        self.depth = depth
        self.num_heads = num_heads
        self.patch_embed = PatchEmbedding(img_size=img_size, patch_size=patch_size, in_channels=in_channels,
                                          embed_dim=embed_dim)
        num_patches = self.patch_embed.num_patches
        self.cls_token = nn.Parameter(torch.zeros(1, 1, embed_dim))
        self.pos_embed = nn.Parameter(torch.zeros(1, num_patches + 1, embed_dim))
        self.pos_drop = nn.Dropout(embed_dropout)
        self.blocks = nn.ModuleList([
            TransformerBlock(embed_dim=embed_dim, num_heads=num_heads, mlp_ratio=mlp_ratio, dropout=dropout,
                             attn_dropout=attn_dropout) for _ in range(depth)])
        self.norm = nn.LayerNorm(embed_dim)
        self.head = nn.Linear(embed_dim, num_classes)
        self._init_weights()

    def _init_weights(self):
        nn.init.normal_(self.cls_token, std=0.02)
        nn.init.normal_(self.pos_embed, std=0.02)
        self.apply(self._init_weights_recursive)

    def _init_weights_recursive(self, m):
        if isinstance(m, nn.Linear):
            nn.init.normal_(m.weight, std=0.02)
            if m.bias is not None:
                nn.init.zeros_(m.bias)
        elif isinstance(m, nn.LayerNorm):
            nn.init.ones_(m.weight)
            nn.init.zeros_(m.bias)

    def forward_features(self, x):
        tok = self.patch_embed(x)
        x = F.run(F.PrologueOp(True), [tok], [self.cls_token, self.pos_embed])
        x = embed_dropout(x, self.pos_drop.p, self.training)
        x = run_encoder(self.blocks, x, None, self.training)
        return F.run(F.FinalNormOp(), [x], [self.norm.weight, self.norm.bias])

    def forward(self, x):
        x = self.forward_features(x)
        return F.run(F.LinearOp(), [x], [self.head.weight, self.head.bias])

    def get_num_parameters(self):
        return sum(p.numel() for p in self.parameters() if p.requires_grad)
```

### include/favit.h

```cpp
#ifndef FAVIT_H_
#define FAVIT_H_

#include <stdint.h>

#ifdef __cplusplus
extern "C" {
#endif

#define FAVIT_ABI_VERSION 8
#define FAVIT_FP8_AMAX_SLOTS 256

enum { FAVIT_F32 = 0, FAVIT_BF16 = 1, FAVIT_FP8 = 2, FAVIT_F32X3 = 3 };
enum { FAVIT_E4M3 = 0, FAVIT_E5M2 = 1 };

enum {
  FAVIT_OK = 0,
  FAVIT_ERR_INVALID = -1,
  FAVIT_ERR_UNSUPPORTED = -2,
  FAVIT_ERR_ALIGN = -3,
  FAVIT_ERR_LAUNCH = -4
};

enum {
  FAVIT_ACT_NONE = 0,
  FAVIT_ACT_GELU = 1,
  FAVIT_ACT_DGELU = 2,
  FAVIT_ACT_GELU_SAVEGRAD = 3,
  FAVIT_ACT_MULAUX = 4
};
enum { FAVIT_POOL_MEAN = 0, FAVIT_POOL_MAX = 1, FAVIT_POOL_ATTENTION = 2 };

int favit_abi_version(void);
const char* favit_strerror(int code);

int favit_set_dropout_epoch(const uint64_t* device_word);

int favit_set_health_word(uint32_t* device_words);

typedef struct favit_gemm_t {
  const void* A;
  const void* B;
  void* C;
  const float* bias;
  const void* aux_in;
  void* aux_out;
  const float* residual;
  float* a_rowsum;
  int64_t M, N, K;
  int64_t lda, ldb, ldc, ld_aux_in, ld_aux_out, ld_res;
  int64_t sAo, sAi, sBo, sBi, sCo, sCi;
  int32_t batch, batch_inner;
  int32_t a_kmajor, b_kmajor;
  int32_t in_dtype, out_dtype;
  int32_t act;
  int32_t accumulate;
  int32_t split_k;
  float alpha;
  float dropout_p;
  int32_t fp8_fmt;
  uint64_t dropout_seed;
  const float* scale_a;
  const float* scale_b;
} favit_gemm_t;

int favit_gemm(const favit_gemm_t* g, void* stream);
const char* favit_gemm_last_kernel(void);

int favit_ln_gemm(const favit_gemm_t* g, const float* x, int64_t ldx, const float* gamma, const float* beta, float eps,
                  void* xn, float* mean, float* rstd, void* stream);

int favit_gemm_grouped_tn(const favit_gemm_t* gs, int32_t count, void* stream);
int64_t favit_gemm_grouped_tn_workspace(const favit_gemm_t* gs, int32_t count);
int favit_gemm_grouped_tn_ws(const favit_gemm_t* gs, int32_t count, void* workspace, int64_t workspace_bytes,
                             void* stream);
int favit_gemm_grouped_tn_ragged(const favit_gemm_t* gs, int32_t count, void* stream);
int64_t favit_gemm_grouped_tn_ragged_workspace(const favit_gemm_t* gs, int32_t count);
int favit_gemm_grouped_tn_ragged_ws(const favit_gemm_t* gs, int32_t count, void* workspace, int64_t workspace_bytes,
                                    void* stream);
int favit_gemm_grouped_last_splits(void);
int favit_gemm_grouped_plan(const favit_gemm_t* gs, int32_t count, int32_t ragged, int64_t* out, int32_t cap);

int favit_fp8_amax(const void* src, int src_dtype, int64_t rows, int64_t cols, int64_t ld_src, float* amax,
                   void* stream);
int favit_fp8_quantize(const void* src, int src_dtype, int64_t rows, int64_t cols, int64_t ld_src, void* dst,
                       int64_t ld_dst, void* dst_t, int64_t ld_t, int fmt, const float* amax, float* scale_inv,
                       float* colsum, float* amax_next, float* amax_clear, void* stream);

int favit_cast(const void* src, int src_dtype, void* dst, int dst_dtype, int64_t n, void* stream);

int favit_layernorm_fwd(const float* x, int64_t ldx, const float* gamma, const float* beta, void* y, int y_dtype,
                        float* mean, float* rstd, int64_t rows, int32_t D, float eps, void* stream);
int favit_layernorm_bwd(const void* dy, int dy_dtype, const float* x, int64_t ldx, const float* gamma,
                        const float* mean, const float* rstd, const float* dres, float* dx, int64_t lddx,
                        void* dx_lp, int lp_dtype, float* dgamma_part, float* dbeta_part, int32_t nparts,
                        float* dgamma, float* dbeta, int32_t accumulate, int64_t rows, int32_t D,
                        float lp_dropout_p, uint64_t lp_dropout_seed, void* stream);
int favit_layernorm_fwd_q8(const float* x, int64_t ldx, const float* gamma, const float* beta, void* y, float* mean,
                           float* rstd, int64_t rows, int32_t D, float eps, void* q, int fmt, const float* amax,
                           float* scale_inv, float* amax_next, float* amax_clear, void* stream);
int favit_layernorm_bwd_q8(const void* dy, const float* x, int64_t ldx, const float* gamma, const float* mean,
                           const float* rstd, const float* dres, float* dx, int64_t lddx, void* dx_lp,
                           float* dgamma_part, float* dbeta_part, int32_t nparts, float* dgamma, float* dbeta,
                           int32_t accumulate, int64_t rows, int32_t D, float lp_dropout_p, uint64_t lp_dropout_seed,
                           void* q, int fmt, const float* amax, float* scale_inv, float* amax_next, float* amax_clear,
                           void* stream);
int favit_small_linear_fwd(const float* x, int64_t ldx, const float* w, const float* bias, float* y, int32_t M, int32_t N,
                           int32_t K, void* stream);
int favit_small_linear_bwd(const float* dy, const float* x, int64_t ldx, const float* w, float* dx, float* dw, float* db,
                           int32_t accumulate, int32_t M, int32_t N, int32_t K, void* stream);
int favit_reduce_rows(const float* in, int64_t ld, float* out, int64_t rows, int32_t cols, int32_t accumulate,
                      void* stream);
int favit_reduce_rows_multi(int32_t n, const float* const* in, float* const* out0, float* const* out1, int64_t rows,
                            int32_t cols, void* stream);
int favit_reduce_rows_multi_ragged(int32_t n, const float* const* in, float* const* out0, float* const* out1,
                                   const int64_t* rows, int32_t cols, void* stream);

int favit_mhla_fold_fwd(const float* wqkv, const float* bqkv, const float* wl, const float* bl, void* weff,
                        int weff_dtype, float* weff_f32 , float* beff, int32_t D,
                        int32_t H, void* stream);
int favit_mhla_fold_fwd_multi(int32_t n, const float* const* wqkv, const float* const* bqkv, const float* const* wl,
                              const float* const* bl, void* const* weff, int weff_dtype, float* const* beff,
                              int32_t D, int32_t H, void* stream);

int favit_mhla_fold_bwd(const float* dweff, const float* dbeff, const float* wqkv, const float* bqkv,
                        const float* wl, float* dwqkv, float* dbqkv, float* dwl, float* dbl, int32_t D, int32_t H,
                        int32_t accumulate, void* stream);
int favit_mhla_fold_bwd_multi(int32_t n, const float* const* dweff, const float* const* dbeff, const float* const* wqkv,
                              const float* const* bqkv, const float* const* wl, float* const* dwqkv,
                              float* const* dbqkv, float* const* dwl, float* const* dbl, int32_t D, int32_t H,
                              void* stream);

int favit_mhla_attn_fwd(const void* qkv, void* out, const uint8_t* mask, int32_t B, int32_t L, int32_t H,
                        int32_t hd, int32_t W, int dtype, float dropout_p, uint64_t seed, void* stream);
int favit_mhla_attn_bwd(const void* qkv, const void* dout, void* dqkv, const uint8_t* mask, int32_t B, int32_t L,
                        int32_t H, int32_t hd, int32_t W, int dtype, float dropout_p, uint64_t seed,
                        void* stream);
int favit_mhla_attn_lse_supported(int32_t L, int32_t hd, int32_t W, int dtype);
int favit_mhla_attn_fwd_lse(const void* qkv, void* out, float* lse, const uint8_t* mask, int32_t B, int32_t L, int32_t H,
                            int32_t hd, int32_t W, int dtype, float dropout_p, uint64_t seed, void* stream);
int favit_mhla_attn_bwd_lse(const void* qkv, const void* dout, const void* o, const float* lse, void* dqkv,
                            const uint8_t* mask, int32_t B, int32_t L, int32_t H, int32_t hd, int32_t W, int dtype,
                            float dropout_p, uint64_t seed, void* stream);

int favit_softmax_fwd(const float* S, void* P, void* Pd, int p_dtype, const uint8_t* mask, int64_t m_sb,
                      int64_t m_sq, int32_t H, int64_t Z, int32_t Lq, int32_t Lk, float dropout_p, uint64_t seed,
                      void* stream);
int favit_softmax_bwd(const void* P, int p_dtype, const float* dPd, void* dS, int ds_dtype, int64_t Z, int32_t Lq,
                      int32_t Lk, float dropout_p, uint64_t seed, void* stream);

int favit_image_transform(const uint8_t* src, uint8_t* tmp, float* out, uint8_t* out_u8, const int32_t* params, int32_t B,
                          int32_t Hs, int32_t Ws, int32_t C, int32_t ch_max, int32_t S, const float* mean,
                          const float* std, void* stream);
int favit_image_transform_ragged(const uint8_t* src, const int64_t* src_desc, uint8_t* tmp, float* out,
                                 uint8_t* out_u8, const int32_t* params, int32_t B, int32_t C, int32_t ch_max,
                                 int32_t S, const float* mean, const float* std, void* stream);

int64_t favit_slic_features_workspace(int32_t B, int32_t H, int32_t W);
int favit_slic_features(const float* img, int16_t* feat, int32_t B, int32_t H, int32_t W, float sigma, int32_t rescale,
                        float* ws, void* stream);
int64_t favit_slic_cluster_workspace(int32_t K, int32_t B);
int favit_slic_cluster(const int16_t* feat, uint8_t* labels, const int32_t* init_yx, int32_t K, int32_t B, int32_t H,
                       int32_t W, int32_t step, int64_t coef, int32_t iters, void* ws, void* stream);
int favit_slic_connect(const uint8_t* labels, int32_t* ws_comp, int32_t* ws_aux, int64_t* out, int32_t* n_regions,
                       int32_t B, int32_t H, int32_t W, int32_t min_size, void* stream);

typedef struct favit_sdpa {
  const void* q;
  const void* k;
  const void* v;
  void* o;
  float* lse;
  const void* dout;
  void* dq;
  void* dk;
  void* dv;
  float* delta;
  const uint8_t* mask;
  int64_t m_sb, m_sq;
  int64_t q_str[3], k_str[3], v_str[3], o_str[3], do_str[3], dq_str[3], dk_str[3], dv_str[3];
  int32_t B, H, Lq, Lk, hd, dtype;
  float scale, dropout_p;
  uint64_t seed;
} favit_sdpa_t;
int favit_sdpa_fwd(const favit_sdpa_t* s, void* stream);
int favit_sdpa_bwd(const favit_sdpa_t* s, void* stream);

int favit_patchify_fwd(const float* img, void* out, int out_dtype, int32_t B, int32_t C, int32_t HW, int32_t P,
                       void* stream);
int favit_patchify_bwd(const float* dpatch, float* dimg, int32_t B, int32_t C, int32_t HW, int32_t P, void* stream);
int favit_embed_prologue_fwd(const float* tok, const float* cls, const float* pos, float* x, int32_t B, int32_t N,
                             int32_t D, void* stream);
int favit_embed_prologue_bwd(const float* dx, void* dtok, int dtok_dtype, float* dcls, float* dpos, int32_t B,
                             int32_t N, int32_t D, void* stream);

int favit_rows_cut_fwd(const float* x, float* y, int32_t B, int32_t n_in, int32_t a, int32_t b, int32_t D, void* stream);
int favit_rows_cut_bwd(const float* dy, float* dx, void* dx_lp, int lp_dtype, int32_t B, int32_t n_in, int32_t a,
                       int32_t b, int32_t D, void* stream);

#define FAVIT_BLOCK_TAPE_SLOTS 13
#define FAVIT_BLOCK_BWD_SLOTS 11
typedef struct favit_mhla_block {
  const float* x;
  void* tape;
  const float* g1;
  const float* b1;
  const float* g2;
  const float* b2;
  const void* weff;
  const float* beff;
  const void* wproj;
  const float* bproj;
  const void* wfc1;
  const float* bfc1;
  const void* wfc2;
  const float* bfc2;
  int64_t tape_bytes;
  int32_t B, n, D, H, W, hidden;
  int32_t training;
  float eps;
} favit_mhla_block_t;
int64_t favit_mhla_block_tape_layout(const favit_mhla_block_t* desc, int64_t* offsets_out );
int64_t favit_mhla_block_bwd_layout(const favit_mhla_block_t* desc, int32_t want_lp_out,
                                    int64_t* offsets_out );
int favit_mhla_block_fwd(const favit_mhla_block_t* desc, void* stream);
int favit_mhla_block_bwd(const favit_mhla_block_t* desc, const float* g_f32, const void* g_lp, void* bwd_buffers,
                         int64_t bwd_bytes, int32_t want_lp_out, void* stream);

int favit_dropout(const void* x, void* y, int dtype, int64_t n, float p, uint64_t seed, void* stream);

int favit_sppp_map_patches(const int64_t* seg, int32_t* patch_rank, int32_t* n_tokens, int32_t* perm,
                           int32_t* offs, int64_t* dom_ws, int32_t B, int32_t HW, int32_t P, void* stream);
int favit_sppp_pool_fwd(const float* emb, const int32_t* perm, const int32_t* offs, float* out, int32_t* argmax,
                        int32_t kind, int32_t B, int32_t N, int32_t R, int32_t D, void* stream);
int favit_sppp_pool_bwd(const float* dout, const float* emb, const int32_t* patch_rank, const int32_t* perm,
                        const int32_t* offs, const int32_t* argmax, float* demb, int32_t kind, int32_t B,
                        int32_t N, int32_t R, int32_t D, void* stream);
int favit_sppp_centroids(const int64_t* seg, float* cent, int32_t B, int32_t HW, int32_t S, void* stream);
int favit_sppp_posenc_fwd(const float* x, const float* cent, float* y, int32_t B, int32_t L, int32_t D,
                          int32_t n_cent, void* stream);

int favit_cross_entropy(const float* logits, const int64_t* labels, float* loss_rows, float* dlogits, int32_t B,
                        int32_t C, float grad_scale, void* stream);
int favit_adamw(float* p, const float* g, float* m, float* v, void* p_bf16, int64_t n, float lr, float beta1,
                float beta2, float eps, float weight_decay, float bias_c1, float bias_c2, float grad_scale,
                void* stream);

int favit_cross_entropy_ls(const float* logits, const int64_t* labels, float* loss_rows, float* dlogits, int32_t B,
                           int32_t C, float grad_scale, float label_smoothing, void* stream);

int64_t favit_grad_norm_workspace(void);
int favit_grad_norm(int32_t n, const float* const* bufs, const int64_t* lens, float scale, float max_norm,
                    float* out, uint32_t* skipped, void* ws, int64_t ws_bytes, void* stream);

int favit_adamw_clip(float* p, const float* g, float* m, float* v, void* p_bf16, int64_t n, float lr, float beta1,
                     float beta2, float eps, float weight_decay, float bias_c1, float bias_c2, float grad_scale,
                     const float* coef, int32_t skip_nonfinite, void* stream);

int favit_adamw_ema(float* p, const float* g, float* m, float* v, void* p_bf16, float* ema, int64_t n, float lr,
                    float beta1, float beta2, float eps, float weight_decay, float bias_c1, float bias_c2,
                    float grad_scale, float ema_decay, void* stream);
int favit_adamw_clip_ema(float* p, const float* g, float* m, float* v, void* p_bf16, float* ema, int64_t n, float lr,
                         float beta1, float beta2, float eps, float weight_decay, float bias_c1, float bias_c2,
                         float grad_scale, const float* coef, int32_t skip_nonfinite, float ema_decay, void* stream);

int favit_swap_params(float* a, float* b, void* a_bf16, int64_t n, void* stream);

int favit_batch_mix(float* x, const float* lam, const int32_t* box, int32_t B, int32_t C, int32_t H, int32_t W,
                    void* stream);
int favit_cross_entropy_mix(const float* logits, const int64_t* labels, const float* lam, float* loss_rows,
                            float* dlogits, int32_t B, int32_t C, float grad_scale, float label_smoothing,
                            void* stream);

int favit_randaugment_max_ops(void);
int favit_randaugment(const uint8_t* src_u8, uint8_t* scratch, float* out, uint8_t* out_u8, const int32_t* ops,
                      int32_t n_ops, const int32_t* erase_box, const float* erase_value, int32_t erase_normal,
                      uint64_t erase_seed, int32_t B, int32_t S, int32_t C, const float* mean, const float* std,
                      void* stream);
int favit_random_erase(float* x, const int32_t* box, const float* value, int32_t normal, uint64_t seed, int32_t B,
                       int32_t C, int32_t H, int32_t W, void* stream);

#ifdef __cplusplus
}
#endif
#endif
```

Before: 55160 images/sec.

## Split encoder block into attention and MLP halves, run MLP on retained rows only

Splits the fused MHLA block into separate attention and MLP forward/backward entry points so the MLP (LN2, fc1, fc2) can run on a compacted subset of token rows (n_mlp) when the following layer cuts tokens. The tape and backward buffers are sized by the reduced row count, which avoids MLP compute and memory on rows that are dropped afterwards. It also adds a cheaper raw-stream lookup for launches. This only takes effect when token cuts are present and narrow-MLP mode is enabled, and it adds extra compaction and bookkeeping.

```diff
diff --git a/focused-attention-vit_amd/_abi.py b/focused-attention-vit_amd/_abi.py
--- a/focused-attention-vit_amd/_abi.py
+++ b/focused-attention-vit_amd/_abi.py
@@ -50,6 +50,10 @@
         ("tape_bytes", i64),
         ("B", i32), ("n", i32), ("D", i32), ("H", i32), ("W", i32), ("hidden", i32), ("training", i32), ("eps", f32),
     ]
+
+
+class BlockMlp(C.Structure):
+    _fields_ = [("x1c", vp), ("n_mlp", i32), ("reserved", i32)]
 
 
 BLOCK_TAPE_SLOTS = ("xn1", "mu1", "rs1", "qkv", "o", "lse", "x1", "xn2", "mu2", "rs2", "h", "pre", "x2")
@@ -108,6 +112,12 @@
     "favit_mhla_block_bwd_layout": ([C.POINTER(BlockDesc), i32, C.POINTER(i64)], C.c_int64),
     "favit_mhla_block_fwd": ([C.POINTER(BlockDesc), vp], C.c_int),
     "favit_mhla_block_bwd": ([C.POINTER(BlockDesc), vp, vp, vp, i64, i32, vp], C.c_int),
+    "favit_mhla_block_tape_layout2": ([C.POINTER(BlockDesc), C.POINTER(BlockMlp), C.POINTER(i64)], C.c_int64),
+    "favit_mhla_block_bwd_layout2": ([C.POINTER(BlockDesc), C.POINTER(BlockMlp), i32, C.POINTER(i64)], C.c_int64),
+    "favit_mhla_block_attn_fwd": ([C.POINTER(BlockDesc), C.POINTER(BlockMlp), vp], C.c_int),
+    "favit_mhla_block_mlp_fwd": ([C.POINTER(BlockDesc), C.POINTER(BlockMlp), vp], C.c_int),
+    "favit_mhla_block_mlp_bwd": ([C.POINTER(BlockDesc), C.POINTER(BlockMlp), vp, vp, vp, i64, i32, vp], C.c_int),
+    "favit_mhla_block_attn_bwd": ([C.POINTER(BlockDesc), C.POINTER(BlockMlp), vp, vp, vp, i64, i32, vp], C.c_int),
     "favit_dropout": ([vp, vp, C.c_int, i64, f32, u64, vp], C.c_int),
     "favit_sppp_map_patches": ([vp, vp, vp, vp, vp, vp, i32, i32, i32, vp], C.c_int),
     "favit_sppp_pool_fwd": ([vp, vp, vp, vp, vp, i32, i32, i32, i32, i32, vp], C.c_int),
diff --git a/focused-attention-vit_amd/csrc/block.hip b/focused-attention-vit_amd/csrc/block.hip
--- a/focused-attention-vit_amd/csrc/block.hip
+++ b/focused-attention-vit_amd/csrc/block.hip
@@ -30,27 +30,32 @@
   return off;
 }
 
-void tape_sizes(const favit_mhla_block_t* d, int64_t* s) {
-  const int64_t M = (int64_t)d->B * d->n, D = d->D, Hd = d->hidden;
+int check_rows(const favit_mhla_block_t* d, const favit_mhla_block_mlp_t* r) {
+  if (!r) return FAVIT_ERR_INVALID;
+  if (r->n_mlp <= 0 || r->n_mlp > d->n) return FAVIT_ERR_INVALID;
+  return FAVIT_OK;
+}
+
+void tape_sizes(const favit_mhla_block_t* d, int32_t n_mlp, int64_t* s) {
+  const int64_t M = (int64_t)d->B * d->n, Mm = (int64_t)d->B * n_mlp, D = d->D, Hd = d->hidden;
   s[T_XN1] = M * D * 2; s[T_MU1] = M * 4; s[T_RS1] = M * 4;
   s[T_QKV] = M * 3 * D * 2; s[T_O] = M * D * 2;
   s[T_LSE] = d->training ? (int64_t)d->B * d->H * d->n * 4 : 0;
   s[T_X1] = M * D * 4;
-  s[T_XN2] = M * D * 2; s[T_MU2] = M * 4; s[T_RS2] = M * 4;
-  s[T_H] = M * Hd * 2; s[T_PRE] = M * Hd * 2;
-  s[T_X2] = M * D * 4;
+  s[T_XN2] = Mm * D * 2; s[T_MU2] = Mm * 4; s[T_RS2] = Mm * 4;
+  s[T_H] = Mm * Hd * 2; s[T_PRE] = Mm * Hd * 2;
+  s[T_X2] = Mm * D * 4;
 }
 
 int32_t ln_parts(int64_t rows) { return (int32_t)((rows + 3) / 4 < 2048 ? (rows + 3) / 4 : 2048); }
 
-void bwd_sizes(const favit_mhla_block_t* d, int want_lp_out, int64_t* s) {
-  const int64_t M = (int64_t)d->B * d->n, D = d->D, Hd = d->hidden;
-  const int64_t part = 2 * (int64_t)ln_parts(M) * D * 4;
-  s[G_DPRE] = M * Hd * 2; s[G_DXN2] = M * D * 2;
-  s[G_G1_F32] = M * D * 4; s[G_G1_LP] = M * D * 2;
+void bwd_sizes(const favit_mhla_block_t* d, int32_t n_mlp, int want_lp_out, int64_t* s) {
+  const int64_t M = (int64_t)d->B * d->n, Mm = (int64_t)d->B * n_mlp, D = d->D, Hd = d->hidden;
+  s[G_DPRE] = Mm * Hd * 2; s[G_DXN2] = Mm * D * 2;
+  s[G_G1_F32] = Mm * D * 4; s[G_G1_LP] = n_mlp == d->n ? M * D * 2 : 0;
   s[G_DO] = M * D * 2; s[G_DQKV] = M * 3 * D * 2; s[G_DXN1] = M * D * 2;
   s[G_OUT_F32] = M * D * 4; s[G_OUT_LP] = want_lp_out ? M * D * 2 : 0;
-  s[G_PART1] = part; s[G_PART2] = part;
+  s[G_PART1] = 2 * (int64_t)ln_parts(M) * D * 4; s[G_PART2] = 2 * (int64_t)ln_parts(Mm) * D * 4;
 }
 
 favit_gemm_t gemm_base(const void* A, const void* B, void* C, int64_t M, int64_t N, int64_t K, int64_t ldb, int b_kmajor,
@@ -75,35 +80,12 @@
   if (((uintptr_t)d->tape % ALIGN) != 0 || ((uintptr_t)d->x % 16) != 0) return FAVIT_ERR_ALIGN;
   return FAVIT_OK;
 }
-}
-
-extern "C" int64_t favit_mhla_block_tape_layout(const favit_mhla_block_t* desc, int64_t* offsets_out) {
-  const int rc = check_geometry(desc);
-  if (rc != FAVIT_OK) return rc;
-  int64_t s[TAPE_N];
-  tape_sizes(desc, s);
-  return layout(s, TAPE_N, offsets_out);
-}
-
-extern "C" int64_t favit_mhla_block_bwd_layout(const favit_mhla_block_t* desc, int32_t want_lp_out, int64_t* offsets_out) {
-  const int rc = check_geometry(desc);
-  if (rc != FAVIT_OK) return rc;
-  int64_t s[BWD_N];
-  bwd_sizes(desc, want_lp_out, s);
-  return layout(s, BWD_N, offsets_out);
-}
-
-extern "C" int favit_mhla_block_fwd(const favit_mhla_block_t* d, void* stream) {
-  int rc = check_geometry(d);
-  if (rc != FAVIT_OK) return rc;
-  if ((rc = check_params(d)) != FAVIT_OK) return rc;
-  int64_t s[TAPE_N], o[TAPE_N];
-  tape_sizes(d, s);
-  if (d->tape_bytes < layout(s, TAPE_N, o)) return FAVIT_ERR_INVALID;
+
+int attn_half_fwd(const favit_mhla_block_t* d, const int64_t* o, void* stream) {
+  int rc;
   char* t = reinterpret_cast<char*>(d->tape);
   const int64_t M = (int64_t)d->B * d->n;
-  const int32_t D = d->D, Hd = d->hidden;
-  float* x1 = reinterpret_cast<float*>(t + o[T_X1]);
+  const int32_t D = d->D;
   if ((rc = favit_layernorm_fwd(d->x, D, d->g1, d->b1, t + o[T_XN1], FAVIT_BF16, reinterpret_cast<float*>(t + o[T_MU1]),
                                 reinterpret_cast<float*>(t + o[T_RS1]), M, D, d->eps, stream)) != FAVIT_OK)
     return rc;
@@ -116,55 +98,55 @@
                    : favit_mhla_attn_fwd(t + o[T_QKV], t + o[T_O], nullptr, d->B, d->n, d->H, 64, d->W, FAVIT_BF16, 0.f, 0,
                                          stream);
   if (rc != FAVIT_OK) return rc;
-  g = gemm_base(t + o[T_O], d->wproj, x1, M, D, D, D, 1, FAVIT_F32);
+  g = gemm_base(t + o[T_O], d->wproj, t + o[T_X1], M, D, D, D, 1, FAVIT_F32);
   g.bias = d->bproj; g.residual = d->x;
   g.ld_aux_out = D; g.ld_res = D;
-  if ((rc = favit_gemm(&g, stream)) != FAVIT_OK) return rc;
+  return favit_gemm(&g, stream);
+}
+
+int mlp_half_fwd(const favit_mhla_block_t* d, const float* x1, int64_t Mm, const int64_t* o, void* stream) {
+  int rc;
+  char* t = reinterpret_cast<char*>(d->tape);
+  const int32_t D = d->D, Hd = d->hidden;
   if ((rc = favit_layernorm_fwd(x1, D, d->g2, d->b2, t + o[T_XN2], FAVIT_BF16, reinterpret_cast<float*>(t + o[T_MU2]),
-                                reinterpret_cast<float*>(t + o[T_RS2]), M, D, d->eps, stream)) != FAVIT_OK)
+                                reinterpret_cast<float*>(t + o[T_RS2]), Mm, D, d->eps, stream)) != FAVIT_OK)
     return rc;
-  g = gemm_base(t + o[T_XN2], d->wfc1, t + o[T_H], M, Hd, D, D, 1, FAVIT_BF16);
+  favit_gemm_t g = gemm_base(t + o[T_XN2], d->wfc1, t + o[T_H], Mm, Hd, D, D, 1, FAVIT_BF16);
   g.bias = d->bfc1; g.act = FAVIT_ACT_GELU_SAVEGRAD; g.aux_out = t + o[T_PRE];
   g.ld_aux_out = Hd; g.ld_res = Hd;
   if ((rc = favit_gemm(&g, stream)) != FAVIT_OK) return rc;
-  g = gemm_base(t + o[T_H], d->wfc2, t + o[T_X2], M, D, Hd, Hd, 1, FAVIT_F32);
+  g = gemm_base(t + o[T_H], d->wfc2, t + o[T_X2], Mm, D, Hd, Hd, 1, FAVIT_F32);
   g.bias = d->bfc2; g.residual = x1;
   g.ld_aux_out = D; g.ld_res = D;
   return favit_gemm(&g, stream);
 }
 
-extern "C" int favit_mhla_block_bwd(const favit_mhla_block_t* d, const float* g_f32, const void* g_lp, void* bwd_buffers,
-                                    int64_t bwd_bytes, int32_t want_lp_out, void* stream) {
-  int rc = check_geometry(d);
-  if (rc != FAVIT_OK) return rc;
-  if ((rc = check_params(d)) != FAVIT_OK) return rc;
-  if (!d->training || !g_f32 || !g_lp || !bwd_buffers) return FAVIT_ERR_INVALID;
-  if (((uintptr_t)bwd_buffers % ALIGN) != 0 || ((uintptr_t)g_f32 % 16) != 0 || ((uintptr_t)g_lp % 16) != 0)
-    return FAVIT_ERR_ALIGN;
-  int64_t s[TAPE_N], o[TAPE_N], bs[BWD_N], b[BWD_N];
-  tape_sizes(d, s);
-  if (d->tape_bytes < layout(s, TAPE_N, o)) return FAVIT_ERR_INVALID;
-  bwd_sizes(d, want_lp_out, bs);
-  if (bwd_bytes < layout(bs, BWD_N, b)) return FAVIT_ERR_INVALID;
-  char* t = reinterpret_cast<char*>(d->tape);
-  char* w = reinterpret_cast<char*>(bwd_buffers);
+int mlp_half_bwd(const favit_mhla_block_t* d, const float* x1, int64_t Mm, const float* g_f32, const void* g_lp,
+                 const int64_t* o, char* w, const int64_t* b, void* g1_lp, void* stream) {
+  int rc;
+  char* t = reinterpret_cast<char*>(d->tape);
+  const int32_t D = d->D, Hd = d->hidden, np = ln_parts(Mm);
+  float* part2 = reinterpret_cast<float*>(w + b[G_PART2]);
+  favit_gemm_t g = gemm_base(g_lp, d->wfc2, w + b[G_DPRE], Mm, Hd, D, Hd, 0, FAVIT_BF16);
+  g.act = FAVIT_ACT_MULAUX; g.aux_in = t + o[T_PRE]; g.ld_aux_in = Hd;
+  if ((rc = favit_gemm(&g, stream)) != FAVIT_OK) return rc;
+  g = gemm_base(w + b[G_DPRE], d->wfc1, w + b[G_DXN2], Mm, D, Hd, D, 0, FAVIT_BF16);
+  g.ld_aux_in = D;
+  if ((rc = favit_gemm(&g, stream)) != FAVIT_OK) return rc;
+  return favit_layernorm_bwd(w + b[G_DXN2], FAVIT_BF16, x1, D, d->g2, reinterpret_cast<const float*>(t + o[T_MU2]),
+                             reinterpret_cast<const float*>(t + o[T_RS2]), g_f32, reinterpret_cast<float*>(w + b[G_G1_F32]),
+                             D, g1_lp, FAVIT_BF16, part2, part2 + (int64_t)np * D, np, nullptr, nullptr, 1, Mm, D, 0.f, 0,
+                             stream);
+}
+
+int attn_half_bwd(const favit_mhla_block_t* d, const float* g1, const void* g1_lp, const int64_t* o, char* w,
+                  const int64_t* b, int want_lp_out, void* stream) {
+  int rc;
+  char* t = reinterpret_cast<char*>(d->tape);
   const int64_t M = (int64_t)d->B * d->n;
-  const int32_t D = d->D, Hd = d->hidden, np = ln_parts(M);
-  float* g1 = reinterpret_cast<float*>(w + b[G_G1_F32]);
+  const int32_t D = d->D, np = ln_parts(M);
   float* part1 = reinterpret_cast<float*>(w + b[G_PART1]);
-  float* part2 = reinterpret_cast<float*>(w + b[G_PART2]);
-  favit_gemm_t g = gemm_base(g_lp, d->wfc2, w + b[G_DPRE], M, Hd, D, Hd, 0, FAVIT_BF16);
-  g.act = FAVIT_ACT_MULAUX; g.aux_in = t + o[T_PRE]; g.ld_aux_in = Hd;
-  if ((rc = favit_gemm(&g, stream)) != FAVIT_OK) return rc;
-  g = gemm_base(w + b[G_DPRE], d->wfc1, w + b[G_DXN2], M, D, Hd, D, 0, FAVIT_BF16);
-  g.ld_aux_in = D;
-  if ((rc = favit_gemm(&g, stream)) != FAVIT_OK) return rc;
-  if ((rc = favit_layernorm_bwd(w + b[G_DXN2], FAVIT_BF16, reinterpret_cast<const float*>(t + o[T_X1]), D, d->g2,
-                                reinterpret_cast<const float*>(t + o[T_MU2]), reinterpret_cast<const float*>(t + o[T_RS2]),
-                                g_f32, g1, D, w + b[G_G1_LP], FAVIT_BF16, part2, part2 + (int64_t)np * D, np, nullptr,
-                                nullptr, 1, M, D, 0.f, 0, stream)) != FAVIT_OK)
-    return rc;
-  g = gemm_base(w + b[G_G1_LP], d->wproj, w + b[G_DO], M, D, D, D, 0, FAVIT_BF16);
+  favit_gemm_t g = gemm_base(g1_lp, d->wproj, w + b[G_DO], M, D, D, D, 0, FAVIT_BF16);
   g.ld_aux_in = D;
   if ((rc = favit_gemm(&g, stream)) != FAVIT_OK) return rc;
   if ((rc = favit_mhla_attn_bwd_lse(t + o[T_QKV], w + b[G_DO], t + o[T_O], reinterpret_cast<const float*>(t + o[T_LSE]),
@@ -179,3 +161,134 @@
                              want_lp_out ? w + b[G_OUT_LP] : nullptr, FAVIT_BF16, part1, part1 + (int64_t)np * D, np, nullptr,
                              nullptr, 1, M, D, 0.f, 0, stream);
 }
+
+int check_call(const favit_mhla_block_t* d, int32_t n_mlp, int64_t* o) {
+  int rc = check_params(d);
+  if (rc != FAVIT_OK) return rc;
+  int64_t s[TAPE_N];
+  tape_sizes(d, n_mlp, s);
+  return d->tape_bytes < layout(s, TAPE_N, o) ? FAVIT_ERR_INVALID : FAVIT_OK;
+}
+
+int check_bwd_call(const favit_mhla_block_t* d, int32_t n_mlp, const float* g_f32, const void* g_lp, void* bwd_buffers,
+                   int64_t bwd_bytes, int32_t want_lp_out, int64_t* o, int64_t* b) {
+  int rc = check_params(d);
+  if (rc != FAVIT_OK) return rc;
+  if (!d->training || !g_f32 || !g_lp || !bwd_buffers) return FAVIT_ERR_INVALID;
+  if (((uintptr_t)bwd_buffers % ALIGN) != 0 || ((uintptr_t)g_f32 % 16) != 0 || ((uintptr_t)g_lp % 16) != 0)
+    return FAVIT_ERR_ALIGN;
+  int64_t s[TAPE_N], bs[BWD_N];
+  tape_sizes(d, n_mlp, s);
+  if (d->tape_bytes < layout(s, TAPE_N, o)) return FAVIT_ERR_INVALID;
+  bwd_sizes(d, n_mlp, want_lp_out, bs);
+  if (bwd_bytes < layout(bs, BWD_N, b)) return FAVIT_ERR_INVALID;
+  return FAVIT_OK;
+}
+
+int check_x1c(const favit_mhla_block_mlp_t* r) {
+  if (!r->x1c) return FAVIT_ERR_INVALID;
+  return ((uintptr_t)r->x1c % 16) != 0 ? FAVIT_ERR_ALIGN : FAVIT_OK;
+}
+}
+
+extern "C" int64_t favit_mhla_block_tape_layout(const favit_mhla_block_t* desc, int64_t* offsets_out) {
+  const int rc = check_geometry(desc);
+  if (rc != FAVIT_OK) return rc;
+  int64_t s[TAPE_N];
+  tape_sizes(desc, desc->n, s);
+  return layout(s, TAPE_N, offsets_out);
+}
+
+extern "C" int64_t favit_mhla_block_bwd_layout(const favit_mhla_block_t* desc, int32_t want_lp_out, int64_t* offsets_out) {
+  const int rc = check_geometry(desc);
+  if (rc != FAVIT_OK) return rc;
+  int64_t s[BWD_N];
+  bwd_sizes(desc, desc->n, want_lp_out, s);
+  return layout(s, BWD_N, offsets_out);
+}
+
+extern "C" int favit_mhla_block_fwd(const favit_mhla_block_t* d, void* stream) {
+  int rc = check_geometry(d);
+  if (rc != FAVIT_OK) return rc;
+  int64_t o[TAPE_N];
+  if ((rc = check_call(d, d->n, o)) != FAVIT_OK) return rc;
+  if ((rc = attn_half_fwd(d, o, stream)) != FAVIT_OK) return rc;
+  return mlp_half_fwd(d, reinterpret_cast<const float*>(reinterpret_cast<char*>(d->tape) + o[T_X1]), (int64_t)d->B * d->n, o,
+                      stream);
+}
+
+extern "C" int favit_mhla_block_bwd(const favit_mhla_block_t* d, const float* g_f32, const void* g_lp, void* bwd_buffers,
+                                    int64_t bwd_bytes, int32_t want_lp_out, void* stream) {
+  int rc = check_geometry(d);
+  if (rc != FAVIT_OK) return rc;
+  int64_t o[TAPE_N], b[BWD_N];
+  if ((rc = check_bwd_call(d, d->n, g_f32, g_lp, bwd_buffers, bwd_bytes, want_lp_out, o, b)) != FAVIT_OK) return rc;
+  char* w = reinterpret_cast<char*>(bwd_buffers);
+  const float* x1 = reinterpret_cast<const float*>(reinterpret_cast<char*>(d->tape) + o[T_X1]);
+  if ((rc = mlp_half_bwd(d, x1, (int64_t)d->B * d->n, g_f32, g_lp, o, w, b, w + b[G_G1_LP], stream)) != FAVIT_OK) return rc;
+  return attn_half_bwd(d, reinterpret_cast<const float*>(w + b[G_G1_F32]), w + b[G_G1_LP], o, w, b, want_lp_out, stream);
+}
+
+extern "C" int64_t favit_mhla_block_tape_layout2(const favit_mhla_block_t* desc, const favit_mhla_block_mlp_t* rows,
+                                                 int64_t* offsets_out) {
+  int rc = check_geometry(desc);
+  if (rc != FAVIT_OK) return rc;
+  if ((rc = check_rows(desc, rows)) != FAVIT_OK) return rc;
+  int64_t s[TAPE_N];
+  tape_sizes(desc, rows->n_mlp, s);
+  return layout(s, TAPE_N, offsets_out);
+}
+
+extern "C" int64_t favit_mhla_block_bwd_layout2(const favit_mhla_block_t* desc, const favit_mhla_block_mlp_t* rows,
+                                                int32_t want_lp_out, int64_t* offsets_out) {
+  int rc = check_geometry(desc);
+  if (rc != FAVIT_OK) return rc;
+  if ((rc = check_rows(desc, rows)) != FAVIT_OK) return rc;
+  int64_t s[BWD_N];
+  bwd_sizes(desc, rows->n_mlp, want_lp_out, s);
+  return layout(s, BWD_N, offsets_out);
+}
+
+extern "C" int favit_mhla_block_attn_fwd(const favit_mhla_block_t* d, const favit_mhla_block_mlp_t* r, void* stream) {
+  int rc = check_geometry(d);
+  if (rc != FAVIT_OK) return rc;
+  if ((rc = check_rows(d, r)) != FAVIT_OK) return rc;
+  int64_t o[TAPE_N];
+  if ((rc = check_call(d, r->n_mlp, o)) != FAVIT_OK) return rc;
+  return attn_half_fwd(d, o, stream);
+}
+
+extern "C" int favit_mhla_block_mlp_fwd(const favit_mhla_block_t* d, const favit_mhla_block_mlp_t* r, void* stream) {
+  int rc = check_geometry(d);
+  if (rc != FAVIT_OK) return rc;
+  if ((rc = check_rows(d, r)) != FAVIT_OK) return rc;
+  if ((rc = check_x1c(r)) != FAVIT_OK) return rc;
+  int64_t o[TAPE_N];
+  if ((rc = check_call(d, r->n_mlp, o)) != FAVIT_OK) return rc;
+  return mlp_half_fwd(d, r->x1c, (int64_t)d->B * r->n_mlp, o, stream);
+}
+
+extern "C" int favit_mhla_block_mlp_bwd(const favit_mhla_block_t* d, const favit_mhla_block_mlp_t* r, const float* g_f32,
+                                        const void* g_lp, void* bwd_buffers, int64_t bwd_bytes, int32_t want_lp_out,
+                                        void* stream) {
+  int rc = check_geometry(d);
+  if (rc != FAVIT_OK) return rc;
+  if ((rc = check_rows(d, r)) != FAVIT_OK) return rc;
+  if ((rc = check_x1c(r)) != FAVIT_OK) return rc;
+  int64_t o[TAPE_N], b[BWD_N];
+  if ((rc = check_bwd_call(d, r->n_mlp, g_f32, g_lp, bwd_buffers, bwd_bytes, want_lp_out, o, b)) != FAVIT_OK) return rc;
+  char* w = reinterpret_cast<char*>(bwd_buffers);
+  return mlp_half_bwd(d, r->x1c, (int64_t)d->B * r->n_mlp, g_f32, g_lp, o, w, b,
+                      r->n_mlp == d->n ? w + b[G_G1_LP] : nullptr, stream);
+}
+
+extern "C" int favit_mhla_block_attn_bwd(const favit_mhla_block_t* d, const favit_mhla_block_mlp_t* r, const float* g1_f32,
+                                         const void* g1_lp, void* bwd_buffers, int64_t bwd_bytes, int32_t want_lp_out,
+                                         void* stream) {
+  int rc = check_geometry(d);
+  if (rc != FAVIT_OK) return rc;
+  if ((rc = check_rows(d, r)) != FAVIT_OK) return rc;
+  int64_t o[TAPE_N], b[BWD_N];
+  if ((rc = check_bwd_call(d, r->n_mlp, g1_f32, g1_lp, bwd_buffers, bwd_bytes, want_lp_out, o, b)) != FAVIT_OK) return rc;
+  return attn_half_bwd(d, g1_f32, g1_lp, o, reinterpret_cast<char*>(bwd_buffers), b, want_lp_out, stream);
+}
diff --git a/focused-attention-vit_amd/functional.py b/focused-attention-vit_amd/functional.py
--- a/focused-attention-vit_amd/functional.py
+++ b/focused-attention-vit_amd/functional.py
@@ -955,6 +955,19 @@
     return plan if any(c is not None for c in plan) else None
 
 
+def mlp_narrow_plan(cuts: Sequence[Optional[Tuple[int, int]]], after: Optional[Tuple[int, int]] = None):
+    cuts = list(cuts)
+    out: List[Optional[Tuple[int, int]]] = []
+    for k, c in enumerate(cuts):
+        nxt = cuts[k + 1] if k + 1 < len(cuts) else after
+        out.append(tuple(nxt) if nxt is not None and (c is None or sum(nxt) < sum(c)) else None)
+    return out
+
+
+def mlp_narrow_on() -> bool:
+    return not os.environ.get("FAVIT_NO_MLP_NARROW") and K.GEMM_TRACE is None
+
+
 _NATIVE = {"on": True}
 
 
@@ -976,11 +989,12 @@
 
 
 class _NativeTape:
-    __slots__ = ("plan", "buf", "x", "ln", "pa", "pm", "weff", "wc", "cut", "_bf", "_f32")
-
-    def __init__(self, plan, buf, x, ln, pa, pm, weff, wc, cut):
+    __slots__ = ("plan", "buf", "x", "ln", "pa", "pm", "weff", "wc", "cut", "mcut", "x1c", "mlp", "arena", "_bf", "_f32")
+
+    def __init__(self, plan, buf, x, ln, pa, pm, weff, wc, cut, mcut=None, x1c=None, mlp=None):
         self.plan, self.buf, self.x, self.ln, self.pa, self.pm, self.weff, self.wc, self.cut = \
             plan, buf, x, ln, pa, pm, weff, wc, cut
+        self.mcut, self.x1c, self.mlp, self.arena = mcut, x1c, mlp, None
         self._bf = self._f32 = None
 
     def bf(self, name, *shape):
@@ -995,32 +1009,46 @@
 
     def unpack(self):
         pl = self.plan
-        M, D, Hd = pl.M, pl.D, pl.hidden
+        M, Mm, D, Hd = pl.M, pl.Mm, pl.D, pl.hidden
         (g1, b1, g2, b2), (wp_c, w1_c, w2_c) = self.ln, self.wc
         lse = self.f32("lse", pl.B, pl.H, pl.n) if pl.off["lse"][1] else None
         sa = (self.bf("xn1", M, D), self.weff, self.bf("qkv", M, 3 * D), self.bf("o", M, D), wp_c, None, pl.B, pl.n,
               0.0, 0, 0.0, 0, self.pa, lse)
-        sm = (self.bf("xn2", M, D), (self.bf("pre", M, Hd), MLPChain.saves_gelu_grad(torch.bfloat16)), self.bf("h", M, Hd),
-              w1_c, w2_c, 0.0, 0, 0, self.pm)
-        return (self.x, self.f32("mu1", M), self.f32("rs1", M), (g1, b1), sa, self.f32("x1", M, D), self.f32("mu2", M),
-                self.f32("rs2", M), (g2, b2), sm, (self.pa, self.pm), self.cut)
+        if self.mlp is not None:
+            _, mu2, rs2, sm, _ = self.mlp
+        else:
+            sm = (self.bf("xn2", Mm, D), (self.bf("pre", Mm, Hd), MLPChain.saves_gelu_grad(torch.bfloat16)),
+                  self.bf("h", Mm, Hd), w1_c, w2_c, 0.0, 0, 0, self.pm)
+            mu2, rs2 = self.f32("mu2", Mm), self.f32("rs2", Mm)
+        x1 = self.x1c if self.mcut is not None else self.f32("x1", M, D)
+        return (self.x, self.f32("mu1", M), self.f32("rs1", M), (g1, b1), sa, x1, mu2, rs2, (g2, b2), sm,
+                (self.pa, self.pm), self.cut, self.mcut)
 
 
 def _tape_cut(tp):
     return tp.cut if isinstance(tp, _NativeTape) else tp[11]
 
 
+def _tape_mcut(tp):
+    return tp.mcut if isinstance(tp, _NativeTape) else tp[12]
+
+
 def _tape_rows(tp):
-    return tp.plan.M if isinstance(tp, _NativeTape) else tp[0].shape[0]
+    if isinstance(tp, _NativeTape):
+        return tp.plan.M + tp.plan.Mm
+    return tp[0].shape[0] + tp[5].shape[0]
 
 
 class EncoderOp:
 
-    def __init__(self, blocks: List[BlockSpec], mask=None, training=False, cuts=None):
+    def __init__(self, blocks: List[BlockSpec], mask=None, training=False, cuts=None, mlp_cuts=None):
         self.blocks, self.mask, self.training = blocks, mask, training
         self.cuts = list(cuts) if cuts is not None else None
         if self.cuts is not None and (len(self.cuts) != len(blocks) or mask is not None):
             raise ValueError("cuts: one entry per block, and no attention mask")
+        self.mlp_cuts = list(mlp_cuts) if mlp_cuts is not None else None
+        if self.mlp_cuts is not None and (self.cuts is None or len(self.mlp_cuts) != len(blocks)):
+            raise ValueError("mlp_cuts: one entry per block of an encoder with cuts")
 
     def fwd(self, ins, prm):
         (x,) = ins
@@ -1058,11 +1086,17 @@
                 cut = (L, ca, cb)
                 L = ca + cb
                 M = B * L
+            mc = self.mlp_cuts[bi] if self.mlp_cuts is not None else None
+            if mc is not None and sum(mc) >= L:
+                mc = None
             if native and pre[bi] is not None:
-                nt = self._fwd_native(bs, p, x, B, L, D, pre[bi], cut)
+                nt = self._fwd_native(bs, p, x, B, L, D, pre[bi], cut, mc)
                 if nt is not None:
                     tapes.append(nt)
-                    x = nt.f32("x2", M, D)
+                    if mc is not None:
+                        L = sum(mc)
+                        M = B * L
+                    x = nt.f32("x2", M, D) if nt.mlp is None else nt.mlp[4]
                     continue
             fuse = fuse_ok and M <= 16384
             if fuse and isinstance(bs.attn, (MHLAChain, DenseChain)):
@@ -1076,18 +1110,28 @@
                     x1, sa = bs.attn.fwd(xn1, pa, B, L, x, self.mask, self.training, pre=pre[bi])
                 else:
                     x1, sa = bs.attn.fwd(xn1, pa, B, L, x, self.mask, self.training)
-            if fuse and isinstance(bs.mlp, MLPChain):
-                o2 = [None, None, None]
-                x2, sm = bs.mlp.fwd(None, pm, x1, self.training, ln=(x1, g2.detach(), b2.detach(), o2))
-                xn2, mu2, rs2 = o2
-            else:
-                xn2, mu2, rs2 = K.layernorm_fwd(x1, D, g2, b2, M, D, cdt, q8=_q8_request(bs.mlp, pm, "fwd", D))
-                x2, sm = bs.mlp.fwd(xn2, pm, x1, self.training)
-            tapes.append((x, mu1, rs1, (g1, b1), sa, x1, mu2, rs2, (g2, b2), sm, (pa, pm), cut))
+            mcut = None
+            if mc is not None:
+                x1 = K.rows_cut_fwd(x1, B, L, mc[0], mc[1], D).reshape(B * sum(mc), D)
+                mcut = (L, mc[0], mc[1])
+                L = sum(mc)
+                M = B * L
+            xn2, mu2, rs2, sm, x2 = self._mlp_half_fwd(bs, pm, x1, g2, b2, M, D, cdt, fuse_ok)
+            tapes.append((x, mu1, rs1, (g1, b1), sa, x1, mu2, rs2, (g2, b2), sm, (pa, pm), cut, mcut))
             x = x2
         return x.reshape(B, L, D), (tapes, B, L_in, D)
 
-    def _fwd_native(self, bs, p, x, B, L, D, pre, cut):
+    def _mlp_half_fwd(self, bs, pm, x1, g2, b2, M, D, cdt, fuse_ok):
+        if fuse_ok and M <= 16384 and isinstance(bs.mlp, MLPChain):
+            o2 = [None, None, None]
+            x2, sm = bs.mlp.fwd(None, pm, x1, self.training, ln=(x1, g2.detach(), b2.detach(), o2))
+            xn2, mu2, rs2 = o2
+        else:
+            xn2, mu2, rs2 = K.layernorm_fwd(x1, D, g2, b2, M, D, cdt, q8=_q8_request(bs.mlp, pm, "fwd", D))
+            x2, sm = bs.mlp.fwd(xn2, pm, x1, self.training)
+        return xn2, mu2, rs2, sm, x2
+
+    def _fwd_native(self, bs, p, x, B, L, D, pre, cut, mc=None):
         at, ml = bs.attn, bs.mlp
         if not (isinstance(at, MHLAChain) and isinstance(ml, MLPChain)) or len(p) != 14:
             return None
@@ -1107,34 +1151,58 @@
         if plans is None:
             plans = g1._favit_blocks = {}
         key = (B, L, D, at.H, at.W, Hd, bool(self.training))
+        if mc is not None:
+            key += (sum(mc),)
         if key not in plans:
-            plans[key] = K.mhla_block_plan(*key)
+            plans[key] = K.mhla_block_plan(*key[:7], n_mlp=sum(mc)) if mc is not None else K.mhla_block_plan(*key)
         plan = plans[key]
         if plan is None:
             return None
         buf = torch.empty(plan.tape_bytes, dtype=torch.uint8, device=x.device)
         if K.mhla_block_fwd(plan, x, buf, g1, b1, g2, b2, weff, beff, wc[0], bp, wc[1], c1, wc[2], c2) != 0:
             return None
-        return _NativeTape(plan, buf, x, (g1, b1, g2, b2), p[2:8], p[10:], weff, wc, cut)
+        nt = _NativeTape(plan, buf, x, (g1, b1, g2, b2), p[2:8], p[10:], weff, wc, cut)
+        if mc is not None:
+            nt.mcut = (L, mc[0], mc[1])
+            nt.x1c = K.rows_cut_fwd(nt.f32("x1", plan.M, D), B, L, mc[0], mc[1], D).reshape(plan.Mm, D)
+            if K.mhla_block_mlp_fwd(plan, nt.x1c) != 0:
+                nt.mlp = self._mlp_half_fwd(bs, p[10:], nt.x1c, g2, b2, plan.Mm, D, torch.bfloat16, False)
+        return nt
 
     def _bwd_native(self, bs, tp, g, g_lp):
         plan = tp.plan
         g1, b1, g2, b2 = tp.ln
-        tg = [_gt(q) for q in tp.ln]
+        handed, tp.arena = tp.arena, None
+        tg = [_gt(g1), _gt(b1)] if handed is not None else [_gt(q) for q in tp.ln]
         if any(t is None for t in tg):
             return None
         M, D, Hd = plan.M, plan.D, plan.hidden
-        if (g.dtype != torch.float32 or g_lp.dtype != torch.bfloat16 or tuple(g.shape) != (M, D) or not g.is_contiguous()
-                or tuple(g_lp.shape) != (M, D) or not g_lp.is_contiguous()):
+        if handed is None and (g.dtype != torch.float32 or g_lp.dtype != torch.bfloat16 or tuple(g.shape) != (M, D)
+                               or not g.is_contiguous() or tuple(g_lp.shape) != (M, D) or not g_lp.is_contiguous()):
             return None
         want_lp = tp.cut is None
-        arena = torch.empty(plan.bwd_bytes[want_lp], dtype=torch.uint8, device=g.device)
+        if handed is not None:
+            arena, abf, af = handed
+        else:
+            arena = torch.empty(plan.bwd_bytes[want_lp], dtype=torch.uint8, device=g.device)
         wp_c, w1_c, w2_c = tp.wc
-        if K.mhla_block_bwd(plan, tp.x, tp.buf, g1, g2, tp.weff, wp_c, w1_c, w2_c, g, g_lp, arena, want_lp) != 0:
+        if handed is not None:
+            rc = K.mhla_block_bwd(plan, tp.x, tp.buf, g1, g2, tp.weff, wp_c, w1_c, w2_c, g, g_lp, arena, want_lp, ptrs_set=True)
+        else:
+            rc = K.mhla_block_bwd(plan, tp.x, tp.buf, g1, g2, tp.weff, wp_c, w1_c, w2_c, g, g_lp, arena, want_lp)
+        if rc != 0:
             return None
         bo = plan.boff[want_lp]
-        abf, af = arena.view(torch.bfloat16), arena.view(torch.float32)
+        if handed is None:
+            abf, af = arena.view(torch.bfloat16), arena.view(torch.float32)
         part = lambda k: _carve(af, bo[k][0] // 4, (2, plan.nparts, D))
+        if tp.mcut is not None:
+            dqkv = _carve(abf, bo["dqkv"][0] // 2, (M, 3 * D))
+            dwp, dbp = bs.attn.proj_grads(g_lp, tp.bf("o", M, D), tp.pa)
+            ga = bs.attn.qkv_grads(dqkv, tp.bf("xn1", M, D), tp.pa) + [dwp, dbp]
+            _DEFER["ln"].append((part("part1"), tg[0], tg[1], (g1, b1)))
+            g_out = _carve(af, bo["g_out_f32"][0] // 4, (M, D))
+            return g_out, (_carve(abf, bo["g_out_lp"][0] // 2, (M, D)) if want_lp else None), ga, None
         g1_lp = _carve(abf, bo["g1_lp"][0] // 2, (M, D))
         dqkv = _carve(abf, bo["dqkv"][0] // 2, (M, 3 * D))
         dw2, db2 = bs.mlp.fc2_grads(g_lp, tp.bf("h", M, Hd), tp.pm)
@@ -1146,12 +1214,35 @@
         g_out = _carve(af, bo["g_out_f32"][0] // 4, (M, D))
         return g_out, (_carve(abf, bo["g_out_lp"][0] // 2, (M, D)) if want_lp else None), ga, [dw1, db1, dw2, db2]
 
+    def _bwd_native_mlp(self, bs, tp, g, g_lp):
+        plan = tp.plan
+        g1, b1, g2, b2 = tp.ln
+        tg2, tb2 = _gt(g2), _gt(b2)
+        if tg2 is None or tb2 is None or tp.mlp is not None:
+            return None
+        Mm, D, Hd = plan.Mm, plan.D, plan.hidden
+        if (g.dtype != torch.float32 or g_lp.dtype != torch.bfloat16 or tuple(g.shape) != (Mm, D) or not g.is_contiguous()
+                or tuple(g_lp.shape) != (Mm, D) or not g_lp.is_contiguous()):
+            return None
+        want_lp = tp.cut is None
+        arena = torch.empty(plan.bwd_bytes[want_lp], dtype=torch.uint8, device=g.device)
+        wp_c, w1_c, w2_c = tp.wc
+        if K.mhla_block_mlp_bwd(plan, tp.x, tp.buf, g1, g2, tp.weff, wp_c, w1_c, w2_c, tp.x1c, g, g_lp, arena, want_lp) != 0:
+            return None
+        bo = plan.boff[want_lp]
+        abf, af = arena.view(torch.bfloat16), arena.view(torch.float32)
+        tp.arena = (arena, abf, af)
+        dw2, db2 = bs.mlp.fc2_grads(g_lp, tp.bf("h", Mm, Hd), tp.pm)
+        dw1, db1 = bs.mlp.fc1_grads(_carve(abf, bo["dpre"][0] // 2, (Mm, Hd)), tp.bf("xn2", Mm, D), tp.pm)
+        _DEFER["ln"].append((_carve(af, bo["part2"][0] // 4, (2, plan.nparts2, D)), tg2, tb2, (g2, b2)))
+        return _carve(af, bo["g1_f32"][0] // 4, (Mm, D)), [dw1, db1, dw2, db2]
+
     def bwd(self, saved, dy, needs):
         tapes, B, L, D = saved
         g = dy.reshape(-1, D)
         g_lp = _as_cdt(g)
         grads = []
-        begin_wgrads(per_block=any(_tape_cut(tp) is not None for tp in tapes))
+        begin_wgrads(per_block=any(_tape_cut(tp) is not None or _tape_mcut(tp) is not None for tp in tapes))
         begin_deferred()
         begin_zero_pool(sum(3 * D + 4 for bs in self.blocks if isinstance(bs.attn, MHLAChain)), dy.device)
 
@@ -1178,26 +1269,50 @@
                     nbs, ntp = order[bi + 1]
                     pd_n = nbs.mlp.out_dropout(ntp[9])
                     q8n = _q8_request(nbs.mlp, ntp[10][1], "bwd", D)
-                done = None
-                if isinstance(tp, _NativeTape):
-                    if not premasked and pd_n[0] == 0 and q8n is None and _DEFER["on"] and _native_blocks_on():
-                        done = self._bwd_native(bs, tp, g, g_lp)
-                    if done is None:
-                        tp = tp.unpack()
+                rows_tp = tp
+                nat_ok = (isinstance(tp, _NativeTape) and not premasked and pd_n[0] == 0 and q8n is None and _DEFER["on"]
+                          and _native_blocks_on())
+                narrowed = isinstance(tp, _NativeTape) and tp.mcut is not None
+                done = self._bwd_native(bs, tp, g, g_lp) if nat_ok and not narrowed else None
                 if done is not None:
                     g, g_lp, ga, gm = done
                     dg1 = db1 = dg2 = db2 = None
                     cut, lp_dt = tp.cut, torch.bfloat16
                 else:
-                    x, mu1, rs1, (g1, b1), sa, x1, mu2, rs2, (g2, b2), sm, (pa_, _), cut = tp
-                    dxn2, gm = bs.mlp.bwd(sm, g_lp, premasked=premasked)
-                    pd = bs.attn.out_dropout(sa) if hasattr(bs.attn, "out_dropout") else (0.0, 0)
-                    g, g_lp, dg2, db2 = ln_bwd(dxn2, x1, g2, b2, mu2, rs2, g, pd,
-                                               q8=_q8_request(bs.attn, pa_, "bwd", D) if hasattr(bs.attn, "out_dropout") else None)
-                    dxn1, ga = (bs.attn.bwd(sa, g_lp, premasked=pd[0] > 0) if hasattr(bs.attn, "out_dropout")
-                                else bs.attn.bwd(sa, g_lp))
-                    g, g_lp, dg1, db1 = ln_bwd(dxn1, x, g1, b1, mu1, rs1, g, pd_n, q8=q8n, want_lp=cut is None)
-                    lp_dt = dxn1.dtype
+                    nt, tp = (tp, None) if narrowed else (None, tp.unpack() if isinstance(tp, _NativeTape) else tp)
+                    half = self._bwd_native_mlp(bs, nt, g, g_lp) if narrowed and nat_ok else None
+                    pd = (0.0, 0)
+                    if half is not None:
+                        g, gm = half
+                        g_lp, dg2, db2 = None, None, None
+                        mcut, lp_dt = nt.mcut, torch.bfloat16
+                    else:
+                        tp = tp if tp is not None else nt.unpack()
+                        x1, mu2, rs2, (g2, b2), sm, (pa_, _), mcut = tp[5], tp[6], tp[7], tp[8], tp[9], tp[10], tp[12]
+                        dxn2, gm = bs.mlp.bwd(sm, g_lp, premasked=premasked)
+                        pd = bs.attn.out_dropout(tp[4]) if hasattr(bs.attn, "out_dropout") else (0.0, 0)
+                        g, g_lp, dg2, db2 = ln_bwd(dxn2, x1, g2, b2, mu2, rs2, g, pd,
+                                                   q8=_q8_request(bs.attn, pa_, "bwd", D) if hasattr(bs.attn, "out_dropout") else None,
+                                                   want_lp=mcut is None)
+                        lp_dt = dxn2.dtype
+                    if mcut is not None:
+                        g, g_lp = K.rows_cut_bwd(g, B, mcut[0], mcut[1], mcut[2], D, lp_dtype=lp_dt if g.dtype != lp_dt else None)
+                        g = g.reshape(B * mcut[0], D)
+                        g_lp = g_lp.reshape(B * mcut[0], D) if g_lp is not None else g
+                    half = self._bwd_native(bs, nt, g, g_lp) if narrowed and nat_ok else None
+                    if half is not None:
+                        g, g_lp, ga, _ = half
+                        dg1 = db1 = None
+                        cut = nt.cut
+                    else:
+                        tp = tp if tp is not None else nt.unpack()
+                        x, mu1, rs1, (g1, b1), sa, cut = tp[0], tp[1], tp[2], tp[3], tp[4], tp[11]
+                        dxn1, ga = (bs.attn.bwd(sa, g_lp, premasked=pd[0] > 0) if hasattr(bs.attn, "out_dropout")
+                                    else bs.attn.bwd(sa, g_lp))
+                        g, g_lp, dg1, db1 = ln_bwd(dxn1, x, g1, b1, mu1, rs1, g, pd_n, q8=q8n, want_lp=cut is None)
+                        lp_dt = dxn1.dtype
+                    if nt is not None:
+                        nt.arena = None
                 premasked = pd_n[0] > 0
                 if cut is not None:
                     n_in, ca, cb = cut
@@ -1205,7 +1320,7 @@
                     g, g_lp = K.rows_cut_bwd(g, B, n_in, ca, cb, D, lp_dtype=lp_dt if more else None)
                     g = g.reshape(B * n_in, D)
                     g_lp = g_lp.reshape(B * n_in, D) if g_lp is not None else g
-                nxt = (_tape_rows(tp), _tape_rows(order[bi + 1][1])) if bi + 1 < len(order) else None
+                nxt = (_tape_rows(rows_tp), _tape_rows(order[bi + 1][1])) if bi + 1 < len(order) else None
                 if flush_wgrads(force=False, next_rows=nxt) and _STATE["grad_ready"] is not None:
                     flush_deferred()
                 if not _SIDE["enabled"]:
diff --git a/focused-attention-vit_amd/kernels.py b/focused-attention-vit_amd/kernels.py
--- a/focused-attention-vit_amd/kernels.py
+++ b/focused-attention-vit_amd/kernels.py
@@ -51,7 +51,12 @@
     return None if t is None else C.c_void_p(t.data_ptr())
 
 
+_raw_stream = getattr(torch._C, "_cuda_getCurrentRawStream", None)
+
+
 def _st():
+    if _raw_stream is not None:
+        return C.c_void_p(_raw_stream(torch.cuda.current_device()))
     return C.c_void_p(torch.cuda.current_stream().cuda_stream)
 
 
@@ -520,27 +525,39 @@
 
 
 class BlockPlan:
-    __slots__ = ("desc", "ref", "M", "D", "hidden", "B", "n", "H", "nparts", "tape_bytes", "off", "bwd_bytes", "boff")
-
-
-def mhla_block_plan(B, n, D, H, W, hidden, training, eps=1e-5) -> Optional[BlockPlan]:
+    __slots__ = ("desc", "ref", "M", "D", "hidden", "B", "n", "H", "nparts", "tape_bytes", "off", "bwd_bytes", "boff",
+                 "n_mlp", "Mm", "nparts2", "rows", "rref", "st")
+
+
+def mhla_block_plan(B, n, D, H, W, hidden, training, eps=1e-5, n_mlp=None) -> Optional[BlockPlan]:
     d = _abi.BlockDesc()
     d.B, d.n, d.D, d.H, d.W, d.hidden, d.training, d.eps = B, n, D, H, W, hidden, int(bool(training)), eps
     lib = _abi.lib()
+    narrow = n_mlp is not None and n_mlp != n
+    p = BlockPlan()
+    p.rows = p.rref = p.st = None
+    if narrow:
+        p.rows = _abi.BlockMlp()
+        p.rows.n_mlp = n_mlp
+        p.rref = C.byref(p.rows)
     to = (C.c_int64 * len(_abi.BLOCK_TAPE_SLOTS))()
-    tape_bytes = lib.favit_mhla_block_tape_layout(C.byref(d), to)
+    tape_bytes = (lib.favit_mhla_block_tape_layout2(C.byref(d), p.rref, to) if narrow
+                  else lib.favit_mhla_block_tape_layout(C.byref(d), to))
     if tape_bytes < 0:
         return None
-    p = BlockPlan()
     p.desc, p.ref, p.M, p.D, p.hidden, p.B, p.n, p.H = d, C.byref(d), B * n, D, hidden, B, n, H
+    p.n_mlp = n_mlp if narrow else n
+    p.Mm = B * p.n_mlp
     p.nparts = int(min(2048, (B * n + 3) // 4))
+    p.nparts2 = int(min(2048, (p.Mm + 3) // 4))
     p.tape_bytes = d.tape_bytes = tape_bytes
     ends = list(to[1:]) + [tape_bytes]
     p.off = {k: (to[i], ends[i] - to[i]) for i, k in enumerate(_abi.BLOCK_TAPE_SLOTS)}
     p.bwd_bytes, p.boff = [], []
     for want_lp in (0, 1):
         bo = (C.c_int64 * len(_abi.BLOCK_BWD_SLOTS))()
-        nb = lib.favit_mhla_block_bwd_layout(C.byref(d), want_lp, bo)
+        nb = (lib.favit_mhla_block_bwd_layout2(C.byref(d), p.rref, want_lp, bo) if narrow
+              else lib.favit_mhla_block_bwd_layout(C.byref(d), want_lp, bo))
         ends = list(bo[1:]) + [nb]
         p.bwd_bytes.append(nb)
         p.boff.append({k: (bo[i], ends[i] - bo[i]) for i, k in enumerate(_abi.BLOCK_BWD_SLOTS)})
@@ -559,14 +576,42 @@
     d.g1, d.b1, d.g2, d.b2 = g1.data_ptr(), b1.data_ptr(), g2.data_ptr(), b2.data_ptr()
     d.weff, d.beff, d.wproj, d.bproj = weff.data_ptr(), beff.data_ptr(), wproj.data_ptr(), bproj.data_ptr()
     d.wfc1, d.bfc1, d.wfc2, d.bfc2 = wfc1.data_ptr(), bfc1.data_ptr(), wfc2.data_ptr(), bfc2.data_ptr()
+    if plan.rows is not None:
+        plan.st = _st()
+        return _block_code(_abi.lib().favit_mhla_block_attn_fwd(plan.ref, plan.rref, plan.st), "favit_mhla_block_attn_fwd")
     return _block_code(_abi.lib().favit_mhla_block_fwd(plan.ref, _st()), "favit_mhla_block_fwd")
 
 
-def mhla_block_bwd(plan: BlockPlan, x, tape, g1, g2, weff, wproj, wfc1, wfc2, g, g_lp, arena, want_lp_out: bool) -> int:
+def mhla_block_mlp_fwd(plan: BlockPlan, x1c) -> int:
+    plan.rows.x1c = x1c.data_ptr()
+    return _block_code(_abi.lib().favit_mhla_block_mlp_fwd(plan.ref, plan.rref, plan.st), "favit_mhla_block_mlp_fwd")
+
+
+def _block_bwd_ptrs(plan, x, tape, g1, g2, weff, wproj, wfc1, wfc2):
     d = plan.desc
     d.x, d.tape, d.tape_bytes = x.data_ptr(), tape.data_ptr(), tape.numel()
     d.g1, d.g2 = g1.data_ptr(), g2.data_ptr()
     d.weff, d.wproj, d.wfc1, d.wfc2 = weff.data_ptr(), wproj.data_ptr(), wfc1.data_ptr(), wfc2.data_ptr()
+
+
+def mhla_block_mlp_bwd(plan: BlockPlan, x, tape, g1, g2, weff, wproj, wfc1, wfc2, x1c, g, g_lp, arena,
+                       want_lp_out: bool) -> int:
+    _block_bwd_ptrs(plan, x, tape, g1, g2, weff, wproj, wfc1, wfc2)
+    plan.rows.x1c = x1c.data_ptr()
+    plan.st = _st()
+    return _block_code(_abi.lib().favit_mhla_block_mlp_bwd(plan.ref, plan.rref, g.data_ptr(), g_lp.data_ptr(),
+                                                           arena.data_ptr(), arena.numel(), int(bool(want_lp_out)), plan.st),
+                       "favit_mhla_block_mlp_bwd")
+
+
+def mhla_block_bwd(plan: BlockPlan, x, tape, g1, g2, weff, wproj, wfc1, wfc2, g, g_lp, arena, want_lp_out: bool,
+                   ptrs_set: bool = False) -> int:
+    if not ptrs_set:
+        _block_bwd_ptrs(plan, x, tape, g1, g2, weff, wproj, wfc1, wfc2)
+    if plan.rows is not None:
+        return _block_code(_abi.lib().favit_mhla_block_attn_bwd(plan.ref, plan.rref, g.data_ptr(), g_lp.data_ptr(),
+                                                                arena.data_ptr(), arena.numel(), int(bool(want_lp_out)),
+                                                                plan.st if ptrs_set else _st()), "favit_mhla_block_attn_bwd")
     return _block_code(_abi.lib().favit_mhla_block_bwd(plan.ref, g.data_ptr(), g_lp.data_ptr(), arena.data_ptr(),
                                                        arena.numel(), int(bool(want_lp_out)), _st()),
                        "favit_mhla_block_bwd")
diff --git a/focused-attention-vit_amd/models/vit.py b/focused-attention-vit_amd/models/vit.py
--- a/focused-attention-vit_amd/models/vit.py
+++ b/focused-attention-vit_amd/models/vit.py
@@ -105,7 +105,12 @@
             prm += params(b, s.names)
         if i:
             x = F.note_segment_boundary(x)
-        x = F.run(F.EncoderOp(specs, m, training, cuts=None if cuts is None else cuts[i:i + per]), [x], prm)
+        seg = mseg = None
+        if cuts is not None:
+            seg = cuts[i:i + per]
+            if F.mlp_narrow_on():
+                mseg = F.mlp_narrow_plan(seg, after=cuts[i + per] if i + per < len(cuts) else None)
+        x = F.run(F.EncoderOp(specs, m, training, cuts=seg, mlp_cuts=mseg), [x], prm)
     return x
 
 
diff --git a/include/favit.h b/include/favit.h
--- a/include/favit.h
+++ b/include/favit.h
@@ -226,6 +226,22 @@
 int favit_mhla_block_bwd(const favit_mhla_block_t* desc, const float* g_f32, const void* g_lp, void* bwd_buffers,
                          int64_t bwd_bytes, int32_t want_lp_out, void* stream);
 
+typedef struct favit_mhla_block_mlp {
+  const float* x1c;
+  int32_t n_mlp;
+  int32_t reserved;
+} favit_mhla_block_mlp_t;
+int64_t favit_mhla_block_tape_layout2(const favit_mhla_block_t* desc, const favit_mhla_block_mlp_t* rows,
+                                      int64_t* offsets_out );
+int64_t favit_mhla_block_bwd_layout2(const favit_mhla_block_t* desc, const favit_mhla_block_mlp_t* rows,
+                                     int32_t want_lp_out, int64_t* offsets_out );
+int favit_mhla_block_attn_fwd(const favit_mhla_block_t* desc, const favit_mhla_block_mlp_t* rows, void* stream);
+int favit_mhla_block_mlp_fwd(const favit_mhla_block_t* desc, const favit_mhla_block_mlp_t* rows, void* stream);
+int favit_mhla_block_mlp_bwd(const favit_mhla_block_t* desc, const favit_mhla_block_mlp_t* rows, const float* g_f32,
+                             const void* g_lp, void* bwd_buffers, int64_t bwd_bytes, int32_t want_lp_out, void* stream);
+int favit_mhla_block_attn_bwd(const favit_mhla_block_t* desc, const favit_mhla_block_mlp_t* rows, const float* g1_f32,
+                              const void* g1_lp, void* bwd_buffers, int64_t bwd_bytes, int32_t want_lp_out, void* stream);
+
 int favit_dropout(const void* x, void* y, int dtype, int64_t n, float p, uint64_t seed, void* stream);
 
 int favit_sppp_map_patches(const int64_t* seg, int32_t* patch_rank, int32_t* n_tokens, int32_t* perm,
```

New measurement: 57310 images/sec (median of 6 runs). +3.9%, better.
